# limuhit/pseudocylindrical_convolution

Measured on AMD Instinct MI355X. Metric: ERP MPix/s enc+dec, 4096x2048 model-idx 3, higher is better.
Workload: dtype f32; 1 GPU; ERP 4096x2048 encode+decode, model-idx 3 --ssim (valid_dim 56), 8 frame(s)/GPU/step; frames_per_gpu=8, parallelism=frames sharded, no data-path collective, weights=seeded random (transforms seed 1234, entropy randn*0.05 seed 7), content=smooth, cores_per_rank=16

## Files before the change

include/pconv_hip.h:

```cpp
#ifndef PCONV_HIP_H
#define PCONV_HIP_H

#include <stddef.h>
#include <stdint.h>

#ifdef __cplusplus
extern "C" {
#endif

#define PCONV_OK 0
#define PCONV_EINVAL (-1)
#define PCONV_ELAUNCH (-2)
#define PCONV_ENOMEM (-3)

const char *pconv_last_error(void);
int pconv_abi_version(void);
int pconv_device_count(void);


int pconv_host_tile_widths(const float *weight, int npart, int height, int width,
                           int32_t *widths);
int pconv_host_slice_widths(const float *weight, int npart, int height, int width,
                            int32_t *widths);

int pconv_host_slice_taps(const int32_t *widths, int npart, int width,
                          int32_t *tap_col, float *tap_coef );

int pconv_host_uslice_taps(const int32_t *widths, int npart, int width,
                           int32_t *tap_col, float *tap_coef);

int pconv_host_pad_table(const int32_t *widths, int npart, int height, int width, int pad,
                         int32_t *src_tile, int32_t *src_row, int32_t *col, float *wgt);

int pconv_host_wavefront(const int32_t *widths, int npart, int height, int width,
                         int32_t *order, int32_t *plane_start);

int pconv_host_causal_halo(const int32_t *widths, int npart, int channel, int height,
                           int width, int pad, int32_t *dst, int32_t *src0, int32_t *src1,
                           float *wgt, int32_t *entry_plane, int32_t *plane_start);

int pconv_host_causal_table(const int32_t *widths, int npart, int height, int width, int pad,
                            int32_t *col, float *wgt);

int pconv_host_project_table(const float *theta, const float *phi, int nview, float fov,
                             int h_out, int w_out, int height, int width, float *tf);


int pconv_sphere_slice(const float *in, float *out, const int32_t *widths,
                       const int32_t *tap_col, const float *tap_coef, int n, int c,
                       int height, int width, int npart, int pad, void *stream);

int pconv_sphere_uslice(const float *in, float *out, const int32_t *widths,
                        const int32_t *tap_col, const float *tap_coef, int n, int c, int h,
                        int width, int npart, int pad, void *stream);

int pconv_pseudo_pad(const float *in, float *out, const int32_t *widths,
                     const int32_t *src_tile, const int32_t *src_row, const int32_t *col,
                     const float *wgt, int tn, int c, int h, int w, int pad, int npart,
                     void *stream);

int pconv_pseudo_pad_ring(float *buf, const int32_t *widths, const int32_t *src_tile,
                          const int32_t *src_row, const int32_t *col, const float *wgt, int tn,
                          int c, int h, int w, int pad, int store, int npart, void *stream);

int pconv_pseudo_fill(float *data, const int32_t *widths, int tn, int c, int h, int w,
                      int npart, int pad, int trim, float fvalue, void *stream);

int pconv_dtow(const float *in, float *out, int n, int c, int h, int w, int stride, int d2w,
               void *stream);

int pconv_quant(const float *x, const float *weight, float *level_tab, float *out_val,
                float *out_idx, float *count, const int32_t *widths, int tn, int c, int h,
                int w, int levels, int npart, void *stream);

int pconv_leaky_clip(float *x, long long n, void *stream);

int pconv_frames_u8_to_f32(const uint8_t *in, float *out, int n, int height, int width, void *stream);
int pconv_frames_f32_to_u8(const float *in, uint8_t *out, int n, int height, int width, void *stream);

int pconv_erp_coded_size(int h, int w, int *H, int *W, int *top);
int pconv_frames_u8_to_f32_erp(const uint8_t *in, float *out, int n, int h, int w, void *stream);
int pconv_erp_pad_f32(const float *in, float *out, int n, int h, int w, void *stream);
int pconv_frames_f32_to_u8_crop(const float *in, uint8_t *out, int n, int h, int w, void *stream);

#define PCONV_YUV_420P 0
#define PCONV_YUV_NV12 1
#define PCONV_YUV_420P10LE 2
#define PCONV_YUV_BT709 0
#define PCONV_YUV_BT601 1
#define PCONV_YUV_LIMITED 0
#define PCONV_YUV_FULL 1
#define PCONV_YUV_MAX_WIDTH 11520
int pconv_frames_yuv420_to_f32(const void *in, float *out, int n, int h, int w, int fmt, int matrix, int range,
                               void *stream);
int pconv_frames_f32_to_yuv420(const float *in, void *out, int n, int h, int w, int fmt, int matrix, int range,
                               void *stream);

#define PCONV_WS_WEIGHT_SPHERE 0
#define PCONV_WS_WEIGHT_UNIFORM 1
long long pconv_ws_metrics_workspace_bytes(int n, int h, int w);
int pconv_ws_metrics_f32(const float *x, const float *y, int n, int c, int h, int w, int weighting, void *workspace,
                         double *out, void *stream);
int pconv_ws_metrics_u8(const uint8_t *x, const uint8_t *y, int n, int c, int h, int w, int weighting,
                        void *workspace, double *out, void *stream);

int pconv_ws_metrics_backward_f32(const float *x, const float *y, const double *gout, int n, int c, int h, int w,
                                  int weighting, float *grad_y, void *stream);

long long pconv_ws_msssim_workspace_bytes(int n, int c, int h, int w);
int pconv_ws_msssim_f32(const float *x, const float *y, int n, int c, int h, int w, int weighting, void *workspace,
                        double *out, void *stream);
int pconv_ws_msssim_u8(const uint8_t *x, const uint8_t *y, int n, int c, int h, int w, int weighting, void *workspace,
                       double *out, void *stream);
long long pconv_ws_msssim_backward_workspace_bytes(int n, int c, int h, int w);
int pconv_ws_msssim_backward_f32(const float *x, const float *y, const void *workspace, const double *values,
                                 const double *gout, int n, int c, int h, int w, int weighting, int swapped,
                                 void *backward_workspace, float *grad_y, void *stream);

int pconv_host_lanczos_taps(int n_in, int n_out, int32_t *first, float *weights, int *taps);
long long pconv_erp_resample_workspace_bytes(int n, int c, int h, int w, int h2, int w2);
int pconv_erp_resample_f32(const float *in, float *out, void *workspace, const int32_t *first_x, const float *wx, int tx,
                           const int32_t *first_y, const float *wy, int ty, int n, int c, int h, int w, int h2, int w2,
                           int clamp, void *stream);

long long pconv_host_lanczos_reverse_size(int n_in, int n_out);
int pconv_host_lanczos_reverse(int n_in, int n_out, int pole, int32_t *rev_start, int32_t *rev_entry, uint8_t *crossed);
long long pconv_erp_resample_backward_workspace_bytes(int n, int c, int h, int w, int h2, int w2);
int pconv_erp_resample_backward_f32(const float *gout, float *gin, void *workspace, const float *wx, int tx,
                                    const int32_t *rev_start_x, const int32_t *rev_entry_x, const float *wy, int ty,
                                    const int32_t *rev_start_y, const int32_t *rev_entry_y, const uint8_t *rev_crossed_y,
                                    int n, int c, int h, int w, int h2, int w2, void *stream);

#define PCONV_ERP_ROTATE_PHASES 256
#define PCONV_ERP_ROTATE_TAPS 6
int pconv_host_erp_rotation_matrix(int yaw, int pitch, int roll, int inverse, double *m);
int pconv_host_lanczos_phases(float *weights);
int pconv_erp_rotation_map(int32_t *map, int h, int w, int yaw, int pitch, int roll, int inverse, void *stream);
int pconv_erp_remap_f32(const float *in, float *out, const int32_t *map, const float *phases, int n, int c, int h, int w,
                        int clamp, void *stream);

#define PCONV_VIEWPORT_MAX_SS 4
int pconv_host_viewport_basis(int yaw, int pitch, int roll, int hfov, int vfov, double *out);
int pconv_viewport_map(int32_t *map, int h, int w, int gh, int gw, int yaw, int pitch, int roll, int hfov, int vfov,
                       void *stream);
int pconv_viewport_render_f32(const float *in, float *out, const int32_t *map, const float *phases, int n, int c, int h,
                              int w, int vh, int vw, int ss, long long out_frame_stride, int clamp, void *stream);

#define PCONV_CUBE_CMP 1
#define PCONV_CUBE_EAC 2
#define PCONV_CUBE_PAD 3
#define PCONV_CUBE_MAX_FACE 9453
int pconv_host_cube_face_of(double x, double y, double z);
int pconv_cube_from_erp_map(int32_t *map, int kind, int a, int ss, int h, int w, void *stream);
int pconv_cube_pad_f32(const float *in, float *out, const int32_t *table, int n, int c, int a, void *stream);
int pconv_cube_to_erp_map(int32_t *map, int kind, int a, int h, int w, int ss, void *stream);

#define PCONV_SPHERE_POINTS_LANCZOS 0
#define PCONV_SPHERE_POINTS_NEAREST 1
#define PCONV_SPHERE_POINTS_CHUNK 1024
int pconv_sphere_points_records(const double *points, int32_t *records, long long P, int h, int w, void *stream);
int pconv_sphere_points_sample_f32(const float *in, float *out, const int32_t *records, const float *phases, int n, int c,
                                   int h, int w, long long P, int mode, void *stream);
long long pconv_sphere_points_mse_workspace_bytes(int n, int c, long long P);
int pconv_sphere_points_mse_f32(const float *x, int h1, int w1, const int32_t *rec_x, const float *y, int h2, int w2,
                                const int32_t *rec_y, const float *phases, int n, int c, long long P, int mode,
                                void *workspace, double *out, void *stream);

long long pconv_host_remap_reverse_size(int gh, int gw);
int pconv_host_remap_reverse(const int32_t *map, int gh, int gw, int h, int w, int32_t *rev_start, int32_t *rev_entry);
int pconv_remap_backward_f32(const float *gout, float *gin, const int32_t *map, const float *phases, const int32_t *rev_start,
                             const int32_t *rev_entry, int n, int c, int h, int w, int vh, int vw, int ss,
                             long long gout_frame_stride, int accumulate, void *stream);

int pconv_dquant(const float *x, const float *weight, float *level_tab, float *out,
                 const int32_t *widths, int tn, int c, int h, int w, int wc, int levels,
                 int npart, void *stream);

int pconv_project(const float *in, const float *tf, float *out, int n, int c, int height,
                  int width, int nview, int h_out, int w_out, int nearest, void *stream);

int pconv_context_reshape(const float *in, float *out, int n, int c, int h, int w, int ngroup,
                          void *stream);


int pconv_context_reshape_backward(const float *top, float *bottom, int n, int c, int h, int w,
                                   int ngroup, void *stream);

int pconv_sphere_slice_backward(const float *gout, float *gin, const int32_t *widths,
                                const int32_t *tap_col, const float *tap_coef, int n, int c,
                                int height, int width, int npart, int pad, void *stream);

int pconv_sphere_uslice_backward(const float *gout, float *gin, const int32_t *widths,
                                 const int32_t *tap_col, const float *tap_coef, int n, int c, int h,
                                 int width, int npart, int pad, void *stream);

int pconv_host_pad_reverse(const int32_t *widths, int npart, int height, int width, int pad,
                           int32_t *rev_start, int32_t *rev_dst, float *rev_wgt);

int pconv_pseudo_pad_backward(const float *gout, float *gin, const int32_t *widths,
                              const int32_t *rev_start, const int32_t *rev_dst, const float *rev_wgt,
                              int tn, int c, int h, int w, int pad, int npart, void *stream);

int pconv_entropy_pad(const float *in, float *out, const int32_t *widths, const int32_t *col,
                      const float *wgt, int tn, int c, int h, int w, int pad, int npart, void *stream);
int pconv_host_entropy_pad_table(const int32_t *widths, int npart, int height, int width, int pad,
                                 int version, int32_t *col, float *wgt);
int pconv_host_causal_reverse(const int32_t *widths, int npart, int height, int width, int pad,
                              int version, int32_t *rev_start, int32_t *rev_dst, float *rev_wgt);
int pconv_entropy_pad_backward(const float *gout, float *gin, const int32_t *widths,
                               const int32_t *rev_start, const int32_t *rev_dst, const float *rev_wgt,
                               int tn, int c, int h, int w, int pad, int npart, void *stream);

int pconv_project_backward(const float *gout, const float *tf, float *gin, float *count, int n, int c,
                           int height, int width, int nview, int h_out, int w_out, int nearest,
                           void *stream);

int pconv_quant_backward(const float *x, const float *val, const float *idx, const float *g_val,
                         const float *g_idx, const float *level_tab, float *g_in, float *g_weight,
                         float *bins, const int32_t *widths, float top_alpha, int tn, int c, int h,
                         int w, int levels, int npart, void *stream);


long long pconv_host_tap_reverse_size(const int32_t *widths, int npart, int width, int uslice);

int pconv_host_tap_reverse(const int32_t *widths, int npart, int width, const int32_t *tap_col,
                           const float *tap_coef, int uslice, int32_t *rev_start, int32_t *rev_src,
                           float *rev_coef);

long long pconv_host_project_reverse_size(int nview, int inner, int nearest);

int pconv_host_project_reverse(const float *tf, int nview, int inner, int height, int width, int nearest,
                               int32_t *rev_start, int32_t *rev_sample, float *rev_wgt);

int pconv_sphere_slice_backward_ordered(const float *gout, float *gin, const int32_t *widths,
                                        const int32_t *rev_start, const int32_t *rev_src,
                                        const float *rev_coef, int n, int c, int height, int width,
                                        int npart, int pad, void *stream);
int pconv_sphere_uslice_backward_ordered(const float *gout, float *gin, const int32_t *widths,
                                         const int32_t *rev_start, const int32_t *rev_src,
                                         const float *rev_coef, int n, int c, int h, int width,
                                         int npart, int pad, void *stream);

int pconv_project_backward_ordered(const float *gout, const int32_t *rev_start, const int32_t *rev_sample,
                                   const float *rev_wgt, float *gin, float *count, int n, int c,
                                   int height, int width, int nview, int h_out, int w_out, void *stream);

long long pconv_quant_backward_ordered_workspace_bytes(int tn, int c, int levels);
int pconv_quant_backward_ordered(const float *x, const float *val, const float *idx, const float *g_val,
                                 const float *g_idx, const float *level_tab, float *g_in, float *g_weight,
                                 float *bins, void *workspace, const int32_t *widths, float top_alpha,
                                 int tn, int c, int h, int w, int levels, int npart, void *stream);

int pconv_mask_constrain(float *weight, int nout, int cin, int k, int ngroup, int constrain,
                         void *stream);

int pconv_gmm_loss(const float *weight, const float *delta, const float *mean,
                   const float *label, float *loss, float *d_weight, float *d_delta,
                   float *d_mean, float *d_label, int m, int ng, void *stream);

int pconv_conv_packed_size(int cout, int cin, int k, int *cout_pad, int *red_pad);
int pconv_conv_pack_weight(const float *w, float *packed, int cout, int cin, int k,
                           void *stream);
int pconv_conv2d(const float *in, const float *packed_w, const float *bias, float *out,
                 int tn, int cin, int h, int w, int cout, int k, int stride, int act,
                 const float *slope, const int32_t *col_limit, int npart,
                 const float *residual, const float *gate, int trim, int d2w,
                 const long long *views, void *stream);

int pconv_conv_pack_weight_transposed(const float *w, float *packed, int cout, int cin, int k,
                                      void *stream);
long long pconv_conv2d_dgrad_workspace_bytes(int tn, int cout, int h, int w, int k, int stride);
int pconv_conv_grad_prepare(const float *gout, float *prepared, int tn, int cout, int h, int w,
                            int k, int stride, void *stream);
int pconv_conv2d_dgrad(const float *gout, const float *packed_wt, float *gin, void *workspace,
                       int tn, int cin, int h, int w, int cout, int k, int stride, void *stream);
long long pconv_conv2d_wgrad_workspace_bytes(int tn, int cin, int cout, int k);
int pconv_conv2d_wgrad(const float *in, const float *gout, float *gw, float *gb, void *workspace,
                       int tn, int cin, int h, int w, int cout, int k, int stride, void *stream);

int pconv_conv5_packed_size(int cout, int cin, int *cout_pad, int *red_pad);
int pconv_conv5_pack_weight(const float *w, float *packed, int cout, int cin, void *stream);
int pconv_conv5_pack_weight_transposed(const float *w, float *packed, int cout, int cin, void *stream);
int pconv_conv5(const float *in, const float *packed_w, const float *bias, float *out, int tn, int cin,
                int h, int w, int cout, void *stream);
long long pconv_conv5_dgrad_workspace_bytes(int tn, int cout, int h, int w);
int pconv_conv5_dgrad(const float *gout, const float *packed_wt, float *gin, void *workspace, int tn,
                      int cin, int h, int w, int cout, void *stream);
long long pconv_conv5_wgrad_workspace_bytes(int tn, int cin, int cout);
int pconv_conv5_wgrad(const float *in, const float *gout, float *gw, float *gb, void *workspace, int tn,
                      int cin, int h, int w, int cout, void *stream);

long long pconv_wino_packed_size(int cout, int cin);
int pconv_wino_pack_weight(const float *w, float *packed, int cout, int cin, void *stream);
int pconv_wino_supported(int cin, int h, int w, int cout, int d2w);
int pconv_conv3x3_wino(const float *in, const float *packed_u, const float *bias, float *out,
                       int tn, int cin, int h, int w, int cout, int act, const float *slope,
                       const int32_t *col_limit, int npart, const float *residual, int trim,
                       int d2w, const long long *views, void *stream);
int pconv_conv3x3_wino_flat(const float *in, const float *packed_u, const float *bias, float *out,
                       int tn, int cin, int h, int w, int cout, int act, const float *slope,
                       const int32_t *col_limit, int npart, const float *residual, int trim,
                       int d2w, const long long *views, void *stream);

long long pconv_wino42_packed_size(int cout, int cin);
int pconv_wino42_pack_weight(const float *w, float *packed, int cout, int cin, void *stream);
int pconv_wino42_supported(int cin, int h, int w, int cout, int d2w);
int pconv_conv3x3_wino42(const float *in, const float *packed_u, const float *bias, float *out,
                       int tn, int cin, int h, int w, int cout, int act, const float *slope,
                       const int32_t *col_limit, int npart, const float *residual, int trim,
                       int d2w, const long long *views, void *stream);

int pconv_gdn(const float *in, const float *packed_gamma, const float *beta, float *out,
              int tn, int ch, int h, int w, int inverse, const int32_t *col_limit, int npart,
              const float *residual ,
              const long long *views ,
              void *stream);


int pconv_dinput2(const float *packed, float *ctx, const int32_t *order, int lo, int len,
                  int nimg, int ngroup, int npart, int h, int w, int pad, int psum,
                  float bias, int rep, void *stream);

int pconv_ctx_pad_run2(float *data, const int32_t *dst, const int32_t *src0,
                       const int32_t *src1, const float *wgt, const int32_t *entry_plane,
                       int lo, int len, int nimg, int cpn, int channel, int npart, int h, int w,
                       int pad, int psum, void *stream);

int pconv_entropy_conv(const float *x, const float *weight, const float *bias,
                       const float *slope, float *y, const int32_t *order,
                       const int32_t *plane_start, int first_plane, int nplane, int max_plane_len,
                       int nimg, int per_set, int cin, int cout, int ngroup, int k, int constrain,
                       int npart, int h, int w, int pad_in, int pad_out, int psum,
                       const float *residual, const int32_t *widths, const int32_t *vh_col,
                       const float *vh_wgt, void *stream);

int pconv_entropy_add(float *y, const float *x, const int32_t *order, int lo, int len,
                      int nimg, int channel, int ngroup, int npart, int h, int w, int pad,
                      int psum, void *stream);

int pconv_dextract2(const float *x, float *out, const int32_t *order, int lo, int len,
                    int nimg, int channel, int cpn, int npart, int h, int w, int psum,
                    void *stream);

int pconv_dextract2_batch(const float *x, float *out, const int32_t *order, int lo, int len,
                          int nimg, int channel, int cpn, int npart, int h, int w, int psum,
                          int nout, long long section_stride, void *stream);

int pconv_gmm_table(float *weight, float *delta, const float *mean, float *table, int tn,
                    int ng, int nstep, float bias, float total, float beta, int batch_arith,
                    void *stream);

int pconv_step_tables(const float *y, const float *symbols, int32_t *table, int32_t *labels,
                      const int32_t *order, int lo, int len, int nimg, int ngroup, int npart, int h,
                      int w, int psum, int nstep, float bias, float total, float beta, void *stream);

int pconv_symbols_to_ctx(const float *symbols, float *ctx, const int32_t *widths, int tn, int c,
                         int h, int w, int pad, int npart, float bias, int rep, void *stream);

int pconv_ctx_to_symbols(const float *ctx, float *out, const int32_t *widths, int tn, int c, int h,
                         int w, int pad, int npart, float bias, void *stream);

typedef struct pconv_entropy_engine pconv_entropy_engine;

pconv_entropy_engine *pconv_ee_create(int npart, int ngroup, int h, int w, int nimg,
                                      const float *tile_weight, float bias, int nlevels, float total,
                                      float beta);
void pconv_ee_destroy(pconv_entropy_engine *e);
int pconv_stream_create(void **stream);
int pconv_stream_destroy(void *stream);
int pconv_ee_set_layer(pconv_entropy_engine *e, int layer, const float *weight, const float *bias,
                       const float *slope, void *stream);
long long pconv_ee_symbols_per_image(const pconv_entropy_engine *e);
int pconv_ee_steps(const pconv_entropy_engine *e);
int pconv_ee_host_cpus(void);
int pconv_ee_spin_us(int call_threads);
int pconv_ee_host_plan(int nimg, int *groups, int *group_threads, int *queued_chain, int *blocking_sync);
int pconv_ee_wait_mode(const pconv_entropy_engine *e);
int pconv_ee_encoder_form(const pconv_entropy_engine *e, int layer);
#define PCONV_OPTION_AUTO (-2147483647 - 1)
int pconv_option(const pconv_entropy_engine *e, const char *name, int *value);
int pconv_device_blocking_sync(int enable);
int pconv_ee_encode(pconv_entropy_engine *e, const float *symbols, void *stream);
int pconv_ee_encode_begin(pconv_entropy_engine *e, const float *symbols, void *stream);
int pconv_ee_set_encode_ranges(pconv_entropy_engine *e, int nrange);
int pconv_ee_encode_end(pconv_entropy_engine *e, void *stream);
const uint8_t *pconv_ee_stream(const pconv_entropy_engine *e, int img, size_t *nbytes);
int pconv_ee_decode(pconv_entropy_engine *e, const uint8_t *const *streams, const size_t *nbytes,
                    float *symbols_out, void *stream);
int pconv_ee_rate(pconv_entropy_engine *e, const float *symbols, double *bits_dev, float *map_dev_or_null, void *stream);


typedef struct pconv_optim_tensor {
  float *p;
  const float *grad;
  float *acc;
  float *m;
  float *v;
  long long n;
  float step_size, bc2_sqrt, eps, one_minus_beta1, beta2, one_minus_beta2;
} pconv_optim_tensor;


long long pconv_host_optim_segments(const long long *counts, int ntensor, int32_t *segments);
long long pconv_optim_workspace_bytes(int ntensor, int nsegment);
int pconv_optim_sqnorm(const pconv_optim_tensor *records, const int32_t *segments, const long long *counts,
                       int ntensor, int nsegment, float clip, void *workspace, void *stream);
int pconv_optim_adam(const pconv_optim_tensor *records, const int32_t *segments, const long long *counts,
                     int ntensor, int nsegment, const void *workspace, void *stream);

#ifdef __cplusplus
}
#endif
#endif
```

pseudocylindrical_convolution_amd/PCONV.py:

```python
import collections
import ctypes
import functools
import os
import weakref

import numpy as np
import torch

from . import _native
from ._native import PconvError, call

__all__ = [
    "ProjectsOp", "DtowOp", "ContextReshapeOp", "EntropyGmmOp", "MaskConstrainOp",
    "SphereSliceOp", "SphereUsliceOp", "EntropyGmmTableOp", "EntropyContextOp",
    "EntropyCtxPadRun2Op", "DExtract2Op", "DInput2Op", "EntropyConv2Op", "PseudoContextOp",
    "PseudoPadOp", "PseudoFillOp", "PseudoEntropyContextOp", "PseudoEntropyPadOp",
    "PseudoQuantOp", "PseudoDQuantOp", "EntropyAddOp",
]

_contexts = weakref.WeakValueDictionary()


def _lookup(addr):
    try:
# ... 1516 lines not shown

def _sphere_points_records_of(what, rec, x):
    if rec.dtype != torch.int32 or rec.dim() != 2 or rec.shape[1] != 2 or not rec.is_contiguous() or rec.device != x.device \
            or not 1 <= rec.shape[0] <= SPHERE_POINTS_MAX:
        raise PconvError("%s: the records must be contiguous int32 (P, 2), 1 <= P < 2^28, on the input's device, got %s %s "
                         "on %s" % (what, rec.dtype, tuple(rec.shape), rec.device))
    return rec.shape[0]


def sphere_points_records(points, h, w, out=None):
    h, w = int(h), int(w)
    if not points.is_cuda or points.dtype != torch.float64 or points.dim() != 2 or points.shape[1] != 2 \
            or not points.is_contiguous() or not 1 <= points.shape[0] <= SPHERE_POINTS_MAX:
        raise PconvError("sphere_points_records: contiguous float64 (P, 2) points, 1 <= P < 2^28, on a GPU expected, got %s "
                         "%s on %s" % (points.dtype, tuple(points.shape), points.device))
    _require_sides("sphere_points_records", h, w)
    count = points.shape[0]
    out = _output("sphere_points_records", out, (count, 2), torch.int32, points.device, "the points' device")
    with _HbmTimed("sphere_points_records_kernel", "SpherePointsRecords %dx%d P%d" % (w, h, count), 24.0 * count, points.device):
        call("pconv_sphere_points_records", _ptr(points), _ptr(out), count, h, w, _stream(points.device))
    return out


def sphere_points_sample_f32(x, records, interp="lanczos", out=None):
    n, c, h, w = _require_frames(x, "sphere_points_sample_f32")
    mode = _sphere_points_mode("sphere_points_sample_f32", interp)
    count = _sphere_points_records_of("sphere_points_sample_f32", records, x)
    out = _output("sphere_points_sample_f32", out, (n, c, count), torch.float32, x.device, "the input's device")
    counted = 4.0 * n * c * count * ((36 if mode == 0 else 1) + 1) + 8.0 * n * count
    with _HbmTimed("sphere_points_sample_kernel", "SpherePointsSample %dx%d n%d P%d" % (w, h, n, count), counted, x.device):
        call("pconv_sphere_points_sample_f32", _ptr(x), _ptr(out), _ptr(records), _ptr(_phase_table(x.device)), n, c, h, w,
             count, mode, _stream(x.device))
    return out


def sphere_points_mse_device(x, rec_x, y, rec_y, interp="lanczos"):
    _require_gpu(x, "sphere_points_mse")
    _require_gpu(y, "sphere_points_mse")
    if x.dim() != 4 or y.dim() != 4 or x.shape[:2] != y.shape[:2] or x.device != y.device:
        raise PconvError("sphere_points_mse: two float32 (n, C, h, w) batches of equal n and C on one device expected, got "
                         "%s on %s and %s on %s" % (tuple(x.shape), x.device, tuple(y.shape), y.device))
    mode = _sphere_points_mode("sphere_points_mse", interp)
    count = _sphere_points_records_of("sphere_points_mse", rec_x, x)
    if _sphere_points_records_of("sphere_points_mse", rec_y, y) != count:
        raise PconvError("sphere_points_mse: the two record lists differ in length: %d and %d" % (count, rec_y.shape[0]))
    n, c = x.shape[:2]
    nbytes = call("pconv_sphere_points_mse_workspace_bytes", n, c, count)
    workspace = torch.empty((nbytes,), dtype=torch.uint8, device=x.device)
    out = torch.empty((n, c), dtype=torch.float64, device=x.device)
    counted = 4.0 * n * c * count * 2 * (36 if mode == 0 else 1) + 16.0 * n * c * count
    with _HbmTimed("sphere_points_mse_kernel", "SpherePointsMse n%d P%d" % (n, count), counted, x.device):
        call("pconv_sphere_points_mse_f32", _ptr(x), x.shape[2], x.shape[3], _ptr(rec_x), _ptr(y), y.shape[2], y.shape[3],
             _ptr(rec_y), _ptr(_phase_table(x.device)), n, c, count, mode, _ptr(workspace), _ptr(out), _stream(x.device))
    return out


def sphere_points_mse(x, rec_x, y, rec_y, interp="lanczos"):
    return sphere_points_mse_device(x, rec_x, y, rec_y, interp).cpu()


def viewport_map(h, w, gh, gw, view, device=None, out=None):
    h, w, gh, gw = int(h), int(w), int(gh), int(gw)
    try:
        yaw, pitch, roll, hfov, vfov = (int(v) for v in view)
    except (TypeError, ValueError):
        raise PconvError("viewport_map: a view is five integers in units of 2^-16 degree, got %r" % (view,))
    device = _gpu_device("viewport_map", device)
    if not (2 <= gh <= 1 << 22 and 2 <= gw <= 1 << 22) or 8 * gh * gw >= 1 << 31:
        raise PconvError("viewport_map: a grid of %dx%d: sides of 2 .. 2^22 and a map below 2^31 bytes expected" % (gw, gh))
    out = _output("viewport_map", out, (gh, gw, 2), torch.int32, device, device)
    with torch.cuda.device(device), _HbmTimed("viewport_map_kernel", "ViewportMap %dx%d" % (gw, gh), 8.0 * gh * gw, device):
        call("pconv_viewport_map", _ptr(out), h, w, gh, gw, yaw, pitch, roll, hfov, vfov, _stream(device))
    return out


def viewport_render_f32(x, map, vh, vw, ss, clamp=False, out=None, slot=0):
    n, c, h, w = _require_frames(x, "viewport_render_f32")
    vh, vw, ss, slot = int(vh), int(vw), int(ss), int(slot)
    _require_view("viewport_render_f32", vh, vw, ss)
    _require_map("viewport_render_f32", map, vh * ss, vw * ss, x.device, "the input's device")
    table = _phase_table(x.device)
    if out is None:
        out = torch.empty((n, 1, c, vh, vw), dtype=torch.float32, device=x.device)
    elif out.dim() != 5 or out.shape[0] != n or tuple(out.shape[2:]) != (c, vh, vw) or out.dtype != torch.float32 \
            or not out.is_contiguous() or out.device != x.device:
        raise PconvError("viewport_render_f32: out must be contiguous float32 (%d, V, %d, %d, %d) on the input's device"
                         % (n, c, vh, vw))
    views = out.shape[1]
    if not 0 <= slot < views:
        raise PconvError("viewport_render_f32: slot %d of %d views" % (slot, views))
    frame = c * vh * vw
    counted = 4.0 * 36 * n * c * vh * vw * ss * ss + 8.0 * n * c * vh * vw * ss * ss + 4.0 * n * frame
    with _HbmTimed("viewport_render_f32_kernel", "ViewportRender %dx%d->%dx%d ss%d n%d" % (w, h, vw, vh, ss, n), counted,
                   x.device):
        call("pconv_viewport_render_f32", _ptr(x), out.data_ptr() + 4 * slot * frame, _ptr(map), _ptr(table), n, c, h, w,
             vh, vw, ss, views * frame, 1 if clamp else 0, _stream(x.device))
    return out


def remap_backward_f32(gout, map, lists, h, w, vh, vw, ss, gin=None, slot=0, accumulate=False):
    _require_gpu(gout, "remap_backward_f32")
    h, w, vh, vw, ss, slot = int(h), int(w), int(vh), int(vw), int(ss), int(slot)
    if gout.dim() == 4:
        gout = gout.unsqueeze(1)
    if gout.dim() != 5 or tuple(gout.shape[3:]) != (vh, vw) or not gout.is_contiguous():
        raise PconvError("remap_backward_f32: a contiguous float32 (n, V, C, %d, %d) or (n, C, %d, %d) gradient expected, got %s"
                         % (vh, vw, vh, vw, tuple(gout.shape)))
    n, views, c = gout.shape[:3]
    if not 0 <= slot < views:
        raise PconvError("remap_backward_f32: slot %d of %d views" % (slot, views))
    _require_view("remap_backward_f32", vh, vw, ss)
    _require_map("remap_backward_f32", map, vh * ss, vw * ss, gout.device, "the gradient's device")
    entries = 36 * vh * ss * vw * ss
    try:
        start, entry = lists
        good = all(t.dtype == torch.int32 and t.dim() == 1 and t.is_contiguous() and t.device == gout.device
                   for t in (start, entry)) and start.numel() == h * w + 1 and entry.numel() == entries
    except (TypeError, ValueError, AttributeError):
        good = False
    if not good:
        raise PconvError("remap_backward_f32: lists must be (start, entry) of viewport.reverse_lists for this map and a %dx%d "
                         "source: contiguous int32 of %d and %d elements on the gradient's device" % (w, h, h * w + 1, entries))
    if gin is None and accumulate:
        raise PconvError("remap_backward_f32: accumulate needs the gin to add to")
    gin = _output("remap_backward_f32", gin, (n, c, h, w), torch.float32, gout.device, "the gradient's device", "gin")
    table = _phase_table(gout.device)
    frame = c * vh * vw
    counted = n * ((c + 3) // 4) * (4.0 * entries + 8.0 * entries + 4.0 * (h * w + 1)) + 4.0 * n * c * entries \
        + 4.0 * gin.numel() * (2 if accumulate else 1)
    with _HbmTimed("remap_backward_f32_kernel", "RemapBackward %dx%d<-%dx%d ss%d n%d" % (w, h, vw, vh, ss, n), counted,
                   gout.device):
        call("pconv_remap_backward_f32", gout.data_ptr() + 4 * slot * frame, _ptr(gin), _ptr(map), _ptr(table), _ptr(start),
             _ptr(entry), n, c, h, w, vh, vw, ss, views * frame, 1 if accumulate else 0, _stream(gout.device))
    return gin


CUBE_KINDS = {"cmp": 1, "eac": 2}
CUBE_PAD = 3
CUBE_MAX_FACE = 9453


def _cube_args(what, kind, a, ss):
    if kind not in CUBE_KINDS:
        raise PconvError("%s: kind must be one of %s, got %r" % (what, sorted(CUBE_KINDS), kind))
    a, ss = int(a), int(ss)
    if not (2 <= a <= CUBE_MAX_FACE and 1 <= ss <= 4):
        raise PconvError("%s: a face size of %d with ss = %d: a of 2 .. %d and ss of 1 .. 4 expected" % (what, a, ss, CUBE_MAX_FACE))
    return CUBE_KINDS[kind], a, ss


def cube_from_erp_map(kind, a, ss, h, w, device=None, out=None):
    code, a, ss = _cube_args("cube_from_erp_map", kind, a, ss)
    h, w = int(h), int(w)
    device = _gpu_device("cube_from_erp_map", device)
    _require_sides("cube_from_erp_map", h, w)
    gs = a * ss
    if 8 * 6 * gs * gs >= 1 << 31:
        raise PconvError("cube_from_erp_map: a map of %dx%d records is 2^31 bytes or more" % (gs, 6 * gs))
    out = _output("cube_from_erp_map", out, (6 * gs, gs, 2), torch.int32, device, device)
    with torch.cuda.device(device), _HbmTimed("cube_from_erp_map_kernel", "CubeFromErpMap a%d ss%d" % (a, ss), 48.0 * gs * gs,
                                              device):
        call("pconv_cube_from_erp_map", _ptr(out), code, a, ss, h, w, _stream(device))
    return out


def cube_to_erp_map(kind, a, h, w, ss, device=None, out=None):
    code, a, ss = _cube_args("cube_to_erp_map", kind, a, ss)
    h, w = int(h), int(w)
    device = _gpu_device("cube_to_erp_map", device)
    _require_sides("cube_to_erp_map", h, w)
    if 8 * h * ss * w * ss >= 1 << 31:
        raise PconvError("cube_to_erp_map: a map of %dx%d records is 2^31 bytes or more" % (w * ss, h * ss))
    out = _output("cube_to_erp_map", out, (h * ss, w * ss, 2), torch.int32, device, device)
    with torch.cuda.device(device), _HbmTimed("cube_to_erp_map_kernel", "CubeToErpMap %dx%d ss%d" % (w, h, ss),
                                              8.0 * h * w * ss * ss, device):
        call("pconv_cube_to_erp_map", _ptr(out), code, a, h, w, ss, _stream(device))
    return out


def cube_pad_f32(x, table, out=None):
    n, c, h6, a = _require_frames(x, "cube_pad_f32")
    if h6 != 6 * a or not 2 <= a <= CUBE_MAX_FACE:
        raise PconvError("cube_pad_f32: a face stack (n, C, 6 a, a), a of 2 .. %d, expected, got %s" % (CUBE_MAX_FACE, tuple(x.shape)))
    A = a + 2 * CUBE_PAD
    ring = 6 * (A * A - a * a)
    if table.dtype != torch.int32 or tuple(table.shape) != (ring, 3) or not table.is_contiguous() or table.device != x.device:
        raise PconvError("cube_pad_f32: the table must be contiguous int32 (%d, 3) on the input's device" % ring)
    out = _output("cube_pad_f32", out, (n, c, 6 * A, A), torch.float32, x.device, "the input's device")
    counted = 4.0 * (x.numel() + out.numel()) + n * c * ring * (12.0 + 16.0)
    with _HbmTimed("cube_pad_f32_kernel", "CubePad a%d n%d" % (a, n), counted, x.device):
        call("pconv_cube_pad_f32", _ptr(x), _ptr(out), _ptr(table), n, c, a, _stream(x.device))
    return out


WS_WEIGHTINGS = {"ws": 0, "uniform": 1}


def ws_metrics(x, y, weighting="ws"):
    return ws_metrics_device(x, y, weighting).cpu()


def _ws_frames(what, x, y, weighting, float_only, min_side, entry):
    if weighting not in WS_WEIGHTINGS:
        raise PconvError("%s: weighting must be one of %s, got %r" % (what, sorted(WS_WEIGHTINGS), weighting))
    if not (x.is_cuda and y.is_cuda):
        raise PconvError("%s: expected GPU tensors (this build has no CPU path), got %s and %s" % (what, x.device, y.device))
    if x.device != y.device or x.dtype != y.dtype or x.shape != y.shape:
        raise PconvError("%s: the two batches differ: %s %s %s vs %s %s %s"
                         % (what, x.device, x.dtype, tuple(x.shape), y.device, y.dtype, tuple(y.shape)))
    if not (x.is_contiguous() and y.is_contiguous()) or x.dim() != 4:
        raise PconvError("%s: contiguous 4-D tensors expected" % what)
    if x.dtype == torch.float32:
        n, c, h, w = x.shape
        fn = entry + "_f32"
    elif x.dtype == torch.uint8 and x.shape[3] == 3 and not float_only:
        n, h, w, c = x.shape
        fn = entry + "_u8"
    else:
        raise PconvError("%s: float32 (n, C, h, w)%s expected, got %s %s"
                         % (what, "" if float_only else " or uint8 (n, h, w, 3)", x.dtype, tuple(x.shape)))
    if h < min_side or w < min_side:
        raise PconvError("%s: h and w must be at least %d, got %dx%d" % (what, min_side, w, h))
    return (n, c, h, w), fn


def _ws_gout(what, gout, x):
    n = x.shape[0]
    if not gout.is_cuda or gout.device != x.device or gout.dtype != torch.float64 or tuple(gout.shape) != (n, 2) \
            or not gout.is_contiguous():
        raise PconvError("%s: gout must be contiguous float64 (%d, 2) on the inputs' device, got %s %s %s"
                         % (what, n, gout.device, gout.dtype, tuple(gout.shape)))


def ws_metrics_device(x, y, weighting="ws"):
    (n, c, h, w), fn = _ws_frames("ws_metrics", x, y, weighting, False, 1, "pconv_ws_metrics")
    nbytes = call("pconv_ws_metrics_workspace_bytes", n, h, w)
    workspace = torch.empty((nbytes,), dtype=torch.uint8, device=x.device)
    out = torch.empty((n, 2), dtype=torch.float64, device=x.device)
    with _HbmTimed("ms_forward_kernel", "WsMetrics n%d" % n, 2.0 * x.numel() * x.element_size(), x.device):
        call(fn, _ptr(x), _ptr(y), n, c, h, w, WS_WEIGHTINGS[weighting], _ptr(workspace), _ptr(out), _stream(x.device))
    return out


def ws_metrics_backward(x, y, gout, weighting="ws"):
    (n, c, h, w), _ = _ws_frames("ws_metrics_backward", x, y, weighting, True, 1, "pconv_ws_metrics")
    _ws_gout("ws_metrics_backward", gout, x)
    out = torch.empty_like(x)
    with _HbmTimed("ms_backward_kernel", "WsMetricsBackward n%d" % n, 12.0 * x.numel(), x.device):
        call("pconv_ws_metrics_backward_f32", _ptr(x), _ptr(y), _ptr(gout), n, c, h, w, WS_WEIGHTINGS[weighting],
             _ptr(out), _stream(x.device))
    return out


WS_MS_SCALES, WS_MS_MIN_SIDE = 5, 16


def ws_msssim_device(x, y, weighting="ws"):
    (n, c, h, w), fn = _ws_frames("ws_msssim", x, y, weighting, False, WS_MS_MIN_SIDE, "pconv_ws_msssim")
    nbytes = call("pconv_ws_msssim_workspace_bytes", n, c, h, w)
    workspace = torch.empty((nbytes,), dtype=torch.uint8, device=x.device)
    out = torch.empty((n, 7), dtype=torch.float64, device=x.device)
    counted = 2.0 * x.numel() * x.element_size() + 2.0 * (2.0 * n * c * h * w * 4 / 3)
    with _HbmTimed("ms_forward_kernel", "WsMsSsim n%d" % n, counted, x.device):
        call(fn, _ptr(x), _ptr(y), n, c, h, w, WS_WEIGHTINGS[weighting], _ptr(workspace), _ptr(out), _stream(x.device))
    return out, workspace


def ws_msssim(x, y, weighting="ws"):
    out, workspace = ws_msssim_device(x, y, weighting)
    return out.cpu(), workspace


def ws_msssim_levels(workspace, n, c, h, w):
    levels, at = [], 0
    for s in range(1, WS_MS_SCALES):
        hs, ws = h >> s, w >> s
        size = n * c * hs * ws
        pair = workspace[4 * at:4 * (at + 2 * size)].view(torch.float32)
        levels.append((pair[:size].view(n, c, hs, ws), pair[size:].view(n, c, hs, ws)))
        at += 2 * size
    return levels


def ws_msssim_backward(x, y, workspace, values, gout, weighting="ws", swapped=False):
    (n, c, h, w), _ = _ws_frames("ws_msssim_backward", x, y, weighting, True, WS_MS_MIN_SIDE, "pconv_ws_msssim")
    _ws_gout("ws_msssim_backward", gout, x)
    if values.device != x.device or values.dtype != torch.float64 or tuple(values.shape) != (n, 7) \
            or not values.is_contiguous():
        raise PconvError("ws_msssim_backward: values must be contiguous float64 (%d, 7) on the inputs' device, got %s %s %s"
                         % (n, values.device, values.dtype, tuple(values.shape)))
    nbytes = call("pconv_ws_msssim_workspace_bytes", n, c, h, w)
    if workspace.device != x.device or workspace.dtype != torch.uint8 or workspace.numel() != nbytes \
            or not workspace.is_contiguous():
        raise PconvError("ws_msssim_backward: the workspace must be the %d bytes ws_msssim_device returned, got %s %s %s"
                         % (nbytes, workspace.device, workspace.dtype, tuple(workspace.shape)))
    coarse = torch.empty((call("pconv_ws_msssim_backward_workspace_bytes", n, c, h, w),), dtype=torch.uint8, device=x.device)
    out = torch.empty_like(x)
    with _HbmTimed("ms_backward_kernel", "WsMsSsimBackward n%d" % n, 16.0 * x.numel(), x.device):
        call("pconv_ws_msssim_backward_f32", _ptr(x), _ptr(y), _ptr(workspace), _ptr(values), _ptr(gout), n, c, h, w,
             WS_WEIGHTINGS[weighting], 1 if swapped else 0, _ptr(coarse), _ptr(out), _stream(x.device))
    return out


def tile_gdn(owner, x, gamma, beta, inverse, col_limit=None, npart=0, residual=None, ring=0):
    x = _require_rows(x, "tile_gdn")
    tn, ch, h, w = x.shape
    stream = _stream(x.device)
    packed = packed_conv_weight(owner, gamma.view(ch, ch, 1, 1), stream)
    out = _ring_output((tn, ch, h, w), ring, x)
    residual = _like_output(residual, out, "tile_gdn: residual")
    views = _views(x, out, residual)

    def describe():
        return (conv_kernel_name(ch, 1, 1, True, cin=ch, pixels=tn * h * w), "GDN %d w%d" % (ch, w),
                2.0 * ch * ch * tn * h * w * _VALID_FRACTION,
                4.0 * ch * tn * h * w * _VALID_FRACTION * (3 if residual is not None else 2))

    with _ConvTimed(x.device, describe):
        call("pconv_gdn", _ptr(x), _ptr(packed), _ptr(beta.detach().contiguous()), _ptr(out), tn, ch, h, w,
             1 if inverse else 0, _ptr(col_limit), int(npart), _ptr(residual), ctypes.addressof(views), stream)
    return out


FUSED_EPILOGUE = True


def tile_conv2d(owner, x, weight, bias, stride, slope=None, col_limit=None, npart=0, sigmoid=False, gate=None,
                residual=None, trim=False, ring=0, d2w=False):
    x = _require_rows(x, "tile_conv2d")
    tn, cin, h, w = x.shape
    cout, cin_w, k, k2 = weight.shape
    if cin != cin_w or k != k2:
        raise PconvError("tile_conv2d: weight %s does not fit input %s" % (tuple(weight.shape), tuple(x.shape)))
    stream = _stream(x.device)
    ho, wo = (h - k) // stride + 1, (w - k) // stride + 1
    out = _ring_output((tn, cout // 4, 2 * ho, 2 * wo) if d2w else (tn, cout, ho, wo), ring, x)
    if sigmoid and slope is not None:
        raise PconvError("tile_conv2d: PReLU and sigmoid are exclusive")
    if d2w and (gate is not None or residual is not None or trim or sigmoid or cout % 4):
        raise PconvError("tile_conv2d: d2w takes no sigmoid / gate / residual / trim and needs cout % 4 == 0")
    gate = _like_output(gate, out, "tile_conv2d: gate")
    residual = _like_output(residual, out, "tile_conv2d: residual")
    aligned = k == 3 and _aligned8(out) and (residual is None or _aligned8(residual))
    launches, fallback = conv_plan(cin, h, w, cout, k, stride, d2w, sigmoid or gate is not None, aligned)
    if fallback:
        key = (cin, h, w, cout, bool(d2w))
        conv_fallbacks[key] = conv_fallbacks.get(key, 0) + 1
    act = 4 if sigmoid else (1 if slope is not None else 0)
    bias_p, slope_p = _ptr(bias.detach()) if bias is not None else None, _ptr(slope.detach()) if slope is not None else None

    def winograd(kind, r0, rows):
        kernel = CONV_KERNELS[kind]
        whole = r0 == 0 and rows == ho
        rs = 2 if d2w else 1
        xv = x if whole else x[:, :, r0:r0 + rows + 2]
        ov = out if whole else out[:, :, rs * r0:rs * (r0 + rows)]
        rv = residual if (whole or residual is None) else residual[:, :, r0:r0 + rows]

        def describe():
            return (kernel.probe_name, "3x3 s1 %d->%d w%d" % (cin, cout, wo) + ("" if whole else (" rows %d of %d" % (rows, ho))),
                    2.0 * cin * 9 * cout * tn * rows * wo * _VALID_FRACTION,
                    4.0 * tn * _VALID_FRACTION * (cin * (rows + 2) * w + cout * rows * wo * (1 + (residual is not None))))

        with _ConvTimed(x.device, describe):
            views = _views(xv, ov, rv)
            call(kernel.entry, _ptr(xv), _ptr(_packed_weight(owner, weight, kind, stream)), bias_p, _ptr(ov), tn, cin,
                 rows + 2, w, cout, act, slope_p, _ptr(col_limit), int(npart), _ptr(rv), 1 if trim else 0,
                 1 if d2w else 0, ctypes.addressof(views), stream)

    def direct():
        def describe():
            return (conv_kernel_name(cout, k, stride, cin=cin, pixels=tn * h * w),
                    "%dx%d s%d %d->%d w%d" % (k, k, stride, cin, cout, wo), 2.0 * cin * k * k * cout * tn * ho * wo * _VALID_FRACTION,
                    4.0 * tn * _VALID_FRACTION * (cin * h * w + cout * ho * wo * (1 + (residual is not None) + (gate is not None))))

        with _ConvTimed(x.device, describe):
            views = _views(x, out, residual, gate)
            call("pconv_conv2d", _ptr(x), _ptr(_packed_weight(owner, weight, "direct", stream)), bias_p, _ptr(out),
                 tn, cin, h, w, cout, k, int(stride), act, slope_p, _ptr(col_limit), int(npart),
                 _ptr(residual), _ptr(gate), 1 if trim else 0, 1 if d2w else 0, ctypes.addressof(views), stream)

    for kind, r0, rows in launches:
        if kind == "direct":
            direct()
        else:
            winograd(kind, r0, rows)
    return out


def _conv_tensors(where, tensors):
    first = tensors[0][1]
    for name, t, dims in tensors:
        if not isinstance(t, torch.Tensor) or t.dim() != dims:
            raise PconvError("%s: %s must be a %d-D tensor" % (where, name, dims))
        _require_gpu(t.detach(), "%s: %s" % (where, name))
        if t.device != first.device:
            raise PconvError("%s: %s is on %s, %s on %s" % (where, name, t.device, tensors[0][0], first.device))


ConvFamily = collections.namedtuple(
    "ConvFamily", "ksizes strides sized slot_t packed_size pack_weight_transposed dgrad_workspace dgrad wgrad_workspace wgrad")
_TILE_CONV = ConvFamily((1, 3), (1, 2), True, "_pconv_packed_t", "pconv_conv_packed_size", "pconv_conv_pack_weight_transposed",
                        "pconv_conv2d_dgrad_workspace_bytes", "pconv_conv2d_dgrad", "pconv_conv2d_wgrad_workspace_bytes",
                        "pconv_conv2d_wgrad")
_CONV5 = ConvFamily((5,), (1,), False, "_pconv_packed5_t", "pconv_conv5_packed_size", "pconv_conv5_pack_weight_transposed",
                    "pconv_conv5_dgrad_workspace_bytes", "pconv_conv5_dgrad", "pconv_conv5_wgrad_workspace_bytes",
                    "pconv_conv5_wgrad")


def _pack_transposed(weight, family, stream):
    cout, cin, k = weight.shape[:3]
    ks = (k,) if family.sized else ()
    return _pack(weight, family.packed_size, (cin, cout) + ks + (None, None), family.pack_weight_transposed, (cout, cin) + ks,
                 stream)


def _conv_backward(where, family, x, weight, gout, stride, need, owner):
    need_x, need_w, need_b = (bool(n) for n in need)
    _conv_tensors(where, [("gout", gout, 4), ("x", x, 4), ("weight", weight, 4)])
    tn, cout, ho, wo = gout.shape
    cout_w, cin, k, k2 = weight.shape
    stride = int(stride)
    tn_x, cin_x, h, w = x.shape
    if (tn_x, cin_x, cout_w, k2) != (tn, cin, cout, k) or k not in family.ksizes or stride not in family.strides or \
            ((h - k) // stride + 1, (w - k) // stride + 1) != (ho, wo) or ho < 1 or wo < 1:
        raise PconvError("%s: x %s, weight %s, gout %s, stride %d do not fit"
                         % (where, tuple(x.shape), tuple(weight.shape), tuple(gout.shape), stride))
    stream = _stream(gout.device)
    lib = _native.hip_lib()
    ks, kst = ((k,), (k, stride)) if family.sized else ((), ())

    def workspace(nbytes):
        if nbytes < 0:
            raise PconvError("%s: workspace query failed: %s" % (where, (lib.pconv_last_error() or b"").decode()))
        return torch.empty(int(nbytes), dtype=torch.uint8, device=gout.device) if nbytes else None

    gin = gw = gb = None
    if need_x:
        packed = _cached_pack(weight if owner is None else owner, family.slot_t, weight, _pack_transposed, family, stream)
        gin = torch.empty((tn, cin, h, w), dtype=torch.float32, device=gout.device)
        ws = workspace(getattr(lib, family.dgrad_workspace)(tn, cout, h, w, *kst))
        call(family.dgrad, _ptr(gout), _ptr(packed), _ptr(gin), _ptr(ws), tn, cin, h, w, cout, *kst + (stream,))
    if need_w or need_b:
        if need_w:
            gw = torch.empty((cout, cin, k, k), dtype=torch.float32, device=gout.device)
        if need_b:
            gb = torch.empty((cout,), dtype=torch.float32, device=gout.device)
        ws = workspace(getattr(lib, family.wgrad_workspace)(tn, cin, cout, *ks) if need_w else tn * cout * 8)
        call(family.wgrad, _ptr(x) if need_w else None, _ptr(gout), _ptr(gw), _ptr(gb), _ptr(ws), tn, cin, h, w, cout,
             *kst + (stream,))
    return gin, gw, gb


def tile_conv2d_backward(x, weight, gout, stride, need=(True, True, True), owner=None):
    return _conv_backward("tile_conv2d_backward", _TILE_CONV, x, weight, gout, stride, need, owner)



OptimSegments = collections.namedtuple("OptimSegments", "table counts ntensor nsegment")


def optim_segments(counts, device):
    counts = np.ascontiguousarray(counts, dtype=np.int64)
    if counts.ndim != 1 or counts.size < 1:
        raise PconvError("optim_segments: a non-empty list of element counts expected")
    nsegment = call("pconv_host_optim_segments", _np_ptr(counts), counts.size, None)
    table = np.empty((nsegment, 2), dtype=np.int32)
    call("pconv_host_optim_segments", _np_ptr(counts), counts.size, _np_ptr(table))
    return OptimSegments(torch.from_numpy(table).to(device), counts, int(counts.size), int(nsegment))


def optim_step(records, segments, clip, device):
    if records.dtype != torch.int64 or tuple(records.shape) != (segments.ntensor, 9) or not records.is_cuda or \
            not records.is_contiguous() or records.device != segments.table.device or records.device != torch.device(device):
        raise PconvError("optim_step: records must be a contiguous (%d, 9) int64 tensor on %s" % (segments.ntensor, device))
    stream = _stream(records.device)
    nbytes = call("pconv_optim_workspace_bytes", segments.ntensor, segments.nsegment)
    ws = torch.empty(nbytes // 8, dtype=torch.float64, device=records.device)
    args = (_ptr(records), _ptr(segments.table), _np_ptr(segments.counts), segments.ntensor, segments.nsegment)
    call("pconv_optim_sqnorm", *args + (float(clip), _ptr(ws), stream))
    call("pconv_optim_adam", *args + (_ptr(ws), stream))
    return ws



def _pack5(weight, stream):
    cout, cin = weight.shape[:2]
    return _pack(weight, "pconv_conv5_packed_size", (cout, cin, None, None), "pconv_conv5_pack_weight", (cout, cin), stream)


def conv5x5(owner, x, weight, bias):
    _conv_tensors("conv5x5", [("x", x, 4), ("weight", weight, 4)] + ([("bias", bias, 1)] if bias is not None else []))
    tn, cin, h, w = x.shape
    cout, cin_w, k, k2 = weight.shape
    if cin != cin_w or (k, k2) != (5, 5) or h < 5 or w < 5 or (bias is not None and bias.shape[0] != cout):
        raise PconvError("conv5x5: weight %s does not fit input %s" % (tuple(weight.shape), tuple(x.shape)))
    stream = _stream(x.device)
    out = torch.empty((tn, cout, h - 4, w - 4), dtype=torch.float32, device=x.device)
    call("pconv_conv5", _ptr(x), _ptr(_cached_pack(owner, "_pconv_packed5", weight, _pack5, stream)),
         _ptr(bias.detach()) if bias is not None else None, _ptr(out), tn, cin, h, w, cout, stream)
    return out


def conv5x5_backward(x, weight, gout, need=(True, True, True), owner=None):
    return _conv_backward("conv5x5_backward", _CONV5, x, weight, gout, 1, need, owner)
```

pseudocylindrical_convolution_amd/PCONV_operator/ops.py:

```python
import math

import torch
from torch import nn

from . import backend
from .BaseOpModule import BaseOpModule, native_call
from .GDN import LowerBound
from .base import set_weight


def _per_gpu(module, factory):
    return {gid: factory(gid) for gid in module.device_list}


class SphereSlice(BaseOpModule):

    def __init__(self, npart, interp_type=0, pad=0, opt=False, device=0, time_it=False):
        super(SphereSlice, self).__init__(device)
        weight = set_weight(npart, opt)
        self.op = _per_gpu(self, lambda g: backend.ops().SphereSliceOp(npart, interp_type, pad, weight, g, time_it))

    def forward(self, x):
        return native_call(self, 'forward', (x,))


class SphereUslice(BaseOpModule):

    def __init__(self, npart, interp_type=0, pad=0, opt=False, device=0, time_it=False):
        super(SphereUslice, self).__init__(device)
        weight = set_weight(npart, opt)
        self.op = _per_gpu(self, lambda g: backend.ops().SphereUsliceOp(npart, interp_type, pad, weight, g, time_it))

    def forward(self, x):
        return native_call(self, 'forward', (x,))


class Dtow(BaseOpModule):

    def __init__(self, stride=2, d2w=False, device=0, time_it=False):
        super(Dtow, self).__init__(device)
        self.op = _per_gpu(self, lambda g: backend.ops().DtowOp(stride, d2w, g, time_it))

    def forward(self, x):
        return native_call(self, 'forward', (x,))


class MultiProjectM(BaseOpModule):

    def __init__(self, h, w, thetas, phis, fov=0.6, near=False, device_id=0, time_flag=False):
        super(MultiProjectM, self).__init__(device_id)
        self.op = _per_gpu(self, lambda g: backend.ops().ProjectsOp(int(h), int(w), thetas, phis, fov, near, g, time_flag))

    def forward(self, x):
        return native_call(self, 'forward', (x,))


class MultiProject(MultiProjectM):
    THETAS = [-0.5, 0, 0.5, 1, -0.5, 0, 0.5, 1, -0.5, 0, 0.5, 1, 0, 0]
    PHIS = [0, 0, 0, 0, 0.25, 0.25, 0.25, 0.25, -0.25, -0.25, -0.25, -0.25, 0.5, -0.5]

    def __init__(self, h, w, fov=0.6, near=False, device_id=0, time_flag=False):
        self.thetas, self.phis = list(self.THETAS), list(self.PHIS)
        super(MultiProject, self).__init__(h, w, self.thetas, self.phis, fov, near, device_id, time_flag)


class _Context(BaseOpModule):

    def setup_context(self, w):
        for op in self.op.values():
            op.start_context(w)

    def get_addr(self, gid):
        return self.op[gid].addr()


class PseudoContextV2(_Context):

    def __init__(self, npart, opt=True, rt=20, device=0, time_it=False):
        super(PseudoContextV2, self).__init__(device)
        weight = set_weight(npart, opt)
        self.op = _per_gpu(self, lambda g: backend.ops().PseudoContextOp(npart, rt, weight, g, time_it))

    def produce_fill_param(self, gid, h, w):
        return self.op[gid].produce_fill_param(h, w)


class PseudoEntropyContext(_Context):

    def __init__(self, npart, context_version=1, opt=True, rt=20, device=0, time_it=False):
        super(PseudoEntropyContext, self).__init__(device)
        weight = set_weight(npart, opt)
        self.op = _per_gpu(self, lambda g: backend.ops().PseudoEntropyContextOp(npart, rt, context_version, weight, g, time_it))


class EntropyContextNew(_Context):

    def __init__(self, npart, rt=18, opt=False, device=0, time_it=False):
        super(EntropyContextNew, self).__init__(device)
        weight = set_weight(npart, opt)
        self.op = _per_gpu(self, lambda g: backend.ops().EntropyContextOp(npart, rt, weight, g, time_it))


class PseudoPadV2(BaseOpModule):

    def __init__(self, pad, npart, ctx, device=0, time_it=False):
        super(PseudoPadV2, self).__init__(device)
        self.op = _per_gpu(self, lambda g: backend.ops().PseudoPadOp(pad, npart, ctx.get_addr(g), g, time_it))

    def forward(self, x):
        op = self.native(x)
        if getattr(x, "_pconv_ring", None) is not None and hasattr(op, "forward_ring") \
                and not torch.is_grad_enabled():
            return op.forward_ring(x)
        return native_call(self, 'forward', (x,))


class PseudoEntropyPad(BaseOpModule):

    def __init__(self, pad, npart, ctx, device=0, time_it=False):
        super(PseudoEntropyPad, self).__init__(device)
        self.op = _per_gpu(self, lambda g: backend.ops().PseudoEntropyPadOp(pad, npart, ctx.get_addr(g), g, time_it))

    def forward(self, x):
        return native_call(self, 'forward', (x,))


class PseudoFillV2(BaseOpModule):

    def __init__(self, pad, npart, ctx, fvalue=0, trim=0, device=0, time_it=False):
        super(PseudoFillV2, self).__init__(device)
        version = 0 if isinstance(ctx, PseudoContextV2) else (1 if isinstance(ctx, PseudoEntropyContext) else 2)
        self.op = _per_gpu(self, lambda g: backend.ops().PseudoFillOp(pad, npart, fvalue, trim, ctx.get_addr(g), version, g, time_it))

    def forward(self, x):
        return native_call(self, 'forward', (x,))


class PseudoGDNV2(nn.Module):

    def __init__(self, ch, npart, ctx, device=0, inverse=False, beta_min=1e-6, gamma_init=.1,
                 reparam_offset=2 ** -18):
        super(PseudoGDNV2, self).__init__()
        self.inverse = inverse
        self.beta_min = beta_min
        self.gamma_init = gamma_init
        self.reparam_offset = torch.FloatTensor([reparam_offset])
        self.trim = PseudoFillV2(0, npart, ctx, device=device)
        self.mask = None
        self.__dict__["ctx"] = ctx
        gid = device if isinstance(device, int) else device[0]
        self.build(ch, torch.device(backend.device_of(gid)))

    def build(self, ch, device):
        self.pedestal = self.reparam_offset ** 2
        self.beta_bound = (self.beta_min + self.reparam_offset ** 2) ** .5
        self.gamma_bound = self.reparam_offset
        self.beta = nn.Parameter(torch.sqrt(torch.ones(ch) + self.pedestal).to(device))
        gamma = torch.sqrt(self.gamma_init * torch.eye(ch) + self.pedestal)
        self.gamma = nn.Parameter(gamma.to(device))
        self.pedestal = self.pedestal.to(device)

    def setup_mask(self, x):
        if self.mask is not None and self.mask.shape == x.shape and self.mask.device == x.device:
            return
        self.mask = self.trim(torch.ones_like(x).detach())

    def effective(self):
        key = (self.gamma._version, self.beta._version, self.gamma.device, backend.param_epoch())
        if getattr(self, "_effective", (None,))[0] != key:
            with torch.no_grad():
                pedestal = self.pedestal.to(self.gamma.device)
                beta = LowerBound.apply(self.beta, self.beta_bound) ** 2 - pedestal
                gamma = LowerBound.apply(self.gamma, self.gamma_bound) ** 2 - pedestal
            self._effective = (key, gamma.contiguous(), beta.contiguous())
        return self._effective[1], self._effective[2]

    def forward(self, inputs, residual=None, trim=None, ring=0):
        ops = backend.ops()
        if hasattr(ops, "tile_gdn") and inputs.is_cuda and not torch.is_grad_enabled():
            gamma, beta = self.effective()
            ctx_op = self.ctx.native(inputs)
            limit, npart = ops.conv_col_limit(ctx_op, inputs.shape[2], inputs.shape[3], 0, inputs)
            return ops.tile_gdn(self, inputs, gamma, beta, self.inverse, limit, npart, residual, ring)
        out = self._formula(inputs)
        if residual is not None:
            out = residual + out
        return trim(out) if trim is not None else out

    def _formula(self, inputs):
        self.pedestal = self.pedestal.to(inputs.device)
        ch = inputs.size(1)
        self.setup_mask(inputs)
        inputs = inputs * self.mask
        beta = LowerBound.apply(self.beta, self.beta_bound) ** 2 - self.pedestal
        gamma = LowerBound.apply(self.gamma, self.gamma_bound) ** 2 - self.pedestal
        ops = backend.ops()
        trains = torch.is_grad_enabled() and (inputs.requires_grad or gamma.requires_grad or beta.requires_grad)
        if trains and inputs.is_cuda and hasattr(ops, "tile_conv2d_backward") and ops.conv_grad_is_native():
            norm_ = TileConvCall.apply(None, (inputs ** 2).contiguous(), gamma.view(ch, ch, 1, 1).contiguous(),
                                       beta.contiguous(), 1)
        else:
            norm_ = nn.functional.conv2d(inputs ** 2, gamma.view(ch, ch, 1, 1), beta)
        norm_ = torch.sqrt(norm_)
        norm_ = norm_ * self.mask + 1 - self.mask
        return inputs * norm_ if self.inverse else inputs / norm_


class _QuantCall(torch.autograd.Function):

    @staticmethod
    def forward(ctx, module, x, weight, count, training):
        op = module.native(x)
        outs = op.forward(x, weight, count, training)
        ctx.op = op
        ctx.save_for_backward(x, outs[0])
        return outs[0] if len(outs) == 1 else (outs[0], outs[1])

    @staticmethod
    def backward(ctx, *grads):
        x, out = ctx.saved_tensors
        g = [t.contiguous() if t is not None else torch.zeros_like(x) for t in grads]
        gx, gw, gc = ctx.op.backward(g, x, out)
        return None, gx, gw, gc.clone().detach(), None


class _Uncached(object):
    """owner of the packed weights of one TileConvCall whose weight is not a parameter"""


class TileConvCall(torch.autograd.Function):

    @staticmethod
    def forward(ctx, owner, x, weight, bias, stride):
        ops = backend.ops()
        owner = owner if owner is not None else _Uncached()
        ctx.owner, ctx.stride, ctx.has_bias = owner, int(stride), bias is not None
        ctx.save_for_backward(x, weight)
        return ops.tile_conv2d(owner, x, weight, bias, int(stride))

    @staticmethod
    @torch.autograd.function.once_differentiable
    def backward(ctx, gout):
        x, weight = ctx.saved_tensors
        need = (ctx.needs_input_grad[1], ctx.needs_input_grad[2], ctx.has_bias and ctx.needs_input_grad[3])
        gin, gw, gb = backend.ops().tile_conv2d_backward(x.contiguous(), weight, gout.contiguous(), ctx.stride, need,
                                                         owner=ctx.owner)
        return None, gin, gw, gb, None


class MaskConvCall(torch.autograd.Function):

    @staticmethod
    def forward(ctx, owner, x, weight, bias):
        ctx.owner, ctx.has_bias = owner, bias is not None
        ctx.save_for_backward(x, weight)
        return backend.ops().conv5x5(owner, x, weight, bias)

    @staticmethod
    @torch.autograd.function.once_differentiable
    def backward(ctx, gout):
        x, weight = ctx.saved_tensors
        need = (ctx.needs_input_grad[1], ctx.needs_input_grad[2], ctx.has_bias and ctx.needs_input_grad[3])
        gin, gw, gb = backend.ops().conv5x5_backward(x, weight, gout.contiguous(), need, owner=ctx.owner)
        return None, gin, gw, gb


class PseudoQUANTV2(BaseOpModule):

    def __init__(self, channel, bin_num, npart, ctx, check_iters=100, weight_decay=0.9, ntop=1,
                 top_alpha=0.1, device_id=0, time_flag=False):
        super(PseudoQUANTV2, self).__init__(device_id)
        dev = backend.device_of(self.device_list[0])
        first = 1. / (bin_num + 1)
        weight = torch.zeros((channel, bin_num), dtype=torch.float32)
        weight[:, 0] = first
        weight[:, 1:] = math.log(first)
        self.weight = nn.Parameter(weight.to(dev))
        self.count = nn.Parameter(torch.zeros((channel, bin_num), dtype=torch.float32).to(dev))
        self.ntop = ntop
        self.op = _per_gpu(self, lambda g: backend.ops().PseudoQuantOp(
            channel, bin_num, npart, weight_decay, check_iters, ntop, top_alpha, ctx.get_addr(g), g, time_flag))

    def forward(self, x):
        if not x.is_contiguous():
            x = x.contiguous()
        if torch.is_grad_enabled() and (x.requires_grad or self.weight.requires_grad):
            return _QuantCall.apply(self, x, self.weight, self.count, self.training)
        outs = self.native(x).forward(x, self.weight, self.count, self.training)
        return outs[0] if len(outs) == 1 else (outs[0], outs[1])

    def call_counters(self):
        return {int(g): int(op.iter_) for g, op in self.op.items()}

    def set_call_counters(self, counters):
        for g, n in counters.items():
            self.op[int(g)].iter_ = int(n)


class PseudoDQUANT(BaseOpModule):

    def __init__(self, channel, bin_num, npart, ctx, device_id=0, time_flag=False):
        super(PseudoDQUANT, self).__init__(device_id)
        dev = backend.device_of(self.device_list[0])
        self.weight = nn.Parameter(torch.zeros((channel, bin_num), dtype=torch.float32).to(dev))
        self.op = _per_gpu(self, lambda g: backend.ops().PseudoDQuantOp(npart, channel, bin_num, ctx.get_addr(g), g, time_flag))

    def forward(self, x):
        if not x.is_contiguous():
            x = x.contiguous()
        return self.native(x).forward(x, self.weight)[0]


class _Restartable(BaseOpModule):

    def restart(self):
        for op in self.op.values():
            op.restart()


class EntropyAdd(_Restartable):

    def __init__(self, npart, channel, ngroup, pad, ctx, device=0, time_it=False):
        super(EntropyAdd, self).__init__(device)
        self.op = _per_gpu(self, lambda g: backend.ops().EntropyAddOp(npart, channel, ngroup, pad, ctx.get_addr(g), g, time_it))

    def forward(self, x, y):
        return self.native(x).forward(x, y)[0]


class EntropyCtxPadRun2(_Restartable):

    def __init__(self, pad, npart, ngroup, ctx, input=False, device=0, time_it=False):
        super(EntropyCtxPadRun2, self).__init__(device)
        self.op = _per_gpu(self, lambda g: backend.ops().EntropyCtxPadRun2Op(pad, npart, ngroup, input, ctx.get_addr(g), g, time_it))

    def forward(self, x):
        return self.native(x).forward(x)[0]


class DExtract2(_Restartable):

    def __init__(self, npart, nchannel, label, ctx, device=0, time_it=False):
        super(DExtract2, self).__init__(device)
        self.op = _per_gpu(self, lambda g: backend.ops().DExtract2Op(npart, nchannel, label, ctx.get_addr(g), g, time_it))

    def forward(self, x):
        if not x.is_contiguous():
            x = x.contiguous()
        out = self.native(x).forward(x)
        return out[0], out[1]


class DExtract2Batch(_Restartable):

    def __init__(self, npart, nchannel, ctx, device=0, time_it=False):
        super(DExtract2Batch, self).__init__(device)
        self.op = _per_gpu(self, lambda g: backend.ops().DExtract2Op(npart, nchannel, True, ctx.get_addr(g), g, time_it))

    def forward(self, x):
        out = self.native(x).forward_batch(x)
        return out[0], out[1]


class DInput2(_Restartable):

    def __init__(self, nchannel, npart, ctx, pad=0, bias=0, repeat=1, device=0, time_it=False):
        super(DInput2, self).__init__(device)
        self.op = _per_gpu(self, lambda g: backend.ops().DInput2Op(nchannel, npart, pad, bias, repeat, ctx.get_addr(g), g, time_it))

    def forward(self, x):
        if not x.is_contiguous():
            x = x.contiguous()
        return self.native(x).forward(x)[0]


class EntropyConv2(_Restartable):

    def __init__(self, npart, ngroup, c_in, c_out, kernel_size, ctx, pad_in=2, pad_out=2, hidden=False,
                 act=True, device=0, time_it=False):
        super(EntropyConv2, self).__init__(device)
        constrain = 6 if hidden else 5
        channel, nout = ngroup * c_in, ngroup * c_out
        self.op = _per_gpu(self, lambda g: backend.ops().EntropyConv2Op(
            npart, channel, ngroup, nout, kernel_size, constrain, pad_in, pad_out, ctx.get_addr(g), g, time_it))
        self.weight = nn.Parameter(torch.rand((nout, channel, kernel_size, kernel_size), dtype=torch.float32))
        self.bias = nn.Parameter(torch.zeros((nout), dtype=torch.float32))
        self.act = act
        self.relu = nn.Parameter(torch.zeros((nout), dtype=torch.float32)) if act else None

    def forward(self, x):
        op = self.native(x)
        if self.act:
            return op.forward_act(x, self.weight, self.bias, self.relu)[0]
        return op.forward(x, self.weight, self.bias)[0]


class EntropyConv2Batch(_Restartable):

    def __init__(self, npart, ngroup, c_in, c_out, kernel_size, ctx, pad_in=2, pad_out=2, batch=3,
                 hidden=False, act=True, device=0, time_it=False):
        super(EntropyConv2Batch, self).__init__(device)
        constrain = 6 if hidden else 5
        channel, nout = ngroup * c_in, ngroup * c_out
        self.op = _per_gpu(self, lambda g: backend.ops().EntropyConv2Op(
            npart, channel, ngroup, nout, kernel_size, constrain, pad_in, pad_out, ctx.get_addr(g), g, time_it))
        self.weight = nn.Parameter(torch.rand((batch, nout, channel, kernel_size, kernel_size), dtype=torch.float32))
        self.bias = nn.Parameter(torch.rand((batch, nout), dtype=torch.float32))
        self.act = act
        self.relu = nn.Parameter(torch.rand((batch, nout), dtype=torch.float32)) if act else None

    def forward(self, x):
        op = self.native(x)
        if self.act:
            return op.forward_act_batch(x, self.weight, self.bias, self.relu)[0]
        return op.forward_batch(x, self.weight, self.bias)[0]


class EntropyConvD(nn.Module):

    def __init__(self, ngroups, cin, cout, hidden, npart, out_layer, ctx, device_id, act=True):
        super(EntropyConvD, self).__init__()
        self.pad = EntropyCtxPadRun2(2, npart, ngroups, ctx, not hidden, device=device_id)
        self.conv = EntropyConv2(npart, ngroups, cin, cout, 5, ctx, 2, 0 if out_layer else 2, hidden=hidden,
                                 act=act, device=device_id)

    def forward(self, x):
        return self.conv(self.pad(x))


class EntropyResidualBlockD(nn.Module):

    def __init__(self, ngroups, cpn, npart, ctx, device_id=0):
        super(EntropyResidualBlockD, self).__init__()
        self.conv1 = EntropyConvD(ngroups, cpn, cpn, True, npart, False, ctx, device_id, True)
        self.conv2 = EntropyConvD(ngroups, cpn, cpn, True, npart, False, ctx, device_id, True)
        self.add = EntropyAdd(npart, cpn * ngroups, ngroups, 2, ctx, device=device_id)

    def forward(self, x):
        return self.add(self.conv2(self.conv1(x)), x)


class EntropyGmmTable(BaseOpModule):

    def __init__(self, nstep, bias, num_gaussian, total_region, beta=1e-6, device=0, time_it=False):
        super(EntropyGmmTable, self).__init__(device)
        self.op = _per_gpu(self, lambda g: backend.ops().EntropyGmmTableOp(nstep, bias, num_gaussian, total_region, beta, g, time_it))

    def forward(self, weight, delta, mean, ntop):
        args = [t if t.is_contiguous() else t.contiguous() for t in (weight, delta, mean)]
        return self.native(weight).forward(args[0], args[1], args[2], ntop)[0]


class EntropyBatchGmmTable(BaseOpModule):

    def __init__(self, nstep, bias, num_gaussian, total_region, beta=1e-6, device=0, time_it=False):
        super(EntropyBatchGmmTable, self).__init__(device)
        self.op = _per_gpu(self, lambda g: backend.ops().EntropyGmmTableOp(nstep, bias, num_gaussian, total_region, beta, g, time_it))

    def forward(self, x, ntop):
        if not x.is_contiguous():
            x = x.contiguous()
        return self.native(x).forward_batch(x, ntop)[0]


class EntropyGmm(BaseOpModule):

    def __init__(self, num_gaussian=3, ignore_label=0, device=0, time_it=False):
        super(EntropyGmm, self).__init__(device)
        self.op = _per_gpu(self, lambda g: backend.ops().EntropyGmmOp(num_gaussian, ignore_label, g, time_it))

    def forward(self, weight, delta, mean, label):
        return native_call(self, 'forward', (weight, delta, mean, label))


class ContextReshape(BaseOpModule):

    def __init__(self, ngroup, device=0, time_it=False):
        super(ContextReshape, self).__init__(device)
        self.op = _per_gpu(self, lambda g: backend.ops().ContextReshapeOp(ngroup, g, time_it))

    def forward(self, x):
        return native_call(self, 'forward', (x,))


class _MaskConv(BaseOpModule):

# ... 92 lines not shown
```

pseudocylindrical_convolution_amd/_native.py:

```python
import ctypes
import os
from ctypes import POINTER, c_char_p, c_float, c_int, c_int32, c_longlong, c_size_t, c_uint8, c_uint32, c_void_p

HERE = os.path.dirname(os.path.abspath(__file__))


class PconvError(RuntimeError):
    pass


P = c_void_p
I = c_int
F = c_float
LL = c_longlong
D = ctypes.c_double

_HIP_SIGNATURES = {
    "pconv_host_tile_widths": [P, I, I, I, P],
    "pconv_host_slice_widths": [P, I, I, I, P],
    "pconv_host_slice_taps": [P, I, I, P, P],
    "pconv_host_uslice_taps": [P, I, I, P, P],
    "pconv_host_pad_table": [P, I, I, I, I, P, P, P, P],
    "pconv_host_wavefront": [P, I, I, I, P, P],
    "pconv_host_causal_halo": [P, I, I, I, I, I, P, P, P, P, P, P],
    "pconv_host_project_table": [P, P, I, F, I, I, I, I, P],
    "pconv_sphere_slice": [P, P, P, P, P, I, I, I, I, I, I, P],
    "pconv_sphere_uslice": [P, P, P, P, P, I, I, I, I, I, I, P],
    "pconv_pseudo_pad": [P, P, P, P, P, P, P, I, I, I, I, I, I, P],
    "pconv_pseudo_pad_ring": [P, P, P, P, P, P, I, I, I, I, I, I, I, P],
    "pconv_pseudo_fill": [P, P, I, I, I, I, I, I, I, F, P],
    "pconv_dtow": [P, P, I, I, I, I, I, I, P],
    "pconv_quant": [P, P, P, P, P, P, P, I, I, I, I, I, I, P],
    "pconv_dquant": [P, P, P, P, P, I, I, I, I, I, I, I, P],
    "pconv_leaky_clip": [P, LL, P],
    "pconv_frames_u8_to_f32": [P, P, I, I, I, P],
    "pconv_frames_f32_to_u8": [P, P, I, I, I, P],
    "pconv_erp_coded_size": [I, I, P, P, P],
    "pconv_frames_u8_to_f32_erp": [P, P, I, I, I, P],
    "pconv_erp_pad_f32": [P, P, I, I, I, P],
    "pconv_frames_f32_to_u8_crop": [P, P, I, I, I, P],
    "pconv_frames_yuv420_to_f32": [P, P, I, I, I, I, I, I, P],
    "pconv_frames_f32_to_yuv420": [P, P, I, I, I, I, I, I, P],
    "pconv_ws_metrics_workspace_bytes": [I, I, I],
    "pconv_ws_metrics_f32": [P, P, I, I, I, I, I, P, P, P],
    "pconv_ws_metrics_u8": [P, P, I, I, I, I, I, P, P, P],
    "pconv_ws_metrics_backward_f32": [P, P, P, I, I, I, I, I, P, P],
    "pconv_ws_msssim_workspace_bytes": [I, I, I, I],
    "pconv_ws_msssim_f32": [P, P, I, I, I, I, I, P, P, P],
    "pconv_ws_msssim_u8": [P, P, I, I, I, I, I, P, P, P],
    "pconv_ws_msssim_backward_workspace_bytes": [I, I, I, I],
    "pconv_ws_msssim_backward_f32": [P, P, P, P, P, I, I, I, I, I, I, P, P, P],
    "pconv_host_lanczos_taps": [I, I, P, P, P],
    "pconv_erp_resample_workspace_bytes": [I, I, I, I, I, I],
    "pconv_erp_resample_f32": [P, P, P, P, P, I, P, P, I, I, I, I, I, I, I, I, P],
    "pconv_host_lanczos_reverse_size": [I, I],
    "pconv_host_lanczos_reverse": [I, I, I, P, P, P],
    "pconv_erp_resample_backward_workspace_bytes": [I, I, I, I, I, I],
    "pconv_erp_resample_backward_f32": [P, P, P, P, I, P, P, P, I, P, P, P, I, I, I, I, I, I, P],
    "pconv_host_erp_rotation_matrix": [I, I, I, I, P],
    "pconv_host_lanczos_phases": [P],
    "pconv_erp_rotation_map": [P, I, I, I, I, I, I, P],
    "pconv_erp_remap_f32": [P, P, P, P, I, I, I, I, I, P],
    "pconv_host_viewport_basis": [I, I, I, I, I, P],
    "pconv_viewport_map": [P, I, I, I, I, I, I, I, I, I, P],
    "pconv_viewport_render_f32": [P, P, P, P, I, I, I, I, I, I, I, LL, I, P],
    "pconv_host_cube_face_of": [D, D, D],
    "pconv_cube_from_erp_map": [P, I, I, I, I, I, P],
    "pconv_cube_pad_f32": [P, P, P, I, I, I, P],
    "pconv_cube_to_erp_map": [P, I, I, I, I, I, P],
    "pconv_host_remap_reverse_size": [I, I],
    "pconv_host_remap_reverse": [P, I, I, I, I, P, P],
    "pconv_remap_backward_f32": [P, P, P, P, P, P, I, I, I, I, I, I, I, LL, I, P],
    "pconv_sphere_points_records": [P, P, LL, I, I, P],
    "pconv_sphere_points_sample_f32": [P, P, P, P, I, I, I, I, LL, I, P],
    "pconv_sphere_points_mse_workspace_bytes": [I, I, LL],
    "pconv_sphere_points_mse_f32": [P, I, I, P, P, I, I, P, P, I, I, LL, I, P, P, P],
    "pconv_project": [P, P, P, I, I, I, I, I, I, I, I, P],
    "pconv_context_reshape": [P, P, I, I, I, I, I, P],
    "pconv_mask_constrain": [P, I, I, I, I, I, P],
    "pconv_context_reshape_backward": [P, P, I, I, I, I, I, P],
    "pconv_sphere_slice_backward": [P, P, P, P, P, I, I, I, I, I, I, P],
    "pconv_sphere_uslice_backward": [P, P, P, P, P, I, I, I, I, I, I, P],
    "pconv_host_pad_reverse": [P, I, I, I, I, P, P, P],
    "pconv_pseudo_pad_backward": [P, P, P, P, P, P, I, I, I, I, I, I, P],
    "pconv_quant_backward": [P, P, P, P, P, P, P, P, P, P, F, I, I, I, I, I, I, P],
    "pconv_project_backward": [P, P, P, P, I, I, I, I, I, I, I, I, P],
    "pconv_host_tap_reverse_size": [P, I, I, I],
    "pconv_host_tap_reverse": [P, I, I, P, P, I, P, P, P],
    "pconv_host_project_reverse_size": [I, I, I],
    "pconv_host_project_reverse": [P, I, I, I, I, I, P, P, P],
    "pconv_sphere_slice_backward_ordered": [P, P, P, P, P, P, I, I, I, I, I, I, P],
    "pconv_sphere_uslice_backward_ordered": [P, P, P, P, P, P, I, I, I, I, I, I, P],
    "pconv_project_backward_ordered": [P, P, P, P, P, P, I, I, I, I, I, I, I, P],
    "pconv_quant_backward_ordered_workspace_bytes": [I, I, I],
    "pconv_quant_backward_ordered": [P, P, P, P, P, P, P, P, P, P, P, F, I, I, I, I, I, I, P],
    "pconv_entropy_pad": [P, P, P, P, P, I, I, I, I, I, I, P],
    "pconv_host_entropy_pad_table": [P, I, I, I, I, I, P, P],
    "pconv_host_causal_reverse": [P, I, I, I, I, I, P, P, P],
    "pconv_entropy_pad_backward": [P, P, P, P, P, P, I, I, I, I, I, I, P],
    "pconv_gmm_loss": [P, P, P, P, P, P, P, P, P, I, I, P],
    "pconv_conv_packed_size": [I, I, I, P, P],
    "pconv_conv_pack_weight": [P, P, I, I, I, P],
    "pconv_conv2d": [P, P, P, P, I, I, I, I, I, I, I, I, P, P, I, P, P, I, I, P, P],
    "pconv_conv_pack_weight_transposed": [P, P, I, I, I, P],
    "pconv_conv2d_dgrad_workspace_bytes": [I, I, I, I, I, I],
    "pconv_conv_grad_prepare": [P, P, I, I, I, I, I, I, P],
    "pconv_conv2d_dgrad": [P, P, P, P, I, I, I, I, I, I, I, P],
    "pconv_conv2d_wgrad_workspace_bytes": [I, I, I, I],
    "pconv_conv2d_wgrad": [P, P, P, P, P, I, I, I, I, I, I, I, P],
    "pconv_conv5_packed_size": [I, I, P, P],
    "pconv_conv5_pack_weight": [P, P, I, I, P],
    "pconv_conv5_pack_weight_transposed": [P, P, I, I, P],
    "pconv_conv5": [P, P, P, P, I, I, I, I, I, P],
    "pconv_conv5_dgrad_workspace_bytes": [I, I, I, I],
    "pconv_conv5_dgrad": [P, P, P, P, I, I, I, I, I, P],
    "pconv_conv5_wgrad_workspace_bytes": [I, I, I],
    "pconv_conv5_wgrad": [P, P, P, P, P, I, I, I, I, I, P],
    "pconv_gdn": [P, P, P, P, I, I, I, I, I, P, I, P, P, P],
    "pconv_wino_packed_size": [I, I],
    "pconv_wino_pack_weight": [P, P, I, I, P],
    "pconv_wino_supported": [I, I, I, I, I],
    "pconv_conv3x3_wino": [P, P, P, P, I, I, I, I, I, I, P, P, I, P, I, I, P, P],
    "pconv_conv3x3_wino_flat": [P, P, P, P, I, I, I, I, I, I, P, P, I, P, I, I, P, P],
    "pconv_wino42_packed_size": [I, I],
    "pconv_wino42_pack_weight": [P, P, I, I, P],
    "pconv_wino42_supported": [I, I, I, I, I],
    "pconv_conv3x3_wino42": [P, P, P, P, I, I, I, I, I, I, P, P, I, P, I, I, P, P],
    "pconv_dinput2": [P, P, P, I, I, I, I, I, I, I, I, I, F, I, P],
    "pconv_ctx_pad_run2": [P, P, P, P, P, P, I, I, I, I, I, I, I, I, I, I, P],
    "pconv_entropy_conv": [P, P, P, P, P, P, P, I, I, I, I, I, I, I, I, I, I, I, I, I, I, I, I, P, P, P, P, P],
    "pconv_host_causal_table": [P, I, I, I, I, P, P],
    "pconv_entropy_add": [P, P, P, I, I, I, I, I, I, I, I, I, I, P],
    "pconv_dextract2": [P, P, P, I, I, I, I, I, I, I, I, I, P],
    "pconv_dextract2_batch": [P, P, P, I, I, I, I, I, I, I, I, I, I, LL, P],
    "pconv_gmm_table": [P, P, P, P, I, I, I, F, F, F, I, P],
    "pconv_ctx_to_symbols": [P, P, P, I, I, I, I, I, I, F, P],
    "pconv_symbols_to_ctx": [P, P, P, I, I, I, I, I, I, F, I, P],
    "pconv_step_tables": [P, P, P, P, P, I, I, I, I, I, I, I, I, I, F, F, F, P],
    "pconv_ee_set_layer": [P, I, P, P, P, P],
    "pconv_ee_steps": [P],
    "pconv_ee_host_cpus": [],
    "pconv_ee_spin_us": [I],
    "pconv_ee_host_plan": [I, P, P, P, P],
    "pconv_ee_wait_mode": [P],
    "pconv_ee_encoder_form": [P, I],
    "pconv_option": [P, c_char_p, P],
    "pconv_device_blocking_sync": [I],
    "pconv_stream_create": [P],
    "pconv_stream_destroy": [P],
    "pconv_ee_encode": [P, P, P],
    "pconv_ee_encode_begin": [P, P, P],
    "pconv_ee_set_encode_ranges": [P, I],
    "pconv_ee_encode_end": [P, P],
    "pconv_ee_decode": [P, P, P, P, P],
    "pconv_ee_rate": [P, P, P, P, P],
    "pconv_host_optim_segments": [P, I, P],
    "pconv_optim_workspace_bytes": [I, I],
    "pconv_optim_sqnorm": [P, P, P, I, I, F, P, P],
    "pconv_optim_adam": [P, P, P, I, I, P, P],
}

_CODER_SIGNATURES = {
    "pconv_coder_new": ([c_char_p], c_void_p),
    "pconv_coder_free": ([c_void_p], None),
    "pconv_coder_error": ([c_void_p], c_char_p),
    "pconv_coder_start_encoder": ([c_void_p], c_int),
    "pconv_coder_encode": ([c_void_p, P, c_uint32, c_uint32, c_uint32], c_int),
    "pconv_coder_encodes": ([c_void_p, P, c_int, P, c_int], c_int),
    "pconv_coder_end_encoder": ([c_void_p], c_int),
    "pconv_coder_bytes": ([c_void_p, POINTER(c_size_t)], POINTER(c_uint8)),
    "pconv_coder_start_decoder": ([c_void_p], c_int),
    "pconv_coder_start_decoder_mem": ([c_void_p, P, c_size_t], c_int),
    "pconv_coder_decode": ([c_void_p, P, c_uint32, c_uint32], c_int),
    "pconv_coder_decodes": ([c_void_p, P, c_int, P, c_int], c_int),
    "pconv_coder_decodes_i32": ([c_void_p, P, c_int, P, c_int], c_int),
    "pconv_coder_encodes_rows16": ([c_void_p, P, c_int], c_int),
    "pconv_coder_decodes_rows16_i32": ([c_void_p, P, P, c_int], c_int),
}

_hip = None
_coder = None


def _load(name):
    path = os.path.join(HERE, name)
    if name == "libpconv_hip.so" and os.environ.get("PCONV_HIP_LIB"):
        path = os.environ["PCONV_HIP_LIB"]
    if not os.path.exists(path):
        raise PconvError(
            "%s is not built: run `python -m pseudocylindrical_convolution_amd.build` "
            "(needs hipcc, targets gfx950); there is no CPU fallback" % path)
    return ctypes.CDLL(path)


def hip_lib():
    global _hip
    if _hip is None:
        lib = _load("libpconv_hip.so")
        for fn, args in _HIP_SIGNATURES.items():
            f = getattr(lib, fn)
            f.argtypes = args
            f.restype = c_int
        lib.pconv_last_error.restype = c_char_p
        lib.pconv_last_error.argtypes = []
        lib.pconv_abi_version.restype = c_int
        lib.pconv_device_count.restype = c_int
        lib.pconv_ee_create.argtypes = [I, I, I, I, I, P, F, I, F, F]
        lib.pconv_ee_create.restype = c_void_p
        lib.pconv_ee_destroy.argtypes = [P]
        lib.pconv_ee_destroy.restype = None
        lib.pconv_ee_symbols_per_image.argtypes = [P]
        lib.pconv_ee_symbols_per_image.restype = c_longlong
        lib.pconv_ee_stream.argtypes = [P, I, POINTER(c_size_t)]
        lib.pconv_ee_stream.restype = POINTER(c_uint8)
        lib.pconv_wino_packed_size.restype = c_longlong
        lib.pconv_wino42_packed_size.restype = c_longlong
        lib.pconv_ws_metrics_workspace_bytes.restype = c_longlong
        lib.pconv_ws_msssim_workspace_bytes.restype = c_longlong
        lib.pconv_ws_msssim_backward_workspace_bytes.restype = c_longlong
        lib.pconv_erp_resample_workspace_bytes.restype = c_longlong
        lib.pconv_erp_resample_backward_workspace_bytes.restype = c_longlong
        lib.pconv_host_lanczos_reverse_size.restype = c_longlong
        lib.pconv_sphere_points_mse_workspace_bytes.restype = c_longlong
        lib.pconv_host_tap_reverse_size.restype = c_longlong
        lib.pconv_host_project_reverse_size.restype = c_longlong
        lib.pconv_host_remap_reverse_size.restype = c_longlong
        lib.pconv_quant_backward_ordered_workspace_bytes.restype = c_longlong
        lib.pconv_conv2d_dgrad_workspace_bytes.restype = c_longlong
        lib.pconv_conv2d_wgrad_workspace_bytes.restype = c_longlong
        lib.pconv_conv5_dgrad_workspace_bytes.restype = c_longlong
        lib.pconv_conv5_wgrad_workspace_bytes.restype = c_longlong
        lib.pconv_host_optim_segments.restype = c_longlong
        lib.pconv_optim_workspace_bytes.restype = c_longlong
        _hip = lib
    return _hip


def coder_lib():
    global _coder
    if _coder is None:
        lib = _load("libpconv_coder.so")
        for fn, (args, res) in _CODER_SIGNATURES.items():
            f = getattr(lib, fn)
            f.argtypes = args
            f.restype = res
        _coder = lib
    return _coder


def declared_hip_symbols():
    return sorted(list(_HIP_SIGNATURES) + ["pconv_last_error", "pconv_abi_version", "pconv_device_count",
                                           "pconv_ee_create", "pconv_ee_destroy", "pconv_ee_symbols_per_image",
                                           "pconv_ee_stream"])


def declared_coder_symbols():
    return sorted(_CODER_SIGNATURES)


def check(rc, what=""):
    if rc < 0:
        msg = hip_lib().pconv_last_error()
        raise PconvError("%s failed (%d): %s" % (what or "pconv call", rc, (msg or b"").decode()))
    return rc


def call(fn, *args):
    lib = hip_lib()
    return check(getattr(lib, fn)(*args), fn)


def option(name, engine=None):
    value = c_int(0)
    call("pconv_option", engine, name.encode(), ctypes.addressof(value))
    return value.value
```

pseudocylindrical_convolution_amd/csrc/conv.hip:

```cpp
#include <atomic>
#include <utility>
#include "options.h"
#include "conv_host.h"

namespace {

typedef float f32x16 __attribute__((ext_vector_type(16)));

constexpr int kTileCols = 64;
#ifndef PCONV_PIPE_ROWS
#define PCONV_PIPE_ROWS(both) ((both) ? 8 : 8)
#endif
#ifndef PCONV_KC1
#define PCONV_KC1 16
#endif
constexpr int kKC5 = 2;
#ifndef PCONV_QUAD_AHEAD
#define PCONV_QUAD_AHEAD 2
#endif
#ifndef PCONV_QUAD_AHEAD_GDN
#define PCONV_QUAD_AHEAD_GDN 2
#endif

template <int ROWS, int KS, int S>
struct Patch {
  static constexpr int PS = (KS == 1) ? S : 1;
  static constexpr int Q = S / PS;
  static constexpr int PR = (ROWS - 1) * Q + KS;
  static constexpr int PC = (kTileCols - 1) * Q + KS;
};

template <int MT, int NT, int WM, int WN, int KS, int S, int KC>
struct ConvCfg {
  static constexpr int THREADS = 64 * WM * WN;
  static constexpr int ROWS = WN * NT / 2;
  static constexpr int BM = 32 * MT * WM;
  static constexpr int KK = KC * KS * KS;
  using P = Patch<ROWS, KS, S>;
  static constexpr int XSZ = KC * P::PR * P::PC;
  static constexpr int WSZ = KK * BM;
  static constexpr int STAGE = XSZ + WSZ;
  static constexpr int XLD = (XSZ + THREADS - 1) / THREADS;
  static constexpr int WLD = (WSZ / 4 + THREADS - 1) / THREADS;
  static constexpr int MTv = MT, NTv = NT, KSv = KS;
  static constexpr int patch_off(int k) {
    return (k / (KS * KS)) * P::PR * P::PC + ((k / KS) % KS) * P::PC + (k % KS);
  }
  static constexpr int ND = (KS == 1) ? 1 : 3;
  static constexpr int delta(int i) {
    return KS == 1 ? P::PR * P::PC : (i == 0 ? 1 : (i == 1 ? P::PC - (KS - 1) : P::PR * P::PC - (KS - 1) * P::PC - (KS - 1)));
  }
  static constexpr int delta_index(int kp) {
    const int d = patch_off(2 * kp + 1) - patch_off(2 * kp);
    return d == delta(0) ? 0 : (d == delta(1) ? 1 : 2);
  }
  static_assert((WN * NT) % 2 == 0, "pixel tile is whole rows of two 32-column segments");
  static_assert(KK % 2 == 0, "chunk reduction length must be even");
  static_assert(BM % 4 == 0, "weight slab rows are float4 multiples");
};

struct ConvEpilogue {
  const float *bias, *slope, *residual, *gate;
  const int32_t *col_limit;
  int npart, act, trim;
  ConvView vres, vgate;
  int d2w;
};


template <int BM, int ROWS, int THREADS>
__device__ __forceinline__ void conv_zero_tile(float *outp, const ConvView &vout, int d2w, int cout0, int cout,
                                               int r0, int c0, int ho, int wo, int tid) {
  for (int e = tid; e < BM * ROWS * kTileCols; e += THREADS) {
    const int col = e % kTileCols, row = (e / kTileCols) % ROWS, co = e / (kTileCols * ROWS);
    if (cout0 + co < cout && r0 + row < ho && c0 + col < wo) {
      const int cg = cout0 + co;
      if (d2w)
        outp[(size_t)(cg >> 2) * vout.cs + (size_t)(2 * (r0 + row) + ((cg >> 1) & 1)) * vout.rs +
             2 * (c0 + col) + (cg & 1)] = 0.f;
      else
        outp[(size_t)cg * vout.cs + (size_t)(r0 + row) * vout.rs + c0 + col] = 0.f;
    }
  }
}

template <int MT, int NT, int WN, int EB = 16>
__device__ __forceinline__ void conv_epilogue(f32x16 (&acc)[MT][NT], const ConvEpilogue &ep, const float *inp,
                                              float *outp, const ConvView &vin, const ConvView &vout, int t, int r0,
                                              int c0, int cout0, int cout, int ho, int wo, int wm, int wn, int l31,
                                              int half, const float *bias_s, const float *slope_s) {
  const int32_t *__restrict__ col_limit = ep.col_limit;
  const int npart = ep.npart, act = ep.act;
  const int trim_at = ((ep.trim || act == 2 || act == 3) && col_limit) ? col_limit[t % npart] : wo;
  const float *resp = ep.residual ? ep.residual + (size_t)t * ep.vres.ts : nullptr;
  const float *gatep = ep.gate ? ep.gate + (size_t)t * ep.vgate.ts : nullptr;
  if (ep.d2w) {
#pragma unroll
    for (int m = 0; m < MT; m++) {
#pragma unroll
      for (int rp = 0; rp < 8; rp++) {
        const int r = 2 * rp;
        const int co = cout0 + (wm * MT + m) * 32 + (r & 3) + 8 * (r >> 2) + 4 * half;
        if (co >= cout) continue;
        const float b0 = bias_s[co - cout0], b1 = bias_s[co - cout0 + 1];
        const float s0 = slope_s[co - cout0], s1 = slope_s[co - cout0 + 1];
        const int cq = co >> 2, sy = (co >> 1) & 1;
#pragma unroll
        for (int n = 0; n < NT; n++) {
          const int seg = wn * NT + n;
          const int orow = r0 + (seg >> 1), ocol = c0 + (seg & 1) * 32 + l31;
          if (orow < ho && ocol < wo) {
            float2 v = make_float2(acc[m][n][r] + b0, acc[m][n][r + 1] + b1);
            if (act == 1) {
              if (v.x < 0) v.x = v.x * s0;
              if (v.y < 0) v.y = v.y * s1;
            }
            *reinterpret_cast<float2 *>(outp + (size_t)cq * vout.cs + (size_t)(2 * orow + sy) * vout.rs + 2 * ocol) = v;
          }
        }
      }
    }
    return;
  }
  static_assert(16 % EB == 0, "epilogue batches are whole fractions of a 32-cout tile");
#pragma unroll
  for (int m = 0; m < MT; m++) {
#pragma unroll
    for (int rb = 0; rb < 16; rb += EB) {
      float rv[EB][NT], q1[EB][NT];
      const bool gdn = act == 2 || act == 3;
      auto batch = [&](float (&dst)[EB][NT], const float *src, const ConvView &v) {
#pragma unroll
        for (int rr = 0; rr < EB; rr++) {
          const int r = rb + rr;
          const int co = cout0 + (wm * MT + m) * 32 + (r & 3) + 8 * (r >> 2) + 4 * half;
#pragma unroll
          for (int n = 0; n < NT; n++) {
            const int seg = wn * NT + n;
            const int orow = r0 + (seg >> 1), ocol = c0 + (seg & 1) * 32 + l31;
            dst[rr][n] = (co < cout && orow < ho && ocol < wo) ? src[(size_t)co * v.cs + (size_t)orow * v.rs + ocol] : 1.f;
          }
        }
      };
      if (resp) batch(rv, resp, ep.vres);
      if (gdn) batch(q1, inp, vin);
      if (gatep) batch(q1, gatep, ep.vgate);
#pragma unroll
      for (int rr = 0; rr < EB; rr++) {
        const int r = rb + rr;
        const int co = cout0 + (wm * MT + m) * 32 + (r & 3) + 8 * (r >> 2) + 4 * half;
        if (co >= cout) continue;
        const float bco = bias_s[co - cout0], sl = slope_s[co - cout0];
#pragma unroll
        for (int n = 0; n < NT; n++) {
          const int seg = wn * NT + n;
          const int orow = r0 + (seg >> 1), ocol = c0 + (seg & 1) * 32 + l31;
          if (orow < ho && ocol < wo) {
            const size_t oi = (size_t)co * vout.cs + (size_t)orow * vout.rs + ocol;
            float v = acc[m][n][r] + bco;
            if (act == 1) {
              if (v < 0) v = v * sl;
            } else if (gdn) {
              const float xv = q1[rr][n];
              const float nrm = sqrtf(v);
              v = act == 2 ? xv / nrm : xv * nrm;
            } else if (act == 4) {
              v = 1.f / (1.f + expf(-v));
            }
            if (gatep) v = q1[rr][n] * v;
            if (resp) v = rv[rr][n] + v;
            if (ocol >= trim_at) v = 0.f;
            outp[oi] = v;
          }
        }
      }
    }
  }
}

template <int MT, int NT, int WN, bool SQ, bool RES>
__device__ __forceinline__ void conv_epilogue_pipe(f32x16 (&acc)[MT][NT], const ConvEpilogue &ep, const float *inp,
                                                   float *outp, const ConvView &vin, const ConvView &vout, int t, int r0,
                                                   int c0, int cout0, int cout, int ho, int wo, int wm, int wn, int l31,
                                                   int half, const float *bias_s, const float *slope_s) {
  const int act = ep.act;
  const int trim_at = ((ep.trim || act == 2 || act == 3) && ep.col_limit) ? ep.col_limit[t % ep.npart] : wo;
  const float *resp = RES ? ep.residual + (size_t)t * ep.vres.ts : nullptr;
  constexpr int NROW = MT * 16, EB = PCONV_PIPE_ROWS(SQ && RES), NB = NROW / EB;
  struct RowIn {
    float r[NT], x[NT];
  };
  auto row_cout = [&](int q) { return cout0 + (wm * MT + (q >> 4)) * 32 + (q & 3) + 8 * ((q & 15) >> 2) + 4 * half; };
  auto request = [&](int q) {
    RowIn v;
    int co = row_cout(q);
    co = co < cout ? co : cout - 1;
#pragma unroll
    for (int n = 0; n < NT; n++) {
      const int seg = wn * NT + n;
      int orow = r0 + (seg >> 1), ocol = c0 + (seg & 1) * 32 + l31;
      orow = orow < ho ? orow : ho - 1;
      ocol = ocol < wo ? ocol : wo - 1;
      v.r[n] = RES ? resp[(size_t)co * ep.vres.cs + (size_t)orow * ep.vres.rs + ocol] : 0.f;
      v.x[n] = SQ ? inp[(size_t)co * vin.cs + (size_t)orow * vin.rs + ocol] : 0.f;
    }
    return v;
  };
  RowIn cur[EB], nxt[EB];
  if (RES || SQ) {
#pragma unroll
    for (int e = 0; e < EB; e++) cur[e] = request(e);
  }
#pragma unroll
  for (int bi = 0; bi < NB; bi++) {
    if ((RES || SQ) && bi + 1 < NB) {
#pragma unroll
      for (int e = 0; e < EB; e++) nxt[e] = request((bi + 1) * EB + e);
    }
#pragma unroll
    for (int e = 0; e < EB; e++) {
      const int q = bi * EB + e, m = q >> 4, r = q & 15;
      const int co = row_cout(q);
      if (co < cout) {
        const float bco = bias_s[co - cout0], sl = slope_s[co - cout0];
#pragma unroll
        for (int n = 0; n < NT; n++) {
          const int seg = wn * NT + n;
          const int orow = r0 + (seg >> 1), ocol = c0 + (seg & 1) * 32 + l31;
          if (orow < ho && ocol < wo) {
            float v = acc[m][n][r] + bco;
            if (SQ) {
              const float xv = cur[e].x[n];
              const float nrm = sqrtf(v);
              v = act == 2 ? xv / nrm : xv * nrm;
            } else if (act == 1) {
              if (v < 0) v = v * sl;
            }
            if (RES) v = cur[e].r[n] + v;
            if (ocol >= trim_at) v = 0.f;
            outp[(size_t)co * vout.cs + (size_t)orow * vout.rs + ocol] = v;
          }
        }
      }
    }
    if ((RES || SQ) && bi + 1 < NB) {
#pragma unroll
      for (int e = 0; e < EB; e++) cur[e] = nxt[e];
    }
  }
}

typedef __attribute__((address_space(3))) void lds_ptr_t;
typedef const __attribute__((address_space(1))) void glb_ptr_t;
typedef const __attribute__((address_space(1))) char glb_bytes_t;

template <int I, int N, class F>
__device__ __forceinline__ void static_for_(F &&f) {
  if constexpr (I < N) {
    f(std::integral_constant<int, I>{});
    static_for_<I + 1, N>(f);
  }
}

__device__ __forceinline__ float4 ld4_base_off(const float *base, unsigned off) {
  asm volatile("" : "+v"(off));
  typedef float v4f __attribute__((ext_vector_type(4)));
  const v4f v = *reinterpret_cast<const __attribute__((address_space(1))) v4f *>((glb_bytes_t *)base + off);
  return make_float4(v.x, v.y, v.z, v.w);
}
__device__ __forceinline__ void st4_base_off(float *base, unsigned off, const float4 &v) {
  asm volatile("" : "+v"(off));
  typedef float v4f __attribute__((ext_vector_type(4)));
  typedef __attribute__((address_space(1))) char glb_char_t;
  const v4f q = {v.x, v.y, v.z, v.w};
  *reinterpret_cast<__attribute__((address_space(1))) v4f *>((glb_char_t *)base + off) = q;
}

template <int MT, int WM, int WN, bool SQ, bool RES>
__device__ __forceinline__ void conv_epilogue_quads(f32x16 (&acc)[MT][1], const ConvEpilogue &ep, const float *in_t,
                                                    float *out_t, const ConvView &vin, const ConvView &vout, int t,
                                                    int r0, int c0, int cout0, int ho, int wo, int wm, int wn, int l31,
                                                    int half, float *park, const float *bias_s, const float *slope_s,
                                                    int tid) {
  constexpr int PX = 32 * WN, QROW = PX / 4, RROWS = 32 * WM, NQR = RROWS * QROW / 512, RSTEP = 512 / QROW;
  static_assert(WM * WN == 8 && RROWS * QROW % 512 == 0 && 32 % RSTEP == 0, "eight waves, whole quads per lane and round");
  const int act = ep.act;
  const int trim_at = ((ep.trim || act == 2 || act == 3) && ep.col_limit) ? ep.col_limit[t % ep.npart] : wo;
  const bool trims = trim_at < c0 + kTileCols;
  const int row0 = tid / QROW, px = (tid % QROW) * 4;
  const int orow_raw = r0 + px / kTileCols, ocol = c0 + px % kTileCols;
  const bool row_ok = orow_raw < ho;
  const int orow = row_ok ? orow_raw : ho - 1;
  auto krow = [](int m, int j) { return ((j * RSTEP) / 32 * MT + m) * 32 + (j * RSTEP) % 32; };
  const unsigned lb_out = (unsigned)(((long long)row0 * vout.cs + (long long)orow * vout.rs + ocol) * 4);
  const unsigned lb_res = RES ? (unsigned)(((long long)row0 * ep.vres.cs + (long long)orow * ep.vres.rs + ocol) * 4) : 0u;
  const unsigned lb_in = (unsigned)(((long long)row0 * vin.cs + (long long)orow * vin.rs + ocol) * 4);
  const float *res_t = RES ? ep.residual + (size_t)t * ep.vres.ts + (size_t)cout0 * ep.vres.cs : nullptr;
  const float *x_t = in_t + (size_t)cout0 * vin.cs;
  float *o_t = out_t + (size_t)cout0 * vout.cs;
  struct QuadIn {
    float4 r, x;
  };
  constexpr int NF = MT * NQR;
  constexpr int D = (SQ && RES) ? PCONV_QUAD_AHEAD_GDN : PCONV_QUAD_AHEAD;
  QuadIn ring[D + 1];
  auto request = [&](auto fc) {
    constexpr int f = decltype(fc)::value, m = f / NQR, j = f % NQR;
    if (RES) ring[f % (D + 1)].r = ld4_base_off(res_t + (size_t)krow(m, j) * ep.vres.cs, lb_res);
    if (SQ) ring[f % (D + 1)].x = ld4_base_off(x_t + (size_t)krow(m, j) * vin.cs, lb_in);
  };
  auto finish = [&](float v, float xv, float rv, float sl, bool trimmed, auto preluc, auto trimc) {
    if (SQ) {
      const float nrm = sqrtf(v);
      v = act == 2 ? xv / nrm : xv * nrm;
    } else if (decltype(preluc)::value) {
      if (v < 0) v = v * sl;
    }
    if (RES) v = rv + v;
    if (decltype(trimc)::value && trimmed) v = 0.f;
    return v;
  };
  auto take_out = [&](auto fc, auto preluc, auto trimc) {
    constexpr int f = decltype(fc)::value, m = f / NQR, j = f % NQR;
    const QuadIn &src = ring[f % (D + 1)];
    const int cb = krow(m, j) + row0;
    const float4 o4 = *reinterpret_cast<const float4 *>(park + (j * RSTEP + row0) * PX + px);
    const float bco = bias_s[cb];
    const float sl = decltype(preluc)::value ? slope_s[cb] : 1.f;
    const float o[4] = {o4.x, o4.y, o4.z, o4.w};
    const float xs[4] = {src.x.x, src.x.y, src.x.z, src.x.w};
    const float rs[4] = {src.r.x, src.r.y, src.r.z, src.r.w};
    float v[4];
#pragma unroll
    for (int k = 0; k < 4; k++) v[k] = finish(o[k] + bco, xs[k], rs[k], sl, ocol + k >= trim_at, preluc, trimc);
    if (row_ok) st4_base_off(o_t + (size_t)krow(m, j) * vout.cs, lb_out, make_float4(v[0], v[1], v[2], v[3]));
  };
  auto whole_tile = [&](auto preluc, auto trimc) {
    if constexpr (RES || SQ) static_for_<0, (D < NF ? D : NF)>([&](auto fc) { request(fc); });
    static_for_<0, MT>([&](auto mc) {
      constexpr int m = decltype(mc)::value;
#pragma unroll
      for (int r = 0; r < 16; r++) park[(wm * 32 + (r & 3) + 8 * (r >> 2) + 4 * half) * PX + wn * 32 + l31] = acc[m][0][r];
      asm volatile("s_waitcnt lgkmcnt(0)\n\ts_barrier" ::: "memory");
      static_for_<0, NQR>([&](auto jc) {
        constexpr int f = m * NQR + decltype(jc)::value;
        if constexpr ((RES || SQ) && f + D < NF) request(std::integral_constant<int, f + D>{});
        take_out(std::integral_constant<int, f>{}, preluc, trimc);
      });
      if constexpr (m + 1 < MT) asm volatile("s_waitcnt lgkmcnt(0)\n\ts_barrier" ::: "memory");
    });
  };
  if (!SQ && act == 1) {
    if (trims)
      whole_tile(std::true_type{}, std::true_type{});
    else
      whole_tile(std::true_type{}, std::false_type{});
  } else {
    if (trims)
      whole_tile(std::false_type{}, std::true_type{});
    else
      whole_tile(std::false_type{}, std::false_type{});
  }
}

template <int MT, int WM, int WN>
__device__ __forceinline__ void conv_epilogue_quads_d2w(f32x16 (&acc)[MT][1], const ConvEpilogue &ep, float *out_t,
                                                        const ConvView &vout, int r0, int c0, int cout0, int wm, int wn,
                                                        int l31, int half, float *park, const float *bias_s,
                                                        const float *slope_s, int tid) {
  constexpr int PX = 32 * WN, PROW = PX / 2, RROWS = 32 * WM, NQR = (RROWS / 2) * PROW / 512, PSTEP = 512 / PROW;
  static_assert(WM * WN == 8 && (RROWS / 2) * PROW % 512 == 0 && 16 % PSTEP == 0, "eight waves, whole quads per lane and round");
  const bool prelu = ep.act == 1;
  const int pair0 = tid / PROW, px = (tid % PROW) * 2;
  const int orow = r0 + px / kTileCols, ocol = c0 + px % kTileCols;
  auto krow = [](int m, int j) { return ((2 * j * PSTEP) / 32 * MT + m) * 32 + (2 * j * PSTEP) % 32; };
#pragma unroll
  for (int m = 0; m < MT; m++) {
#pragma unroll
    for (int r = 0; r < 16; r++) park[(wm * 32 + (r & 3) + 8 * (r >> 2) + 4 * half) * PX + wn * 32 + l31] = acc[m][0][r];
    asm volatile("s_waitcnt lgkmcnt(0)\n\ts_barrier" ::: "memory");
#pragma unroll
    for (int j = 0; j < NQR; j++) {
      const int cb = krow(m, j) + 2 * pair0;
      const float2 a = *reinterpret_cast<const float2 *>(park + (2 * (j * PSTEP + pair0)) * PX + px);
      const float2 b = *reinterpret_cast<const float2 *>(park + (2 * (j * PSTEP + pair0) + 1) * PX + px);
      const float ba = bias_s[cb], bb = bias_s[cb + 1];
      float v[4] = {a.x + ba, b.x + bb, a.y + ba, b.y + bb};
      if (prelu) {
        const float sa = slope_s[cb], sb = slope_s[cb + 1];
        if (v[0] < 0) v[0] = v[0] * sa;
        if (v[1] < 0) v[1] = v[1] * sb;
        if (v[2] < 0) v[2] = v[2] * sa;
        if (v[3] < 0) v[3] = v[3] * sb;
      }
      const int co = cout0 + cb;
      float *dst = out_t + (size_t)(co >> 2) * vout.cs + (size_t)(2 * orow + ((co >> 1) & 1)) * vout.rs + 2 * ocol;
      *reinterpret_cast<float4 *>(dst) = make_float4(v[0], v[1], v[2], v[3]);
    }
    if (m + 1 < MT) asm volatile("s_waitcnt lgkmcnt(0)\n\ts_barrier" ::: "memory");
  }
}

template <class C>
struct ConvStager {
  using P = typename C::P;
  static constexpr int PIECES = C::XLD + C::WLD;
  const float *xb, *wb;
  float *xs, *ws;
  const unsigned (&xoffs)[C::XLD];
  const unsigned (&woffs)[C::WLD];
  int tid, wave, tail;
  long long cs;
  bool active, ragged;

  template <int J>
  __device__ __forceinline__ void issue() const {
    if (!active) return;
    if constexpr (J < C::XLD) {
      const int e = tid + J * C::THREADS;
      if (e < C::XSZ) {
        unsigned off = xoffs[J];
        if (ragged) {
          const int ci = e / (P::PC * P::PR);
          if (ci >= tail) off -= (unsigned)((ci - tail + 1) * cs * 4);
        }
        asm volatile("" : "+v"(off));
        __builtin_amdgcn_global_load_lds((glb_ptr_t *)((glb_bytes_t *)xb + off),
                                         (lds_ptr_t *)(xs + J * C::THREADS + wave * 64), 4, 0, 0);
      }
    } else {
      constexpr int JW = J - C::XLD;
      const int e4 = tid + JW * C::THREADS;
      if (e4 < C::WSZ / 4) {
        unsigned off = woffs[JW];
        asm volatile("" : "+v"(off));
        __builtin_amdgcn_global_load_lds((glb_ptr_t *)((glb_bytes_t *)wb + off),
                                         (lds_ptr_t *)(ws + (JW * C::THREADS + wave * 64) * 4), 16, 0, 0);
      }
    }
  }

  template <int J = 0>
  __device__ __forceinline__ void issue_all() const {
    if constexpr (J < PIECES) {
      issue<J>();
      issue_all<J + 1>();
    }
  }
};

template <int OFF>
__device__ __forceinline__ float lds_read_imm(unsigned addr) {
  static_assert(OFF >= 0 && OFF < 65536, "ds_read offset field is 16 bits");
  float v;
  asm volatile("ds_read_b32 %0, %1 offset:%2" : "=v"(v) : "v"(addr), "n"(OFF));
  return v;
}

template <class C, int KP>
__device__ __forceinline__ void conv_read_pair(float (&A)[C::MTv], float (&B)[C::NTv], unsigned abase,
                                               const unsigned (&bbase)[C::NTv][C::ND]) {
  static_assert(C::MTv <= 3 && C::NTv <= 2, "operand reads are written out for MT <= 3, NT <= 2");
  constexpr int aoff = 2 * KP * C::BM * 4;
  A[0] = lds_read_imm<aoff>(abase);
  if constexpr (C::MTv > 1) A[1] = lds_read_imm<aoff + 128>(abase);
  if constexpr (C::MTv > 2) A[2] = lds_read_imm<aoff + 256>(abase);
  constexpr int boff = C::patch_off(2 * KP) * 4, di = C::delta_index(KP);
  B[0] = lds_read_imm<boff>(bbase[0][di]);
  if constexpr (C::NTv > 1) B[1] = lds_read_imm<boff>(bbase[1][di]);
}

template <int PENDING, int MT, int NT>
__device__ __forceinline__ void conv_wait_pair(float (&A)[MT], float (&B)[NT]) {
  if constexpr (MT == 3 && NT == 1)
    asm volatile("s_waitcnt lgkmcnt(%4)" : "+v"(A[0]), "+v"(A[1]), "+v"(A[2]), "+v"(B[0]) : "n"(PENDING));
  else if constexpr (MT == 1 && NT == 1)
    asm volatile("s_waitcnt lgkmcnt(%2)" : "+v"(A[0]), "+v"(B[0]) : "n"(PENDING));
  else if constexpr (MT == 3 && NT == 2)
    asm volatile("s_waitcnt lgkmcnt(%5)" : "+v"(A[0]), "+v"(A[1]), "+v"(A[2]), "+v"(B[0]), "+v"(B[1]) : "n"(PENDING));
  else
    static_assert(MT == 3 || MT == 1, "conv_wait_pair: unsupported tile");
}

#ifndef PCONV_PREFETCH
#define PCONV_PREFETCH 1
#endif
constexpr int kAhead = PCONV_PREFETCH;

template <class C, bool SQ, int KP>
__device__ __forceinline__ void conv_chunk_step(f32x16 (&acc)[C::MTv][C::NTv], float (&a)[kAhead + 1][C::MTv],
                                                float (&b)[kAhead + 1][C::NTv], unsigned abase,
                                                const unsigned (&bbase)[C::NTv][C::ND]) {
  constexpr int NP = C::KK / 2, SETS = kAhead + 1;
  if constexpr (KP + kAhead < NP)
    conv_read_pair<C, KP + kAhead>(a[(KP + kAhead) % SETS], b[(KP + kAhead) % SETS], abase, bbase);
  constexpr int ahead = (NP - 1 - KP) < kAhead ? (NP - 1 - KP) : kAhead;
  float(&A)[C::MTv] = a[KP % SETS];
  float(&B)[C::NTv] = b[KP % SETS];
  conv_wait_pair<ahead * (C::MTv + C::NTv)>(A, B);
  if (SQ) {
#pragma unroll
    for (int n = 0; n < C::NTv; n++) B[n] = B[n] * B[n];
  }
  __builtin_amdgcn_sched_barrier(0);
#pragma unroll
  for (int m = 0; m < C::MTv; m++)
#pragma unroll
    for (int n = 0; n < C::NTv; n++) acc[m][n] = __builtin_amdgcn_mfma_f32_32x32x2f32(A[m], B[n], acc[m][n], 0, 0, 0);
  __builtin_amdgcn_sched_barrier(0);
  if constexpr (KP + 1 < NP) conv_chunk_step<C, SQ, KP + 1>(acc, a, b, abase, bbase);
}

template <class C, int KP>
__device__ __forceinline__ void conv_chunk_prologue(float (&a)[kAhead + 1][C::MTv], float (&b)[kAhead + 1][C::NTv],
                                                    unsigned abase, const unsigned (&bbase)[C::NTv][C::ND]) {
  if constexpr (KP < kAhead && KP < C::KK / 2) {
    conv_read_pair<C, KP>(a[KP], b[KP], abase, bbase);
    conv_chunk_prologue<C, KP + 1>(a, b, abase, bbase);
  }
}

#ifndef PCONV_1X1_WAVES_EU
#define PCONV_1X1_WAVES_EU 2
#endif
#ifndef PCONV_1X1_EPI_ROWS
#define PCONV_1X1_EPI_ROWS 16
#endif

#ifndef PCONV_QUAD_FALLBACK_ROWS
#define PCONV_QUAD_FALLBACK_ROWS 4
#endif
#ifdef PCONV_CONV_STAMP
__device__ unsigned long long conv_stamps[64][8][6];
#define CONV_STAMP(v) const unsigned long long v = __builtin_readcyclecounter()
#else
#define CONV_STAMP(v)
#endif

template <int MT, int NT, int WM, int WN, int KS, int S, int KC, bool SQ, int WAY = 0>
__global__ __launch_bounds__(64 * WM * WN, (KS == 1 && S == 1 && MT == 3) ? PCONV_1X1_WAVES_EU : 2) void conv_mfma_kernel(
    const float *__restrict__ in, const float *__restrict__ wp, float *__restrict__ out, int cin, int h,
    int w, int cout, int cout_pad, int ho, int wo, int tiles_r, int tiles_c, int cblocks, int xcd_group, ConvView vin,
    ConvView vout, ConvEpilogue ep) {
  const int32_t *__restrict__ col_limit = ep.col_limit;
  const int npart = ep.npart;
  using C = ConvCfg<MT, NT, WM, WN, KS, S, KC>;
  using P = typename C::P;
  constexpr int kThreads = C::THREADS;
  constexpr int kTileRows = C::ROWS;
  extern __shared__ float lds[];
  CONV_STAMP(st0);

  int b = blockIdx.x;
  if (xcd_group > 0) {
    const int full = (int)(gridDim.x / (8u * xcd_group)) * 8 * xcd_group;
    if (b < full) {
      const int x = b & 7, j = b >> 3;
      b = (j / xcd_group) * 8 * xcd_group + x * xcd_group + j % xcd_group;
    }
  }
  const int cb = b % cblocks;
  b /= cblocks;
  const int trx = b % tiles_r;
  b /= tiles_r;
  const int tcx = b % tiles_c;
  const int t = b / tiles_c;
  const int r0 = trx * kTileRows, c0 = tcx * kTileCols;
  const int cout0 = cb * C::BM;

  const int tid = threadIdx.x;
  const int lane = tid & 63;
  const int wave = __builtin_amdgcn_readfirstlane(tid >> 6);
  const int wm = wave / WN, wn = wave % WN;
  const int l31 = lane & 31, half = lane >> 5;

  float *outp = out + (size_t)t * vout.ts;

  if (col_limit && c0 >= col_limit[t % npart]) {
    conv_zero_tile<C::BM, kTileRows, kThreads>(outp, vout, ep.d2w, cout0, cout, r0, c0, ho, wo, tid);
    return;
  }

  const float *inp = in + (size_t)t * vin.ts;
  const int nchunk = (cin + KC - 1) / KC;

  f32x16 acc[MT][NT];
#pragma unroll
  for (int m = 0; m < MT; m++)
#pragma unroll
    for (int n = 0; n < NT; n++)
#pragma unroll
      for (int r = 0; r < 16; r++) acc[m][n][r] = 0.f;

  unsigned xoffs[C::XLD], woffs[C::WLD];
#pragma unroll
  for (int j = 0; j < C::XLD; j++) {
    int e = tid + j * kThreads;
    e = e < C::XSZ ? e : 0;
    const int pc = e % P::PC;
    const int pr = (e / P::PC) % P::PR;
    const int ci = e / (P::PC * P::PR);
    int ir = r0 * S + pr * P::PS;
    int ic = c0 * S + pc * P::PS;
    ir = ir < h ? ir : h - 1;
    ic = ic < w ? ic : w - 1;
    xoffs[j] = (unsigned)((ci * vin.cs + (long long)ir * vin.rs + ic) * 4);
  }
#pragma unroll
  for (int j = 0; j < C::WLD; j++) {
    int e4 = tid + j * kThreads;
    e4 = e4 < C::WSZ / 4 ? e4 : 0;
    const int kk = e4 / (C::BM / 4);
    const int co = (e4 % (C::BM / 4)) * 4;
    woffs[j] = (unsigned)(kk * cout_pad + co) * 4u;
  }
  const int tail = cin % KC;
  const size_t xstep = (size_t)KC * vin.cs, wstep = (size_t)C::KK * cout_pad;

  auto stager = [&](int chunk, int buf) {
    float *xs = lds + buf * C::STAGE;
    return ConvStager<C>{inp + chunk * xstep, wp + chunk * wstep + cout0, xs, xs + C::XSZ, xoffs, woffs, tid, wave, tail,
                         vin.cs, chunk < nchunk, tail != 0 && chunk == nchunk - 1};
  };

  const unsigned lds0 = (unsigned)reinterpret_cast<uintptr_t>(lds);
  unsigned abase = lds0 + (unsigned)(C::XSZ + half * C::BM + wm * MT * 32 + l31) * 4u;
  unsigned bbase[NT][C::ND];
#pragma unroll
  for (int n = 0; n < NT; n++) {
    const int seg = wn * NT + n;
    const int prow = seg >> 1, pcol = (seg & 1) * 32 + l31;
#pragma unroll
    for (int d = 0; d < C::ND; d++)
      bbase[n][d] = lds0 + (unsigned)(prow * P::Q * P::PC + pcol * P::Q + half * C::delta(d)) * 4u;
  }
  static_assert(C::STAGE * 4 <= 65536, "operand offsets of one buffer fit the 16-bit immediate");
  static_assert(kAhead * (MT + NT) <= 15, "lgkmcnt counts to 15");

  float my_bias = 0.f, my_slope = 0.f;
  if (tid < C::BM) {
    const int co = cout0 + tid < cout ? cout0 + tid : cout - 1;
    if (ep.bias) my_bias = ep.bias[co];
    if (ep.act == 1) my_slope = ep.slope[co];
  }

  stager(0, 0).issue_all();
  __syncthreads();
  CONV_STAMP(st1);

  for (int chunk = 0; chunk < nchunk; chunk++) {
    stager(chunk + 1, (chunk & 1) ^ 1).issue_all();
    float a[kAhead + 1][MT], b[kAhead + 1][NT];
    conv_chunk_prologue<C, 0>(a, b, abase, bbase);
    conv_chunk_step<C, SQ, 0>(acc, a, b, abase, bbase);
    const unsigned flip = (chunk & 1) ? (unsigned)(-C::STAGE * 4) : (unsigned)(C::STAGE * 4);
    abase += flip;
#pragma unroll
    for (int n = 0; n < NT; n++)
#pragma unroll
      for (int d = 0; d < C::ND; d++) bbase[n][d] += flip;
    __syncthreads();
  }

  CONV_STAMP(st2);
  static_assert(2 * C::BM <= C::STAGE && C::BM <= kThreads, "bias / slope table fits the stage memory");
  if (tid < C::BM) {
    lds[tid] = my_bias;
    lds[C::BM + tid] = my_slope;
  }
  __syncthreads();
  {
    if constexpr (WAY == 0) {
      conv_epilogue<MT, NT, WN, (KS == 1 && S == 1 && MT == 3) ? PCONV_1X1_EPI_ROWS : 16>(acc, ep, inp, outp, vin, vout, t, r0, c0, cout0,
                                                                                          cout, ho, wo, wm, wn, l31, half, lds, lds + C::BM);
    } else if constexpr (WAY == 5) {
      static_assert(WAY != 5 || (MT == 3 && NT == 1 && kThreads == 512 && !SQ), "d2w quad way out: 96 couts x 32 pixels per wave");
      static_assert(WAY != 5 || (2 * C::BM + 32 * WM * 32 * WN) <= 2 * C::STAGE, "a round fits the stage memory behind the tables");
      if (c0 + kTileCols <= wo && r0 + kTileRows <= ho && cout0 + C::BM <= cout)
        conv_epilogue_quads_d2w<MT, WM, WN>(acc, ep, outp, vout, r0, c0, cout0, wm, wn, l31, half, lds + 2 * C::BM, lds, lds + C::BM, tid);
      else
        conv_epilogue<MT, NT, WN, PCONV_QUAD_FALLBACK_ROWS>(acc, ep, inp, outp, vin, vout, t, r0, c0, cout0, cout, ho, wo, wm, wn, l31, half,
                                                           lds, lds + C::BM);
    } else if constexpr (WAY >= 3) {
      static_assert(WAY < 3 || WAY == 5 || (MT == 3 && NT == 1 && kThreads == 512 && (!SQ || (KS == 1 && S == 1))), "quad way out: 96 couts x 32 pixels per wave, eight waves");
      static_assert(WAY < 3 || WAY == 5 || (2 * C::BM + 32 * WM * 32 * WN) <= 2 * C::STAGE, "a round fits the stage memory behind the tables");
      if (c0 + kTileCols <= wo && cout0 + C::BM <= cout)
        conv_epilogue_quads<MT, WM, WN, SQ, WAY == 4>(acc, ep, inp, outp, vin, vout, t, r0, c0, cout0, ho, wo, wm, wn, l31,
                                                      half, lds + 2 * C::BM, lds, lds + C::BM, tid);
      else
        conv_epilogue<MT, NT, WN, PCONV_QUAD_FALLBACK_ROWS>(acc, ep, inp, outp, vin, vout, t, r0, c0, cout0, cout, ho, wo, wm, wn, l31, half,
                                                           lds, lds + C::BM);
    } else
      conv_epilogue_pipe<MT, NT, WN, SQ, WAY == 2>(acc, ep, inp, outp, vin, vout, t, r0, c0, cout0, cout, ho, wo, wm, wn,
                                                  l31, half, lds, lds + C::BM);
  }
#ifdef PCONV_CONV_STAMP
  {
    asm volatile("s_waitcnt vmcnt(0)" ::: "memory");
    CONV_STAMP(st3);
    const int slot = (int)blockIdx.x - (int)(gridDim.x / 2);
    if (slot >= 0 && slot < 64 && lane == 0) {
      unsigned hw;
      asm volatile("s_getreg_b32 %0, hwreg(HW_REG_HW_ID)" : "=s"(hw));
      unsigned long long *o = conv_stamps[slot][wave & 7];
      o[0] = st0, o[1] = st1, o[2] = st2, o[3] = st3, o[4] = hw, o[5] = blockIdx.x;
    }
  }
#endif
}

typedef const __attribute__((address_space(1))) char global_bytes;
__device__ __forceinline__ float4 load4_base_off(global_bytes *base, unsigned off) {
  asm volatile("" : "+v"(off));
  typedef float v4f __attribute__((ext_vector_type(4)));
  const v4f v = *reinterpret_cast<const __attribute__((address_space(1))) v4f *>(base + off);
  return make_float4(v.x, v.y, v.z, v.w);
}

template <int WM, bool SQ, bool RES>
__global__ __launch_bounds__(512, 2) void conv1x1_rb_kernel(
    const float *__restrict__ in, const float *__restrict__ wp, float *__restrict__ out, int kpad, int h, int w,
    int cout, int cout_pad, int tiles_r, int tiles_c, int cblocks, int passes, int stagger, ConvView vin,
    ConvView vout, ConvEpilogue ep) {
  constexpr int kThreads = 512, MT = 3, NT = 4, BM = 96 * WM, WP = 8 / WM, ROWS = WP / 2, D = 5;
  constexpr int kCols = 256;
  extern __shared__ float lds[];
  int b = blockIdx.x;
  const int cb = b % cblocks;
  b /= cblocks;
  const int trx = b % tiles_r;
  b /= tiles_r;
  const int tcx = b % tiles_c;
  const int t = b / tiles_c;
  const int cout0 = cb * BM;
  const int tid = threadIdx.x, lane = tid & 63, wave = tid >> 6;
  const int wm = wave % WM, wq = wave / WM;
  const int l31 = lane & 31, half = lane >> 5;
  float *outp = out + (size_t)t * vout.ts;
  const float *inp = in + (size_t)t * vin.ts;
  const int gc0 = tcx * kCols + (wq & 1) * 128;
  const int limit = ep.col_limit ? ep.col_limit[t % ep.npart] : w;
  const int dead_at = ep.col_limit ? (limit + 63) / 64 * 64 : w;
  const bool tile_dead = tcx * kCols >= dead_at;
  if (!tile_dead) {
    typedef __attribute__((address_space(3))) void lds_ptr_t;
    typedef const __attribute__((address_space(1))) void glb_ptr_t;
    const int n4 = kpad * BM / 4;
    for (int e4 = tid; e4 < n4; e4 += kThreads) {
      const int kk = e4 / (BM / 4), co = (e4 % (BM / 4)) * 4;
      __builtin_amdgcn_global_load_lds((glb_ptr_t *)(wp + (size_t)kk * cout_pad + cout0 + co),
                                       (lds_ptr_t *)(lds + (size_t)(e4 - lane) * 4), 16, 0, 0);
    }
    if (tid < BM) {
      const int co = cout0 + tid < cout ? cout0 + tid : cout - 1;
      lds[kpad * BM + tid] = ep.bias ? ep.bias[co] : 0.f;
      lds[kpad * BM + BM + tid] = ep.act == 1 ? ep.slope[co] : 1.f;
    }
    __syncthreads();
  }
  const float *bias_s = lds + kpad * BM, *slope_s = bias_s + BM;
  if (gc0 >= w) return;
  const int KP = kpad / 2;
  const size_t kstep = (size_t)2 * vin.cs * sizeof(float);
  const float *wsl = lds + half * BM + wm * 96 + l31;
  const int col = gc0 + 4 * l31 < w - 4 ? gc0 + 4 * l31 : w - 4;
  const bool group_dead = gc0 >= dead_at;
  if (wave >= 4)
    for (int i = 0; i < stagger; i++) __builtin_amdgcn_s_sleep(127);
#pragma unroll 1
  for (int pass = 0; pass < passes; pass++) {
    const int orow = (trx * passes + pass) * ROWS + (wq >> 1);
    if (orow >= h) break;
    int cbase = __builtin_amdgcn_readfirstlane(cout0 + wm * 96);
    asm volatile("" : "+s"(cbase));
    if (group_dead) {
      const int c2 = gc0 + 2 * lane;
#pragma unroll 1
      for (int e = 0; e < 96; e++) {
        const int co = cbase + e;
        if (co >= cout) break;
        for (int j = 0; j < 2; j++) {
          if (c2 + j >= w) continue;
          outp[(size_t)co * vout.cs + (size_t)orow * vout.rs + c2 + j] = 0.f;
        }
      }
      continue;
    }
    const unsigned loff = (unsigned)(((long long)half * vin.cs + (long long)orow * vin.rs + col) * sizeof(float));
    const unsigned long long in_u = reinterpret_cast<unsigned long long>(inp);
    global_bytes *bbase = reinterpret_cast<global_bytes *>(
        ((unsigned long long)(unsigned)__builtin_amdgcn_readfirstlane((unsigned)(in_u >> 32)) << 32) |
        (unsigned long long)(unsigned)__builtin_amdgcn_readfirstlane((unsigned)in_u));
    f32x16 acc[MT][NT];
#pragma unroll
    for (int m = 0; m < MT; m++)
#pragma unroll
      for (int n = 0; n < NT; n++)
#pragma unroll
        for (int r = 0; r < 16; r++) acc[m][n][r] = 0.f;
    float4 bq[D];
    float a[2][MT];
#pragma unroll
    for (int j = 0; j < D; j++) bq[j] = load4_base_off(bbase + (size_t)(j < KP ? j : KP - 1) * kstep, loff);
#pragma unroll
    for (int m = 0; m < MT; m++) a[0][m] = wsl[m * 32];
    constexpr int U = (D % 2) ? 2 * D : D;
#pragma unroll 1
    for (int kp0 = 0; kp0 < KP; kp0 += U) {
#pragma unroll
      for (int j = 0; j < U; j++) {
        const int kp = kp0 + j;
        if (kp < KP) {
          float4 bv = bq[j % D];
          const int kpre = kp + D < KP ? kp + D : KP - 1;
          bq[j % D] = load4_base_off(bbase + (size_t)kpre * kstep, loff);
          const int knext = kp + 1 < KP ? kp + 1 : KP - 1;
#pragma unroll
          for (int m = 0; m < MT; m++) a[(j + 1) & 1][m] = wsl[(size_t)knext * 2 * BM + m * 32];
          if (SQ) {
            bv.x *= bv.x;
            bv.y *= bv.y;
            bv.z *= bv.z;
            bv.w *= bv.w;
          }
          __builtin_amdgcn_sched_barrier(0);
#pragma unroll
          for (int m = 0; m < MT; m++) {
            acc[m][0] = __builtin_amdgcn_mfma_f32_32x32x2f32(a[j & 1][m], bv.x, acc[m][0], 0, 0, 0);
            acc[m][1] = __builtin_amdgcn_mfma_f32_32x32x2f32(a[j & 1][m], bv.y, acc[m][1], 0, 0, 0);
            acc[m][2] = __builtin_amdgcn_mfma_f32_32x32x2f32(a[j & 1][m], bv.z, acc[m][2], 0, 0, 0);
            acc[m][3] = __builtin_amdgcn_mfma_f32_32x32x2f32(a[j & 1][m], bv.w, acc[m][3], 0, 0, 0);
          }
          __builtin_amdgcn_sched_barrier(0);
        }
      }
    }
    const int act = ep.act;
    const int trim_at = ((ep.trim || act == 2 || act == 3) && ep.col_limit) ? limit : dead_at;
    const float *resp = RES ? ep.residual + (size_t)t * ep.vres.ts : nullptr;
    constexpr int NROW = MT * 16, EB = (SQ && RES) ? 1 : 4, NB = NROW / EB;
    struct RowIn {
      float4 r, x;
    };
    auto row_cout = [&](int q) { return cbase + (q >> 4) * 32 + (q & 3) + 8 * ((q & 15) >> 2) + 4 * half; };
    auto request = [&](int q) {
      RowIn v = {make_float4(0.f, 0.f, 0.f, 0.f), make_float4(0.f, 0.f, 0.f, 0.f)};
      int co = row_cout(q);
      co = co < cout ? co : cout - 1;
      if (RES) v.r = *reinterpret_cast<const float4 *>(resp + (size_t)co * ep.vres.cs + (size_t)orow * ep.vres.rs + col);
      if (SQ) v.x = *reinterpret_cast<const float4 *>(inp + (size_t)co * vin.cs + (size_t)orow * vin.rs + col);
      return v;
    };
    RowIn cur[EB], nxt[EB];
    if (RES || SQ) {
#pragma unroll
      for (int e = 0; e < EB; e++) cur[e] = request(e);
    }
#pragma unroll
    for (int bi = 0; bi < NB; bi++) {
      if ((RES || SQ) && bi + 1 < NB) {
#pragma unroll
        for (int e = 0; e < EB; e++) nxt[e] = request((bi + 1) * EB + e);
      }
#pragma unroll
      for (int e = 0; e < EB; e++) {
        const int q = bi * EB + e, m = q >> 4, r = q & 15;
        const int co = row_cout(q);
        if (co < cout) {
          const float bco = bias_s[co - cout0], sl = slope_s[co - cout0];
          float v[4] = {acc[m][0][r] + bco, acc[m][1][r] + bco, acc[m][2][r] + bco, acc[m][3][r] + bco};
          if (SQ) {
            const float xs[4] = {cur[e].x.x, cur[e].x.y, cur[e].x.z, cur[e].x.w};
#pragma unroll
            for (int j = 0; j < 4; j++) {
              const float nrm = sqrtf(v[j]);
              v[j] = act == 2 ? xs[j] / nrm : xs[j] * nrm;
            }
          } else {
#pragma unroll
            for (int j = 0; j < 4; j++)
              if (v[j] < 0) v[j] = v[j] * sl;
          }
          if (RES) {
            v[0] = cur[e].r.x + v[0];
            v[1] = cur[e].r.y + v[1];
            v[2] = cur[e].r.z + v[2];
            v[3] = cur[e].r.w + v[3];
          }
#pragma unroll
          for (int j = 0; j < 4; j++)
            if (col + j >= trim_at) v[j] = 0.f;
          *reinterpret_cast<float4 *>(outp + (size_t)co * vout.cs + (size_t)orow * vout.rs + col) =
              make_float4(v[0], v[1], v[2], v[3]);
        }
      }
      if ((RES || SQ) && bi + 1 < NB) {
#pragma unroll
        for (int e = 0; e < EB; e++) cur[e] = nxt[e];
      }
    }
  }
}

template <int WM, bool SQ, bool RES>
int launch_conv1x1(const float *in, const float *wp, float *out, int tn, int cin, int h, int w, int cout,
                   int cout_pad, const ConvView &vin, const ConvView &vout, const ConvEpilogue &ep,
                   const ConvOptions &opt, hipStream_t stream) {
  constexpr int BM = 96 * WM, ROWS = (8 / WM) / 2;
  const int kpad = (cin + 15) / 16 * 16;
  const int tiles_c = (w + 255) / 256;
  const int cblocks = (cout + BM - 1) / BM;
  const long long single = (long long)tn * ((h + ROWS - 1) / ROWS) * tiles_c * cblocks;
  const int passes = single >= 4096 ? 4 : (single >= 2048 ? 2 : 1);
  const int tiles_r = (h + ROWS * passes - 1) / (ROWS * passes);
  const long long grid = (long long)tn * tiles_r * tiles_c * cblocks;
  if (grid <= 0 || grid > 0x7fffffffLL) {
    pconv_set_error("conv2d: grid %lld out of range", grid);
    return PCONV_EINVAL;
  }
  const size_t smem = ((size_t)kpad * BM + 2 * BM) * sizeof(float);
  auto kern = conv1x1_rb_kernel<WM, SQ, RES>;
  if (smem > 64 * 1024) {
    static std::atomic<unsigned long long> raised{0};
    if (int rc = pconv_raise_lds(kern, smem, raised, "conv2d")) return rc;
  }
  const int stagger = opt.stagger >= 0 ? opt.stagger : 0;
  hipLaunchKernelGGL(kern, dim3((unsigned)grid), dim3(512), smem, stream, in, wp, out, kpad, h, w, cout, cout_pad,
                     tiles_r, tiles_c, cblocks, passes, stagger, vin, vout, ep);
  return PCONV_OK;
}

inline bool use_resident_1x1(const ConvOptions &opt, int cin, int cout, int tn, int h, int w) {
  if (opt.conv1x1 == 1) return false;
  const int kpad = (cin + 15) / 16 * 16;
  const int bm = cout > 96 ? 192 : 96;
  if (!(cin >= 32 && cin % 16 == 0 && cout > 32 && ((size_t)kpad * bm + 2 * bm) * sizeof(float) <= 160 * 1024)) return false;
  if (w < 4) return false;
  if (opt.conv1x1 == 2) return true;
  (void)tn, (void)h;
  return false;
}

template <int KS, int KC>
__global__ __launch_bounds__(512, 2) void conv_small_kernel(const float *__restrict__ in, const float *__restrict__ wp,
                                                            float *__restrict__ out, int cin, int h, int w, int cout,
                                                            int cout_pad, int ho, int wo, int tiles_r, int tiles_c,
                                                            ConvView vin, ConvView vout, ConvEpilogue ep) {
  static_assert(KS == 3, "small-cout kernel: 3x3 stride 1");
  constexpr int ROWS = 8, PR = ROWS + KS - 1, PC = kTileCols + KS - 1, KK = KC * KS * KS, NS = KK / 4;
  constexpr int XSZ = KC * PR * PC, WSZ = KK * 16, STAGE = XSZ + WSZ, kThreads = 512;
  constexpr int XLD = (XSZ + kThreads - 1) / kThreads;
  static_assert(KK % 4 == 0 && KK * 4 <= kThreads && (2 * STAGE) * 4 + 256 < 65536, "immediate offsets reach both buffers");
  __shared__ __attribute__((aligned(16))) float lds[2 * STAGE];
  int b = blockIdx.x;
  const int trx = b % tiles_r;
  b /= tiles_r;
  const int tcx = b % tiles_c;
  const int t = b / tiles_c;
  const int r0 = trx * ROWS, c0 = tcx * kTileCols;
  const int tid = threadIdx.x, lane = tid & 63;
  const int wave = __builtin_amdgcn_readfirstlane(tid >> 6);
  const int r = lane & 15, q = lane >> 4;
  float *outp = out + (size_t)t * vout.ts;
  if (ep.col_limit && c0 >= ep.col_limit[t % ep.npart]) {
    conv_zero_tile<16, ROWS, kThreads>(outp, vout, ep.d2w, 0, cout, r0, c0, ho, wo, tid);
    return;
  }
  const float *inp = in + (size_t)t * vin.ts;
  const int nchunk = (cin + KC - 1) / KC, tail = cin % KC;
  unsigned xoffs[XLD];
#pragma unroll
  for (int j = 0; j < XLD; j++) {
    int e = tid + j * kThreads;
    e = e < XSZ ? e : 0;
    const int pc = e % PC, pr = (e / PC) % PR, ci = e / (PC * PR);
    int ir = r0 + pr, ic = c0 + pc;
    ir = ir < h ? ir : h - 1;
    ic = ic < w ? ic : w - 1;
    xoffs[j] = (unsigned)((ci * vin.cs + (long long)ir * vin.rs + ic) * 4);
  }
  const int we4 = tid < KK * 4 ? tid : 0;
  const unsigned woff = (unsigned)(((we4 >> 2) * cout_pad + (we4 & 3) * 4) * 4);
  const size_t xstep = (size_t)KC * vin.cs, wstep = (size_t)KK * cout_pad;
  auto stage = [&](int chunk, int buf) {
    if (chunk >= nchunk) return;
    float *xs = lds + buf * STAGE;
    const float *xb = inp + chunk * xstep;
    const bool ragged = tail != 0 && chunk == nchunk - 1;
#pragma unroll
    for (int j = 0; j < XLD; j++) {
      const int e = tid + j * kThreads;
      if (e < XSZ) {
        unsigned off = xoffs[j];
        if (ragged) {
          const int ci = e / (PC * PR);
          if (ci >= tail) off -= (unsigned)((ci - tail + 1) * vin.cs * 4);
        }
        asm volatile("" : "+v"(off));
        __builtin_amdgcn_global_load_lds((glb_ptr_t *)((glb_bytes_t *)xb + off), (lds_ptr_t *)(xs + j * kThreads + wave * 64), 4, 0,
                                         0);
      }
    }
    if (tid < KK * 4) {
      unsigned off = woff;
      asm volatile("" : "+v"(off));
      __builtin_amdgcn_global_load_lds((glb_ptr_t *)((glb_bytes_t *)(wp + chunk * wstep) + off),
                                       (lds_ptr_t *)(xs + XSZ + wave * 64 * 4), 16, 0, 0);
    }
  };
  int boff[NS];
#pragma unroll
  for (int s4 = 0; s4 < NS; s4++) {
    const int k = 4 * s4 + q;
    boff[s4] = (k / (KS * KS)) * PR * PC + ((k / KS) % KS) * PC + k % KS + wave * PC + r;
  }
  const int aoff = XSZ + q * 16 + r;
  typedef float f32x4 __attribute__((ext_vector_type(4)));
  f32x4 acc[4];
#pragma unroll
  for (int n = 0; n < 4; n++) acc[n] = f32x4{0.f, 0.f, 0.f, 0.f};
  const unsigned lds0 = (unsigned)reinterpret_cast<uintptr_t>(lds);
  const unsigned abase = lds0 + (unsigned)aoff * 4u;
  unsigned bbase[NS];
#pragma unroll
  for (int s4 = 0; s4 < NS; s4++) bbase[s4] = lds0 + (unsigned)boff[s4] * 4u;
  auto chunk_body = [&](auto bufc) {
    constexpr int BO = decltype(bufc)::value * STAGE * 4;
    float a[2], bq[2][4];
    a[0] = lds_read_imm<BO>(abase);
    static_for_<0, 4>([&](auto nc) { bq[0][decltype(nc)::value] = lds_read_imm<BO + 64 * decltype(nc)::value>(bbase[0]); });
    static_for_<0, NS>([&](auto sc) {
      constexpr int S4 = decltype(sc)::value;
      if constexpr (S4 + 1 < NS) {
        a[(S4 + 1) & 1] = lds_read_imm<BO + (S4 + 1) * 256>(abase);
        static_for_<0, 4>([&](auto nc) {
          bq[(S4 + 1) & 1][decltype(nc)::value] = lds_read_imm<BO + 64 * decltype(nc)::value>(bbase[S4 + 1]);
        });
      }
      float &A = a[S4 & 1];
      float(&B)[4] = bq[S4 & 1];
      asm volatile("s_waitcnt lgkmcnt(%5)" : "+v"(A), "+v"(B[0]), "+v"(B[1]), "+v"(B[2]), "+v"(B[3]) : "n"(S4 + 1 < NS ? 5 : 0));
      __builtin_amdgcn_sched_barrier(0);
#pragma unroll
      for (int n = 0; n < 4; n++) acc[n] = __builtin_amdgcn_mfma_f32_16x16x4f32(A, B[n], acc[n], 0, 0, 0);
      __builtin_amdgcn_sched_barrier(0);
    });
  };
  stage(0, 0);
  __syncthreads();
  for (int chunk = 0; chunk < nchunk; chunk += 2) {
    stage(chunk + 1, 1);
    chunk_body(std::integral_constant<int, 0>{});
    __syncthreads();
    if (chunk + 1 >= nchunk) break;
    stage(chunk + 2, 0);
    chunk_body(std::integral_constant<int, 1>{});
    __syncthreads();
  }
  const int orow = r0 + wave;
  if (orow >= ho) return;
  const int act = ep.act;
  const int trim_at = (ep.trim && ep.col_limit) ? ep.col_limit[t % ep.npart] : wo;
  float bco[4], sl[4];
#pragma unroll
  for (int i = 0; i < 4; i++) {
    const int co = 4 * q + i < cout ? 4 * q + i : cout - 1;
    bco[i] = ep.bias ? ep.bias[co] : 0.f;
    sl[i] = act == 1 ? ep.slope[co] : 1.f;
  }
#pragma unroll
  for (int n = 0; n < 4; n++) {
    const int ocol = c0 + 16 * n + r;
    if (ocol >= wo) continue;
    float v[4];
#pragma unroll
    for (int i = 0; i < 4; i++) {
      v[i] = acc[n][i] + bco[i];
      if (act == 1 && v[i] < 0) v[i] = v[i] * sl[i];
    }
    if (ep.d2w) {
      if (4 * q + 3 < cout) {
#pragma unroll
        for (int sy = 0; sy < 2; sy++)
          *reinterpret_cast<float2 *>(outp + (size_t)q * vout.cs + (size_t)(2 * orow + sy) * vout.rs + 2 * ocol) =
              make_float2(v[2 * sy], v[2 * sy + 1]);
      }
    } else {
#pragma unroll
      for (int i = 0; i < 4; i++)
        if (4 * q + i < cout) outp[(size_t)(4 * q + i) * vout.cs + (size_t)orow * vout.rs + ocol] = ocol >= trim_at ? 0.f : v[i];
    }
  }
}

inline bool use_small_cout(const ConvOptions &opt) { return opt.small_cout != 0; }

int launch_conv_small(const float *in, const float *wp, float *out, int tn, int cin, int h, int w, int cout, int cout_pad,
                      int ho, int wo, const ConvView &vin, const ConvView &vout, const ConvEpilogue &ep, hipStream_t stream) {
  const int tiles_r = (ho + 7) / 8, tiles_c = (wo + kTileCols - 1) / kTileCols;
  const long long grid = (long long)tn * tiles_r * tiles_c;
  if (grid <= 0 || grid > 0x7fffffffLL) {
    pconv_set_error("conv2d: grid %lld out of range", grid);
    return PCONV_EINVAL;
  }
  hipLaunchKernelGGL((conv_small_kernel<3, 4>), dim3((unsigned)grid), dim3(512), 0, stream, in, wp, out, cin, h, w, cout,
                     cout_pad, ho, wo, tiles_r, tiles_c, vin, vout, ep);
  return PCONV_OK;
}

#ifdef PCONV_CONV_STAMP
extern "C" int pconv_conv_read_stamps(unsigned long long *out) {
  return hipMemcpyFromSymbol(out, HIP_SYMBOL(conv_stamps), sizeof(conv_stamps)) == hipSuccess ? 0 : 1;
}
#endif

inline bool pipe_way_out(const ConvOptions &opt) { return opt.wayout != 2; }
inline bool quad_way_out(const ConvOptions &opt) { return opt.wayout == 0; }

__global__ void pack_weight_kernel(const float *__restrict__ w, float *__restrict__ packed, int cout,
                                   int red, int cout_pad, int red_pad) {
  const int i = blockIdx.x * blockDim.x + threadIdx.x;
  if (i >= cout_pad * red_pad) return;
  const int co = i % cout_pad, kk = i / cout_pad;
  packed[i] = (co < cout && kk < red) ? w[(size_t)co * red + kk] : 0.f;
}

template <int MT, int NT, int WM, int WN, int KS, int S, int KC, bool SQ = false, int WAY = 0>
int launch_conv(const float *in, const float *wp, float *out, int tn, int cin, int h, int w, int cout,
                int cout_pad, int ho, int wo, const ConvView &vin, const ConvView &vout, const ConvEpilogue &ep,
                const ConvOptions &opt, hipStream_t stream) {
  using C = ConvCfg<MT, NT, WM, WN, KS, S, KC>;
  constexpr int kThreads = C::THREADS;
  constexpr int kTileRows = C::ROWS;
  const int tiles_r = (ho + kTileRows - 1) / kTileRows;
  const int tiles_c = (wo + kTileCols - 1) / kTileCols;
  const int cblocks = (cout + C::BM - 1) / C::BM;
  const long long grid = (long long)tn * tiles_r * tiles_c * cblocks;
  if (grid <= 0 || grid > 0x7fffffffLL) {
    pconv_set_error("conv2d: grid %lld out of range", grid);
    return PCONV_EINVAL;
  }
  const size_t smem = (size_t)2 * C::STAGE * sizeof(float);
  auto kern = conv_mfma_kernel<MT, NT, WM, WN, KS, S, KC, SQ, WAY>;
  if (smem > 64 * 1024) {
    static std::atomic<unsigned long long> raised{0};
    if (int rc = pconv_raise_lds(kern, smem, raised, "conv2d")) return rc;
  }
  const int xcd_group = (opt.xcd == 1 && KS == 3) ? cblocks * tiles_r : 0;
  hipLaunchKernelGGL(kern, dim3((unsigned)grid), dim3(kThreads), smem, stream, in, wp, out, cin, h, w, cout,
                     cout_pad, ho, wo, tiles_r, tiles_c, cblocks, xcd_group, vin, vout, ep);
  return PCONV_OK;
}

template <int KS, int S, int KC, class... Args>
int launch_by_tile(int cout, const Args &...args) {
  if (cout > 96) return launch_conv<3, 1, 2, 4, KS, S, KC>(args...);
  if (cout > 32) return launch_conv<3, 1, 1, 8, KS, S, KC>(args...);
  return launch_conv<1, 1, 1, 4, KS, S, KC>(args...);
}

int run_pack(const char *what, const float *w, float *packed, int cout, int cin, int k, void *stream) {
  PCONV_REQUIRE(w && packed, "%s: null pointer", what);
  int cp, rp;
  const long long total = pconv_conv_packed_floats(cout, cin, k, &cp, &rp);
  PCONV_REQUIRE(total <= 0x7fffffffLL, "%s: weight exceeds int32", what);
  hipLaunchKernelGGL(pack_weight_kernel, dim3(((int)total + 255) / 256), dim3(256), 0, as_stream(stream), w, packed, cout,
                     cin * k * k, cp, rp);
  PCONV_LAUNCH_CHECK(what);
  return PCONV_OK;
}

}

long long pconv_conv_packed_floats(int cout, int cin, int k, int *cout_pad, int *red_pad) {
  const int tile = cout > 96 ? 192 : (cout > 32 ? 96 : 32);
  const int kc = k == 1 ? PCONV_KC1 : (k == 5 ? kKC5 : 4);
  const long long cp = ((long long)cout + tile - 1) / tile * tile, rp = ((long long)cin + kc - 1) / kc * kc * k * k;
  if (cout_pad) *cout_pad = (int)cp;
  if (red_pad) *red_pad = (int)rp;
  return cp * rp;
}

extern "C" int pconv_conv_packed_size(int cout, int cin, int k, int *cout_pad, int *red_pad) {
  return (int)pconv_conv_packed_floats(cout, cin, k, cout_pad, red_pad);
}

extern "C" int pconv_conv_pack_weight(const float *w, float *packed, int cout, int cin, int k,
                                      void *stream) {
  PCONV_REQUIRE(cout > 0 && cin > 0 && (k == 1 || k == 3), "conv_pack_weight: bad argument");
  return run_pack("conv_pack_weight", w, packed, cout, cin, k, stream);
}

extern "C" int pconv_conv2d(const float *in, const float *packed_w, const float *bias, float *out,
                            int tn, int cin, int h, int w, int cout, int k, int stride, int act,
                            const float *slope, const int32_t *col_limit, int npart,
                            const float *residual, const float *gate, int trim, int d2w,
                            const long long *views, void *stream) {
  PCONV_REQUIRE(in && packed_w && out, "conv2d: null pointer");
  PCONV_REQUIRE(!d2w || (cout % 4 == 0 && act <= 1 && !residual && !gate && !trim),
                "conv2d: depth-to-width needs cout %% 4 == 0 and takes no sigmoid / gate / residual / trim");
  PCONV_REQUIRE((k == 1 || k == 3) && (stride == 1 || stride == 2), "conv2d: k=%d stride=%d unsupported",
                k, stride);
  PCONV_REQUIRE(h >= k && w >= k && tn > 0 && cin > 0 && cout > 0, "conv2d: bad shape");
  PCONV_REQUIRE(act == 0 || (act == 1 && slope) || act == 4, "conv2d: bad activation %d", act);
  PCONV_REQUIRE(!col_limit || npart > 0, "conv2d: col_limit needs npart");
  PCONV_REQUIRE(!trim || col_limit, "conv2d: trim needs col_limit");
  PCONV_REQUIRE(residual != out && gate != out, "conv2d: residual / gate must not alias the output");
  const int ho = (h - k) / stride + 1, wo = (w - k) / stride + 1;
  int cp, rp;
  pconv_conv_packed_size(cout, cin, k, &cp, &rp);
  hipStream_t s = as_stream(stream);
  const ConvOptions opt = ConvOptions::from_env();
  const int oc = d2w ? cout / 4 : cout, oh = d2w ? 2 * ho : ho, ow = d2w ? 2 * wo : wo;
  const ConvView vin = view_at(views, 0, cin, h, w), vout = view_at(views, 1, oc, oh, ow);
  const ConvEpilogue ep = {bias,  slope, residual, gate, col_limit, npart, act, trim,
                           view_at(views, 2, cout, ho, wo), view_at(views, 3, cout, ho, wo), d2w};
  PCONV_REQUIRE(!d2w || view_aligned8(vout, out), "conv2d: depth-to-width output must be 8-byte aligned row by row");
  PCONV_REQUIRE(view_ok(vin, cin, h, w) && view_ok(vout, oc, oh, ow) &&
                    (!residual || view_ok(ep.vres, cout, ho, wo)) && (!gate || view_ok(ep.vgate, cout, ho, wo)),
                "conv2d: strides overlap");
  PCONV_REQUIRE(((long long)(16 - 1) * vin.cs + (long long)(h - 1) * vin.rs + w) * 4 < (1LL << 32),
                "conv2d: input channel stride too large for 32-bit byte offsets inside a chunk");
  PCONV_REQUIRE(((long long)(32 - 1) * vout.cs + (long long)(oh - 1) * vout.rs + ow) * 4 < (1LL << 32) &&
                    (!residual || ((long long)(32 - 1) * ep.vres.cs + (long long)(ho - 1) * ep.vres.rs + wo) * 4 < (1LL << 32)),
                "conv2d: output / residual channel stride too large for 32-bit byte offsets inside a round");
  int rc;
#define ARGS in, packed_w, out, tn, cin, h, w, cout, cp, ho, wo, vin, vout, ep, opt, s
  if (k == 3 && stride == 1 && cout <= 16 && !residual && !gate && act != 4 && (!d2w || cout % 4 == 0) && use_small_cout(opt)) {
    rc = launch_conv_small(in, packed_w, out, tn, cin, h, w, cout, cp, ho, wo, vin, vout, ep, s);
  } else if (k == 3 && stride == 1) {
    rc = launch_by_tile<3, 1, 4>(cout, ARGS);
  } else if (k == 3 && stride == 2 && cout > 32 && !gate && !d2w && act != 4 && quad_way_out(opt)) {
    if (cout > 96)
      rc = residual ? launch_conv<3, 1, 2, 4, 3, 2, 4, false, 4>(ARGS) : launch_conv<3, 1, 2, 4, 3, 2, 4, false, 3>(ARGS);
    else
      rc = residual ? launch_conv<3, 1, 1, 8, 3, 2, 4, false, 4>(ARGS) : launch_conv<3, 1, 1, 8, 3, 2, 4, false, 3>(ARGS);
  } else if (k == 3 && stride == 2) {
    rc = launch_by_tile<3, 2, 4>(cout, ARGS);
  } else if (k == 1 && stride == 1 && !gate && !d2w && act != 4 && use_resident_1x1(opt, cin, cout, tn, h, w)) {
    if (cout > 96 && residual)
      rc = launch_conv1x1<2, false, true>(in, packed_w, out, tn, cin, h, w, cout, cp, vin, vout, ep, opt, s);
    else if (cout > 96)
      rc = launch_conv1x1<2, false, false>(in, packed_w, out, tn, cin, h, w, cout, cp, vin, vout, ep, opt, s);
    else if (residual)
      rc = launch_conv1x1<1, false, true>(in, packed_w, out, tn, cin, h, w, cout, cp, vin, vout, ep, opt, s);
    else
      rc = launch_conv1x1<1, false, false>(in, packed_w, out, tn, cin, h, w, cout, cp, vin, vout, ep, opt, s);
  } else if (k == 1 && stride == 1 && d2w && cout > 32 && quad_way_out(opt)) {
    if (cout > 96)
      rc = launch_conv<3, 1, 2, 4, 1, 1, PCONV_KC1, false, 5>(ARGS);
    else
      rc = launch_conv<3, 1, 1, 8, 1, 1, PCONV_KC1, false, 5>(ARGS);
  } else if (k == 1 && stride == 1 && !gate && !d2w && act != 4 && cout > 32 && quad_way_out(opt)) {
    if (cout > 96)
      rc = residual ? launch_conv<3, 1, 2, 4, 1, 1, PCONV_KC1, false, 4>(ARGS) : launch_conv<3, 1, 2, 4, 1, 1, PCONV_KC1, false, 3>(ARGS);
    else
      rc = residual ? launch_conv<3, 1, 1, 8, 1, 1, PCONV_KC1, false, 4>(ARGS) : launch_conv<3, 1, 1, 8, 1, 1, PCONV_KC1, false, 3>(ARGS);
  } else if (k == 1 && stride == 1 && !gate && !d2w && act != 4 && residual && pipe_way_out(opt)) {
    if (cout > 96)
      rc = launch_conv<3, 1, 2, 4, 1, 1, PCONV_KC1, false, 2>(ARGS);
    else if (cout > 32)
      rc = launch_conv<3, 1, 1, 8, 1, 1, PCONV_KC1, false, 2>(ARGS);
    else
      rc = launch_conv<1, 1, 1, 4, 1, 1, PCONV_KC1, false, 2>(ARGS);
  } else if (k == 1 && stride == 1) {
    rc = launch_by_tile<1, 1, PCONV_KC1>(cout, ARGS);
  } else if (cout > 32 && !gate && !d2w && act != 4 && quad_way_out(opt)) {
    if (cout > 96)
      rc = residual ? launch_conv<3, 1, 2, 4, 1, 2, PCONV_KC1, false, 4>(ARGS) : launch_conv<3, 1, 2, 4, 1, 2, PCONV_KC1, false, 3>(ARGS);
    else
      rc = residual ? launch_conv<3, 1, 1, 8, 1, 2, PCONV_KC1, false, 4>(ARGS) : launch_conv<3, 1, 1, 8, 1, 2, PCONV_KC1, false, 3>(ARGS);
  } else {
    rc = launch_by_tile<1, 2, PCONV_KC1>(cout, ARGS);
  }
#undef ARGS
  if (rc != PCONV_OK) return rc;
  PCONV_LAUNCH_CHECK("conv2d");
  return PCONV_OK;
}

constexpr int kK5 = 5;

extern "C" int pconv_conv5_packed_size(int cout, int cin, int *cout_pad, int *red_pad) {
  PCONV_REQUIRE(cout > 0 && cin > 0, "conv5_packed_size: bad shape");
  const long long total = pconv_conv_packed_floats(cout, cin, kK5, cout_pad, red_pad);
  PCONV_REQUIRE(total <= 0x7fffffffLL, "conv5_packed_size: weight exceeds int32");
  return (int)total;
}

extern "C" int pconv_conv5_pack_weight(const float *w, float *packed, int cout, int cin, void *stream) {
  PCONV_REQUIRE(cout > 0 && cin > 0, "conv5_pack_weight: bad shape");
  return run_pack("conv5_pack_weight", w, packed, cout, cin, kK5, stream);
}

extern "C" int pconv_conv5(const float *in, const float *packed_w, const float *bias, float *out, int tn, int cin, int h,
                           int w, int cout, void *stream) {
  PCONV_REQUIRE(in && packed_w && out, "conv5: null pointer");
  PCONV_REQUIRE(tn > 0 && cin > 0 && cout > 0 && h >= 5 && w >= 5, "conv5: bad shape (%d, %d, %d, %d) -> %d: h and w >= 5", tn,
                cin, h, w, cout);
  int cp, rp;
  PCONV_REQUIRE(pconv_conv5_packed_size(cout, cin, &cp, &rp) > 0 && (long long)h * w <= 0x7fffffffLL &&
                    (long long)tn * cin <= 0x7fffffffLL && (long long)tn * cout <= 0x7fffffffLL,
                "conv5: shape exceeds int32");
  PCONV_REQUIRE((reinterpret_cast<uintptr_t>(packed_w) & 15) == 0, "conv5: the packed weight must be 16-byte aligned");
  const int ho = h - 4, wo = w - 4;
  const ConvView vin = dense_view(cin, h, w), vout = dense_view(cout, ho, wo);
  PCONV_REQUIRE(((long long)(kKC5 - 1) * vin.cs + (long long)(h - 1) * vin.rs + w) * 4 < (1LL << 32),
                "conv5: plane too large for 32-bit byte offsets inside a chunk");
  const ConvEpilogue ep = {bias, nullptr, nullptr, nullptr, nullptr, 0, 0, 0, vout, vout, 0};
  const ConvOptions opt = ConvOptions::from_env();
  hipStream_t s = as_stream(stream);
  if (int rc = launch_by_tile<kK5, 1, kKC5>(cout, in, packed_w, out, tn, cin, h, w, cout, cp, ho, wo, vin, vout, ep, opt, s))
    return rc;
  PCONV_LAUNCH_CHECK("conv5");
  return PCONV_OK;
}

extern "C" int pconv_gdn(const float *in, const float *packed_gamma, const float *beta, float *out, int tn,
                         int ch, int h, int w, int inverse, const int32_t *col_limit, int npart,
                         const float *residual, const long long *views, void *stream) {
  PCONV_REQUIRE(in && packed_gamma && beta && out && in != out && residual != out, "gdn: bad pointer");
  PCONV_REQUIRE(tn > 0 && ch > 0 && h > 0 && w > 0, "gdn: bad shape");
  PCONV_REQUIRE(!col_limit || npart > 0, "gdn: col_limit needs npart");
  int cp, rp;
  pconv_conv_packed_size(ch, ch, 1, &cp, &rp);
  hipStream_t s = as_stream(stream);
  const ConvOptions opt = ConvOptions::from_env();
  const ConvView vin = view_at(views, 0, ch, h, w), vout = view_at(views, 1, ch, h, w);
  const ConvEpilogue ep = {beta, nullptr, residual, nullptr, col_limit, npart, inverse ? 3 : 2, 1,
                           view_at(views, 2, ch, h, w), dense_view(ch, h, w), 0};
  PCONV_REQUIRE(view_ok(vin, ch, h, w) && view_ok(vout, ch, h, w) && (!residual || view_ok(ep.vres, ch, h, w)),
                "gdn: strides overlap");
  int rc;
  if (use_resident_1x1(opt, ch, ch, tn, h, w) && ch > 96 && residual)
    rc = launch_conv1x1<2, true, true>(in, packed_gamma, out, tn, ch, h, w, ch, cp, vin, vout, ep, opt, s);
  else if (use_resident_1x1(opt, ch, ch, tn, h, w) && ch > 96)
    rc = launch_conv1x1<2, true, false>(in, packed_gamma, out, tn, ch, h, w, ch, cp, vin, vout, ep, opt, s);
  else if (use_resident_1x1(opt, ch, ch, tn, h, w) && residual)
    rc = launch_conv1x1<1, true, true>(in, packed_gamma, out, tn, ch, h, w, ch, cp, vin, vout, ep, opt, s);
  else if (use_resident_1x1(opt, ch, ch, tn, h, w))
    rc = launch_conv1x1<1, true, false>(in, packed_gamma, out, tn, ch, h, w, ch, cp, vin, vout, ep, opt, s);
  else if (quad_way_out(opt) && ch > 96)
    rc = residual ? launch_conv<3, 1, 2, 4, 1, 1, PCONV_KC1, true, 4>(in, packed_gamma, out, tn, ch, h, w, ch, cp, h, w, vin, vout, ep, opt, s)
                  : launch_conv<3, 1, 2, 4, 1, 1, PCONV_KC1, true, 3>(in, packed_gamma, out, tn, ch, h, w, ch, cp, h, w, vin, vout, ep, opt, s);
  else if (pipe_way_out(opt) && ch > 96 && residual)
    rc = launch_conv<3, 1, 2, 4, 1, 1, PCONV_KC1, true, 2>(in, packed_gamma, out, tn, ch, h, w, ch, cp, h, w, vin, vout, ep, opt, s);
  else if (pipe_way_out(opt) && ch > 96)
    rc = launch_conv<3, 1, 2, 4, 1, 1, PCONV_KC1, true, 1>(in, packed_gamma, out, tn, ch, h, w, ch, cp, h, w, vin, vout, ep, opt, s);
  else if (ch > 96)
    rc = launch_conv<3, 1, 2, 4, 1, 1, PCONV_KC1, true>(in, packed_gamma, out, tn, ch, h, w, ch, cp, h, w, vin, vout, ep, opt, s);
  else if (ch > 32)
    rc = launch_conv<3, 1, 1, 8, 1, 1, PCONV_KC1, true>(in, packed_gamma, out, tn, ch, h, w, ch, cp, h, w, vin, vout, ep, opt, s);
  else
    rc = launch_conv<1, 1, 1, 4, 1, 1, PCONV_KC1, true>(in, packed_gamma, out, tn, ch, h, w, ch, cp, h, w, vin, vout, ep, opt, s);
  if (rc != PCONV_OK) return rc;
  PCONV_LAUNCH_CHECK("gdn");
  return PCONV_OK;
}
```

pseudocylindrical_convolution_amd/model_zoo_v2.py:

```python
import os

import torch
from torch import nn

from .PCONV_operator import (ContextReshape, DropGrad, Dtow, EntropyGmm, Extract, MaskConv2, PseudoContextV2,
                             PseudoEntropyContext, PseudoEntropyPad, PseudoFillV2, PseudoGDNV2, PseudoPadV2,
                             PseudoQUANTV2, SphereSlice, SphereUslice, StubMask, TileConvCall, backend)

__all__ = ["ClipData", "TileConv2d", "ResidualBlock", "AttentionBlock", "ResidualBlockV2", "ResidualBlockDown",
           "SphereConv2", "EncoderV2", "ResidualBlockUp", "SphereConvOld", "DecoderV2", "EntropyConv",
           "EntropyResidualBlock", "EntropySubNet", "EntropyNet", "CMPNetV2MF", "CMPNetV2M", "CMPNetV2MFExtractor",
           "CMPNetV2Decoder", "CMPNetV2MFEntropy", "AccGrad"]


class _LeakyClip(torch.autograd.Function):

    @staticmethod
    def forward(ctx, x):
        ops = backend.ops()
        if x.is_cuda and not ctx.needs_input_grad[0] and hasattr(ops, "leaky_clip_"):
            return ops.leaky_clip_(x.detach().clone().contiguous())
        below, above = x < 0, x > 1
        y = x.clone().detach()
        y[below] = x[below] * 0.01
        y[above] = 1 + (x[above] - 1) * 0.01
        ctx.save_for_backward(below, above)
        return y

    @staticmethod
    def backward(ctx, grad_output):
        below, above = ctx.saved_tensors
        g = grad_output.clone().detach()
        g[below] = grad_output[below] * 0.01
        g[above] = grad_output[above] * 0.01
        return g


class ClipData(nn.Module):

    def forward(self, x):
        return _LeakyClip.apply(x)


class TileConv2d(nn.Conv2d):

    def _native(self, x, prelu=None, live=None, sigmoid=False, gate=None, residual=None, trim=None, ring=0,
                d2w=None):
        ops = backend.ops()
        slope = prelu.weight if prelu is not None else None
        vendor = not hasattr(ops, "tile_conv2d")
        native_grad = False
        if torch.is_grad_enabled() and (x.requires_grad or self.weight.requires_grad):
            vendor, live = True, None
            native_grad = hasattr(ops, "tile_conv2d_backward") and ops.conv_grad_is_native()
        fused = (not vendor) and getattr(ops, "FUSED_EPILOGUE", False)
        limit, npart = None, 0
        if live is not None and hasattr(ops, "conv_col_limit") and os.environ.get("PCONV_SKIP_DEAD", "1") == "1":
            ctx, base = live
            k, s = self.kernel_size[0], self.stride[0]
            wo = (x.shape[3] - k) // s + 1
            limit, npart = ops.conv_col_limit(ctx.native(x), x.shape[2], base, wo - base, x)
            if trim is not None and wo != base:
                raise ValueError("trim on an output that still carries halo columns")
        if fused and (trim is None or limit is not None):
            return ops.tile_conv2d(self, x, self.weight, self.bias, self.stride[0], slope, limit, npart,
                                   sigmoid=sigmoid, gate=gate, residual=residual, trim=trim is not None,
                                   ring=ring, d2w=d2w is not None)
        if vendor:
            if native_grad:
                y = TileConvCall.apply(self, x, self.weight, self.bias, self.stride[0])
            else:
                y = nn.functional.conv2d(x, self.weight, self.bias, self.stride)
            y = nn.functional.prelu(y, slope) if slope is not None else y
        else:
            y = ops.tile_conv2d(self, x, self.weight, self.bias, self.stride[0], slope, limit, npart)
        if sigmoid:
            y = torch.sigmoid(y)
        if gate is not None:
            y = gate * y
        if residual is not None:
            y = residual + y
        if d2w is not None:
            y = d2w(y)
        return trim(y) if trim is not None else y

    def forward(self, x, live=None, **epilogue):
        return self._native(x, None, live, **epilogue)

    def fuse(self, x, prelu, live=None, **epilogue):
        return self._native(x, prelu, live, **epilogue)


RING = 2 if os.environ.get("PCONV_PAD_RING", "1") == "1" else 0


def _conv(cin, cout, k, stride=1):
    return TileConv2d(cin, cout, k, stride)


class ResidualBlock(nn.Module):

    def __init__(self, channels, npart, ctx, device_id=0):
        super(ResidualBlock, self).__init__()
        mid = channels // 2
        self.pad = PseudoPadV2(1, npart, ctx, device=device_id)
        self.conv1 = _conv(channels, mid, 1)
        self.relu1 = nn.PReLU(mid)
        self.conv2 = _conv(mid, mid, 3)
        self.relu2 = nn.PReLU(mid)
        self.conv3 = _conv(mid, channels, 1)
        self.trim = PseudoFillV2(0, npart, ctx, device=device_id)
        self.__dict__["ctx"] = ctx

    def forward(self, x):
        live = (self.ctx, x.shape[3])
        y = self.conv1.fuse(self.pad(x), self.relu1, live)
        y = self.conv2.fuse(y, self.relu2, live)
        return self.conv3(y, live, residual=x, trim=self.trim, ring=RING)


class AttentionBlock(nn.Module):

    def __init__(self, channels, npart, ctx, device_id=0):
        super(AttentionBlock, self).__init__()
        block = lambda: ResidualBlock(channels, npart, ctx, device_id)
        self.trunk = nn.Sequential(block(), block(), block())
        self.attention = nn.Sequential(block(), block(), block(), _conv(channels, channels, 1), nn.Sigmoid())
        self.trim = PseudoFillV2(0, npart, ctx, device=device_id)
        self.__dict__["ctx"] = ctx

    def forward(self, x):
        a = x
        for m in self.attention[:3]:
            a = m(a)
        return self.attention[3](a, (self.ctx, x.shape[3]), sigmoid=True, gate=self.trunk(x), residual=x,
                                 trim=self.trim, ring=RING)


class ResidualBlockV2(nn.Module):

    def __init__(self, channels, npart, ctx, device_id):
        super(ResidualBlockV2, self).__init__()
        self.pad = PseudoPadV2(2, npart, ctx, device=device_id)
        self.conv1 = _conv(channels, channels, 3)
        self.relu1 = nn.PReLU(channels)
        self.conv2 = _conv(channels, channels, 3)
        self.relu2 = nn.PReLU(channels)
        self.trim = PseudoFillV2(0, npart, ctx, device=device_id)
        self.__dict__["ctx"] = ctx

    def forward(self, x):
        live = (self.ctx, x.shape[3])
        y = self.conv1.fuse(self.pad(x), self.relu1, live)
        return self.conv2.fuse(y, self.relu2, live, residual=x, trim=self.trim, ring=RING)


class ResidualBlockDown(nn.Module):

    def __init__(self, channels, channel_in, npart, ctx, device_id):
        super(ResidualBlockDown, self).__init__()
        self.pad1 = PseudoPadV2(1, npart, ctx, device=device_id)
        self.conv1 = _conv(channel_in, channels, 3, 2)
        self.relu1 = nn.PReLU(channels)
        self.pad2 = PseudoPadV2(1, npart, ctx, device=device_id)
        self.conv2 = _conv(channels, channels, 3)
        self.relu2 = PseudoGDNV2(channels, npart, ctx, device_id)
        self.short_cut = _conv(channel_in, channels, 1, 2)
        self.trim = PseudoFillV2(0, npart, ctx, device=device_id)
        self.__dict__["ctx"] = ctx

    def forward(self, x):
        live = (self.ctx, x.shape[3] // 2)
        t = self.short_cut(x, live)
        y = self.conv1.fuse(self.pad1(x), self.relu1, live, ring=RING)
        return self.relu2(self.conv2(self.pad2(y), live), residual=t, trim=self.trim, ring=RING)


class SphereConv2(nn.Module):

    def __init__(self, channel_in, channel_out, npart, ctx, device_id=0):
        super(SphereConv2, self).__init__()
        self.conv = _conv(channel_in, channel_out, 3, 2)
        self.pad = PseudoPadV2(1, npart, ctx, device=device_id)
        self.trim = PseudoFillV2(0, npart, ctx, device=device_id)
        self.__dict__["ctx"] = ctx

    def forward(self, x):
        return self.conv(self.pad(x), (self.ctx, x.shape[3] // 2), trim=self.trim, ring=RING)


class EncoderV2(nn.Module):

    def __init__(self, channels, code_channels, npart, ctx, device_id):
        super(EncoderV2, self).__init__()
        down = lambda cin: ResidualBlockDown(channels, cin, npart, ctx, device_id)
        res = lambda: ResidualBlockV2(channels, npart, ctx, device_id)
        att = lambda: AttentionBlock(channels, npart, ctx, device_id)
        self.net = nn.Sequential(
            down(3), res(), down(channels), att(), res(), down(channels), res(),
            SphereConv2(channels, channels, npart, ctx, device_id), att(),
            _conv(channels, code_channels, 1),
        )
        self.act = nn.Sigmoid()
        self.trim = PseudoFillV2(0, npart, ctx, device=device_id)
        self.__dict__["ctx"] = ctx
        backend.watch_state_dict(self)

    def forward(self, x):
        return self.forward_range(x, 0, len(self.net))

    def forward_range(self, x, lo, hi):
        last = len(self.net) - 1
        for m in self.net[lo:min(hi, last)]:
            x = m(x)
        if lo <= last < hi:
            x = self.net[-1](x, (self.ctx, x.shape[3]), sigmoid=True, trim=self.trim)
        return x


class ResidualBlockUp(nn.Module):

    def __init__(self, channels, npart, ctx, device_id):
        super(ResidualBlockUp, self).__init__()
        self.pad1 = PseudoPadV2(1, npart, ctx, device=device_id)
        self.conv1 = _conv(channels, channels * 4, 3)
        self.relu1 = nn.PReLU(channels * 4)
        self.dtow1 = Dtow(2, True, device_id)
        self.pad2 = PseudoPadV2(1, npart, ctx, device=device_id)
        self.conv2 = _conv(channels, channels, 3)
        self.relu2 = PseudoGDNV2(channels, npart, ctx, device_id, inverse=True)
        self.short_cut = _conv(channels, channels * 4, 1)
        self.dtow2 = Dtow(2, True, device_id)
        self.trim = PseudoFillV2(0, npart, ctx, device=device_id)
        self.__dict__["ctx"] = ctx

    def forward(self, x):
        w = x.shape[3]
        br1 = self.conv1.fuse(self.pad1(x), self.relu1, (self.ctx, w), d2w=self.dtow1, ring=RING)
        br2 = self.short_cut(x, (self.ctx, w), d2w=self.dtow2)
        return self.relu2(self.conv2(self.pad2(br1), (self.ctx, 2 * w)), residual=br2, trim=self.trim, ring=RING)


class SphereConvOld(nn.Module):

    def __init__(self, npart, channel_in, channel_out, ctx, device_id=0):
        super(SphereConvOld, self).__init__()
        self.conv = _conv(channel_in, channel_out, 1)
        self.trim = PseudoFillV2(0, npart, ctx, device=device_id)
        self.__dict__["ctx"] = ctx

    def forward(self, x):
        return self.conv(x, (self.ctx, x.shape[3]), trim=self.trim, ring=RING)


class DecoderV2(nn.Module):

    def __init__(self, channels, code_channels, npart, ctx, device_id):
        super(DecoderV2, self).__init__()
        up = lambda: ResidualBlockUp(channels, npart, ctx, device_id)
        res = lambda: ResidualBlockV2(channels, npart, ctx, device_id)
        att = lambda: AttentionBlock(channels, npart, ctx, device_id)
        self.net = nn.Sequential(
            SphereConvOld(npart, code_channels, channels, ctx, device_id),
            att(), res(), up(), res(), up(), att(), res(), up(), res(),
            PseudoPadV2(1, npart, ctx, device=device_id),
            _conv(channels, 12, 3),
            Dtow(2, True, device_id),
        )
        self.__dict__["ctx"] = ctx
        backend.watch_state_dict(self)

    def forward(self, x):
        return self.forward_range(x, 0, len(self.net))

    def forward_range(self, x, lo, hi):
        mods = list(self.net)
        body = len(mods) - 2
        for m in mods[lo:min(hi, body)]:
            x = m(x)
        if lo <= body < hi:
            x = mods[-2](x, (self.ctx, x.shape[3] - 2), d2w=mods[-1])
        return x


class EntropyConv(nn.Module):

    def __init__(self, ngroups, cin, cout, hidden, npart, ctx, device_id, act=True):
        super(EntropyConv, self).__init__()
        self.pad = PseudoEntropyPad(2, npart, ctx, device=device_id)
        self.conv = MaskConv2(ngroups, cin, cout, 5, hidden, device_id)
        self.trim = PseudoFillV2(0, npart, ctx, device=device_id)
        self.act = nn.PReLU(ngroups * cout) if act else None

    def forward(self, x):
        y = self.conv(self.pad(x))
        if self.act is not None:
            y = self.act(y)
        return self.trim(y)


class EntropyResidualBlock(nn.Module):

    def __init__(self, ngroups, cpn, npart, ctx, device_id=0):
        super(EntropyResidualBlock, self).__init__()
        self.conv1 = EntropyConv(ngroups, cpn, cpn, True, npart, ctx, device_id, True)
        self.conv2 = EntropyConv(ngroups, cpn, cpn, True, npart, ctx, device_id, True)

    def forward(self, x):
        return self.conv2(self.conv1(x)) + x


class EntropySubNet(nn.Module):

    def __init__(self, ngroups, cpn, npart, num_gaussian, net_type, ctx, device_id):
        super(EntropySubNet, self).__init__()
        block = lambda: EntropyResidualBlock(ngroups, cpn, npart, ctx, device_id)
        self.net = nn.Sequential(
            EntropyConv(ngroups, 1, cpn, False, npart, ctx, device_id),
            block(), block(), block(), block(), block(),
            EntropyConv(ngroups, cpn, num_gaussian, True, npart, ctx, device_id, False),
        )
        self.reshape = ContextReshape(ngroups, device_id)
        self.act = None
        if net_type == 0:
            self.act = nn.Softmax(dim=1)
        elif net_type == 2:
            self.act = nn.ReLU()
            self.net[6].conv.bias.data.fill_(2)

    def forward(self, x):
        y = self.reshape(self.net(x))
        return self.act(y) if self.act is not None else y


class EntropyNet(nn.Module):

    def __init__(self, ngroups, npart, ctx, cpn=3, num_gaussian=3, device_id=0, drop_flag=False):
        super(EntropyNet, self).__init__()
        self.drop = DropGrad(drop_flag)
        self.weight_net = EntropySubNet(ngroups, cpn, npart, num_gaussian, 0, ctx, device_id)
        self.mean_net = EntropySubNet(ngroups, cpn, npart, num_gaussian, 1, ctx, device_id)
        self.delta_net = EntropySubNet(ngroups, cpn, npart, num_gaussian, 2, ctx, device_id)
        self.mask = None
        self.fill = PseudoFillV2(0, npart, ctx, device=device_id)
        self.fill2 = PseudoFillV2(0, npart, ctx, device=device_id)
        self.ent_loss = EntropyGmm(num_gaussian, device=device_id)

    def setup_mask(self, x):
        with torch.no_grad():
            self.mask = self.fill(torch.ones_like(x).detach()).view(-1)

    def forward(self, x):
        self.setup_mask(x)
        x = self.drop(self.fill2(x))
        weight = self.weight_net(x)
        mean = self.mean_net(x)
        delta = self.delta_net(x) + 1e-6
        loss_vec = self.ent_loss(weight, delta, mean, x.view(-1, 1))
        return loss_vec * self.mask, self.mask


class CMPNetV2MF(nn.Module):

    def __init__(self, valid_dim=162, channels=192, code_channels=192, npart=16, quant_levels=8, opt=False,
                 init=False, device_id=0):
        super(CMPNetV2MF, self).__init__()
        self.slice = SphereSlice(npart, pad=0, opt=opt, device=device_id)
        self.uslice = SphereUslice(npart, pad=0, opt=opt, device=device_id)
        self.ctx = PseudoContextV2(npart, opt, device=device_id)
        self.ctx_ent = PseudoEntropyContext(npart, 1, opt, device=device_id)
        self.encoder = EncoderV2(channels, code_channels, npart, self.ctx, device_id)
        self.decoder = DecoderV2(channels, code_channels, npart, self.ctx, device_id)
        self.quant = PseudoQUANTV2(code_channels, quant_levels, npart, self.ctx, top_alpha=0.0001,
                                   device_id=device_id, ntop=2)
        self.vm = StubMask(valid_dim)
        self.ext = Extract(valid_dim)
        self.clip = ClipData()
        self.ent = EntropyNet(valid_dim // 4, npart, self.ctx_ent, 3, 3, device_id, drop_flag=init)
        self.mean_val = (quant_levels - 1) / 2.
        self.dtw = Dtow(2, True, device_id)

    def forward(self, x):
        code = self.encoder(self.slice(x))
        code_f, code_i = self.quant(code)
        code_f = code_f * self.vm(code_f)
        y = self.uslice(self.decoder(code_f))
        symbols = self.dtw(self.ext(code_i)) - self.mean_val
        ent_vec, mask = self.ent(symbols)
        return self.clip(y), ent_vec, mask


class CMPNetV2M(nn.Module):

    def __init__(self, valid_dim=162, channels=192, code_channels=192, npart=16, quant_levels=8, opt=False,
                 init=False, device_id=0):
        super(CMPNetV2M, self).__init__()
        self.slice = SphereSlice(npart, pad=0, opt=opt, device=device_id)
        self.uslice = SphereUslice(npart, pad=0, opt=opt, device=device_id)
        self.ctx = PseudoContextV2(npart, opt, device=device_id)
        self.encoder = EncoderV2(channels, code_channels, npart, self.ctx, device_id)
        self.decoder = DecoderV2(channels, code_channels, npart, self.ctx, device_id)
        self.quant = PseudoQUANTV2(code_channels, quant_levels, npart, self.ctx, top_alpha=0.0001,
                                   device_id=device_id, ntop=2)
        self.vm = StubMask(valid_dim)
        self.clip = ClipData()

    def forward(self, x):
        code_f, _ = self.quant(self.encoder(self.slice(x)))
        code_f = code_f * self.vm(code_f)
        return self.clip(self.uslice(self.decoder(code_f)))


class CMPNetV2MFExtractor(nn.Module):

    def __init__(self, valid_dim=162, channels=192, code_channels=192, npart=16, quant_levels=8, opt=False,
                 init=False, device_id=0):
        super(CMPNetV2MFExtractor, self).__init__()
        self.slice = SphereSlice(npart, pad=0, opt=opt, device=device_id)
        self.ctx = PseudoContextV2(npart, opt, device=device_id)
        self.encoder = EncoderV2(channels, code_channels, npart, self.ctx, device_id)
        self.quant = PseudoQUANTV2(code_channels, quant_levels, npart, self.ctx, top_alpha=0.0001,
                                   device_id=device_id, ntop=2)
        self.ext = Extract(valid_dim)
        self.mean_val = (quant_levels - 1) / 2.
        self.dtw = Dtow(2, True, device_id)

    def forward(self, x):
        _, code_i = self.quant(self.encoder(self.slice(x)))
        return self.dtw(self.ext(code_i))


class CMPNetV2Decoder(nn.Module):

    def __init__(self, channels=192, code_channels=192, npart=16, opt=False, init=False, device_id=0):
        super(CMPNetV2Decoder, self).__init__()
        self.uslice = SphereUslice(npart, pad=0, opt=opt, device=device_id)
        self.ctx = PseudoContextV2(npart, opt, device=device_id)
        self.decoder = DecoderV2(channels, code_channels, npart, self.ctx, device_id)
        self.clip = ClipData()

    def forward(self, x):
        return self.clip(self.uslice(self.decoder(x)))


class CMPNetV2MFEntropy(nn.Module):

    def __init__(self, valid_dim=162, channels=192, code_channels=192, npart=16, quant_levels=8, opt=False,
                 init=False, device_id=0):
        super(CMPNetV2MFEntropy, self).__init__()
        self.ctx = PseudoEntropyContext(npart, 1, opt, device=device_id)
        self.ent = EntropyNet(valid_dim // 4, npart, self.ctx, 3, 3, device_id, drop_flag=init)
        self.mean_val = (quant_levels - 1) / 2.

    def forward(self, x):
        return self.ent(x - self.mean_val)


class AccGrad():

    def __init__(self, params):
        self.acc_grad = [torch.zeros_like(p, memory_format=torch.preserve_format) for p in list(params)]
        self.num_param = len(self.acc_grad)

    def zero(self):
        for g in self.acc_grad:
            g.zero_()

    def acc(self, params):
        torch._foreach_add_(self.acc_grad, [p.grad for p in list(params)])

    def copy_back(self, param):
        torch._foreach_add_([p.grad for p in list(param)], self.acc_grad)
        self.zero()
```

Baseline: 95.27 MPix/s.

## Fuse stride-2 1x1 shortcut conv into GDN kernel epilogue for downsampling blocks

Adds a GDN kernel variant that also computes the stride-2 1x1 shortcut convolution as a second GEMM in the same launch. The shortcut result is added in the epilogue instead of being written to memory and read back as a residual. This removes one kernel launch and the round trip of the shortcut tensor through global memory in ResidualBlockDown. In exchange the kernel needs more registers and LDS (a second accumulator set and a second park buffer) and runs at different occupancy. By default it is enabled only for the shapes listed as measured (ch 192 with particular widths).

```diff
diff --git a/include/pconv_hip.h b/include/pconv_hip.h
--- a/include/pconv_hip.h
+++ b/include/pconv_hip.h
@@ -315,6 +315,13 @@
               const float *residual ,
               const long long *views ,
               void *stream);
+
+#define PCONV_SHORTCUT_DOWN 1
+int pconv_gdn_shortcut_takes(int mode, int ch, int sc_cin, int tn, int h, int w);
+int pconv_gdn_shortcut(const float *in, const float *packed_gamma, const float *beta, float *out,
+                       int tn, int ch, int h, int w, int inverse, const int32_t *col_limit, int npart,
+                       int mode, const float *sc_in, const float *sc_packed_w, const float *sc_bias,
+                       int sc_cin, int sc_h, int sc_w, const long long *views, void *stream);
 
 
 int pconv_dinput2(const float *packed, float *ctx, const int32_t *order, int lo, int len,
diff --git a/pseudocylindrical_convolution_amd/PCONV.py b/pseudocylindrical_convolution_amd/PCONV.py
--- a/pseudocylindrical_convolution_amd/PCONV.py
+++ b/pseudocylindrical_convolution_amd/PCONV.py
@@ -1842,12 +1842,45 @@
     return out
 
 
-def tile_gdn(owner, x, gamma, beta, inverse, col_limit=None, npart=0, residual=None, ring=0):
+GDN_SHORTCUT_DOWN = 1
+
+
+def gdn_shortcut_takes(conv, x, gdn_shape):
+    tn, ch, h, w = gdn_shape
+    if conv.kernel_size != (1, 1) or conv.stride != (2, 2) or conv.out_channels != ch or x.dim() != 4 or \
+            x.shape[0] != tn or ((x.shape[2] - 1) // 2 + 1, (x.shape[3] - 1) // 2 + 1) != (h, w):
+        return 0
+    return int(_native.hip_lib().pconv_gdn_shortcut_takes(GDN_SHORTCUT_DOWN, ch, conv.in_channels, tn, h, w))
+
+
+def tile_gdn(owner, x, gamma, beta, inverse, col_limit=None, npart=0, residual=None, ring=0, shortcut=None):
     x = _require_rows(x, "tile_gdn")
     tn, ch, h, w = x.shape
     stream = _stream(x.device)
     packed = packed_conv_weight(owner, gamma.view(ch, ch, 1, 1), stream)
     out = _ring_output((tn, ch, h, w), ring, x)
+    if shortcut is not None:
+        if residual is not None:
+            raise PconvError("tile_gdn: a shortcut stands where the residual stands: give one of them")
+        conv, xs = shortcut
+        xs = _require_rows(xs, "tile_gdn: shortcut input")
+        cin, hs, ws = xs.shape[1:]
+        if tuple(conv.weight.shape) != (ch, cin, 1, 1) or xs.shape[0] != tn or xs.device != x.device:
+            raise PconvError("tile_gdn: shortcut weight %s / input %s do not fit %s"
+                             % (tuple(conv.weight.shape), tuple(xs.shape), tuple(x.shape)))
+        views = _views(x, out, xs)
+
+        def describe_fused():
+            return (conv_kernel_name(ch, 1, 1, True, cin=ch, pixels=tn * h * w)[:-1] + ", 3, 1>", "GDN+sc %d w%d" % (ch, w),
+                    2.0 * ch * (ch + cin) * tn * h * w * _VALID_FRACTION,
+                    4.0 * tn * _VALID_FRACTION * (2 * ch * h * w + cin * hs * ws))
+
+        with _ConvTimed(x.device, describe_fused):
+            call("pconv_gdn_shortcut", _ptr(x), _ptr(packed), _ptr(beta.detach().contiguous()), _ptr(out), tn, ch, h, w,
+                 1 if inverse else 0, _ptr(col_limit), int(npart), GDN_SHORTCUT_DOWN, _ptr(xs),
+                 _ptr(_packed_weight(conv, conv.weight, "direct", stream)),
+                 _ptr(conv.bias.detach()) if conv.bias is not None else None, cin, hs, ws, ctypes.addressof(views), stream)
+        return out
     residual = _like_output(residual, out, "tile_gdn: residual")
     views = _views(x, out, residual)
 
diff --git a/pseudocylindrical_convolution_amd/PCONV_operator/ops.py b/pseudocylindrical_convolution_amd/PCONV_operator/ops.py
--- a/pseudocylindrical_convolution_amd/PCONV_operator/ops.py
+++ b/pseudocylindrical_convolution_amd/PCONV_operator/ops.py
@@ -175,13 +175,19 @@
             self._effective = (key, gamma.contiguous(), beta.contiguous())
         return self._effective[1], self._effective[2]
 
-    def forward(self, inputs, residual=None, trim=None, ring=0):
+    def fuses(self, inputs):
+        return hasattr(backend.ops(), "tile_gdn") and inputs.is_cuda and not torch.is_grad_enabled()
+
+    def forward(self, inputs, residual=None, trim=None, ring=0, shortcut=None):
         ops = backend.ops()
-        if hasattr(ops, "tile_gdn") and inputs.is_cuda and not torch.is_grad_enabled():
+        if self.fuses(inputs):
             gamma, beta = self.effective()
             ctx_op = self.ctx.native(inputs)
             limit, npart = ops.conv_col_limit(ctx_op, inputs.shape[2], inputs.shape[3], 0, inputs)
-            return ops.tile_gdn(self, inputs, gamma, beta, self.inverse, limit, npart, residual, ring)
+            return ops.tile_gdn(self, inputs, gamma, beta, self.inverse, limit, npart, residual, ring,
+                                **({} if shortcut is None else {"shortcut": shortcut}))
+        if shortcut is not None:
+            raise ValueError("PseudoGDNV2: a shortcut needs the fused launch (fuses(inputs))")
         out = self._formula(inputs)
         if residual is not None:
             out = residual + out
diff --git a/pseudocylindrical_convolution_amd/_native.py b/pseudocylindrical_convolution_amd/_native.py
--- a/pseudocylindrical_convolution_amd/_native.py
+++ b/pseudocylindrical_convolution_amd/_native.py
@@ -117,6 +117,8 @@
     "pconv_conv5_wgrad_workspace_bytes": [I, I, I],
     "pconv_conv5_wgrad": [P, P, P, P, P, I, I, I, I, I, P],
     "pconv_gdn": [P, P, P, P, I, I, I, I, I, P, I, P, P, P],
+    "pconv_gdn_shortcut_takes": [I, I, I, I, I, I],
+    "pconv_gdn_shortcut": [P, P, P, P, I, I, I, I, I, P, I, I, P, P, P, I, I, I, P, P],
     "pconv_wino_packed_size": [I, I],
     "pconv_wino_pack_weight": [P, P, I, I, P],
     "pconv_wino_supported": [I, I, I, I, I],
diff --git a/pseudocylindrical_convolution_amd/csrc/conv.hip b/pseudocylindrical_convolution_amd/csrc/conv.hip
--- a/pseudocylindrical_convolution_amd/csrc/conv.hip
+++ b/pseudocylindrical_convolution_amd/csrc/conv.hip
@@ -42,7 +42,7 @@
   static constexpr int STAGE = XSZ + WSZ;
   static constexpr int XLD = (XSZ + THREADS - 1) / THREADS;
   static constexpr int WLD = (WSZ / 4 + THREADS - 1) / THREADS;
-  static constexpr int MTv = MT, NTv = NT, KSv = KS;
+  static constexpr int MTv = MT, NTv = NT, KSv = KS, KCv = KC, Sv = S;
   static constexpr int patch_off(int k) {
     return (k / (KS * KS)) * P::PR * P::PC + ((k / KS) % KS) * P::PC + (k % KS);
   }
@@ -65,6 +65,12 @@
   int npart, act, trim;
   ConvView vres, vgate;
   int d2w;
+};
+
+struct ConvShortcut {
+  const float *in, *wp, *bias;
+  int cin, h, w, cout_pad;
+  ConvView vin;
 };
 
 
@@ -88,7 +94,8 @@
 __device__ __forceinline__ void conv_epilogue(f32x16 (&acc)[MT][NT], const ConvEpilogue &ep, const float *inp,
                                               float *outp, const ConvView &vin, const ConvView &vout, int t, int r0,
                                               int c0, int cout0, int cout, int ho, int wo, int wm, int wn, int l31,
-                                              int half, const float *bias_s, const float *slope_s) {
+                                              int half, const float *bias_s, const float *slope_s,
+                                              const f32x16 (*sc_acc)[NT] = nullptr, const float *sbias_s = nullptr) {
   const int32_t *__restrict__ col_limit = ep.col_limit;
   const int npart = ep.npart, act = ep.act;
   const int trim_at = ((ep.trim || act == 2 || act == 3) && col_limit) ? col_limit[t % npart] : wo;
@@ -169,6 +176,7 @@
             }
             if (gatep) v = q1[rr][n] * v;
             if (resp) v = rv[rr][n] + v;
+            if (sc_acc) v = (sc_acc[m][n][r] + sbias_s[co - cout0]) + v;
             if (ocol >= trim_at) v = 0.f;
             outp[oi] = v;
           }
@@ -276,12 +284,14 @@
   *reinterpret_cast<__attribute__((address_space(1))) v4f *>((glb_char_t *)base + off) = q;
 }
 
-template <int MT, int WM, int WN, bool SQ, bool RES>
+template <int MT, int WM, int WN, bool SQ, bool RES, bool SCUT = false>
 __device__ __forceinline__ void conv_epilogue_quads(f32x16 (&acc)[MT][1], const ConvEpilogue &ep, const float *in_t,
                                                     float *out_t, const ConvView &vin, const ConvView &vout, int t,
                                                     int r0, int c0, int cout0, int ho, int wo, int wm, int wn, int l31,
                                                     int half, float *park, const float *bias_s, const float *slope_s,
-                                                    int tid) {
+                                                    int tid, const f32x16 (*sc_acc)[1] = nullptr, float *park2 = nullptr,
+                                                    const float *sbias_s = nullptr) {
+  static_assert(!(RES && SCUT), "the shortcut stands where the residual stands");
   constexpr int PX = 32 * WN, QROW = PX / 4, RROWS = 32 * WM, NQR = RROWS * QROW / 512, RSTEP = 512 / QROW;
   static_assert(WM * WN == 8 && RROWS * QROW % 512 == 0 && 32 % RSTEP == 0, "eight waves, whole quads per lane and round");
   const int act = ep.act;
@@ -302,21 +312,21 @@
     float4 r, x;
   };
   constexpr int NF = MT * NQR;
-  constexpr int D = (SQ && RES) ? PCONV_QUAD_AHEAD_GDN : PCONV_QUAD_AHEAD;
+  constexpr int D = SCUT ? 1 : (SQ && RES) ? PCONV_QUAD_AHEAD_GDN : PCONV_QUAD_AHEAD;
   QuadIn ring[D + 1];
   auto request = [&](auto fc) {
     constexpr int f = decltype(fc)::value, m = f / NQR, j = f % NQR;
     if (RES) ring[f % (D + 1)].r = ld4_base_off(res_t + (size_t)krow(m, j) * ep.vres.cs, lb_res);
     if (SQ) ring[f % (D + 1)].x = ld4_base_off(x_t + (size_t)krow(m, j) * vin.cs, lb_in);
   };
-  auto finish = [&](float v, float xv, float rv, float sl, bool trimmed, auto preluc, auto trimc) {
+  auto finish = [&](float v, float xv, float rv, float sl, bool trimmed, auto preluc, auto trimc, auto addc) {
     if (SQ) {
       const float nrm = sqrtf(v);
       v = act == 2 ? xv / nrm : xv * nrm;
     } else if (decltype(preluc)::value) {
       if (v < 0) v = v * sl;
     }
-    if (RES) v = rv + v;
+    if (RES && decltype(addc)::value) v = rv + v;
     if (decltype(trimc)::value && trimmed) v = 0.f;
     return v;
   };
@@ -331,16 +341,38 @@
     const float xs[4] = {src.x.x, src.x.y, src.x.z, src.x.w};
     const float rs[4] = {src.r.x, src.r.y, src.r.z, src.r.w};
     float v[4];
-#pragma unroll
-    for (int k = 0; k < 4; k++) v[k] = finish(o[k] + bco, xs[k], rs[k], sl, ocol + k >= trim_at, preluc, trimc);
+    if constexpr (SCUT) {
+#pragma unroll
+      for (int k = 0; k < 4; k++) v[k] = finish(o[k] + bco, xs[k], 0.f, sl, false, preluc, std::false_type{}, std::false_type{});
+      asm volatile("" : "+v"(v[0]), "+v"(v[1]), "+v"(v[2]), "+v"(v[3]));
+      const float4 s4 = *reinterpret_cast<const float4 *>(park2 + (j * RSTEP + row0) * PX + px);
+      const float sb = sbias_s[cb];
+      const float ss[4] = {s4.x + sb, s4.y + sb, s4.z + sb, s4.w + sb};
+#pragma unroll
+      for (int k = 0; k < 4; k++) {
+        v[k] = ss[k] + v[k];
+        if (decltype(trimc)::value && ocol + k >= trim_at) v[k] = 0.f;
+      }
+    } else {
+#pragma unroll
+      for (int k = 0; k < 4; k++) v[k] = finish(o[k] + bco, xs[k], rs[k], sl, ocol + k >= trim_at, preluc, trimc, std::true_type{});
+    }
     if (row_ok) st4_base_off(o_t + (size_t)krow(m, j) * vout.cs, lb_out, make_float4(v[0], v[1], v[2], v[3]));
   };
   auto whole_tile = [&](auto preluc, auto trimc) {
-    if constexpr (RES || SQ) static_for_<0, (D < NF ? D : NF)>([&](auto fc) { request(fc); });
+    auto first_requests = [&]() {
+      if constexpr (RES || SQ) static_for_<0, (D < NF ? D : NF)>([&](auto fc) { request(fc); });
+    };
+    if constexpr (!SCUT) first_requests();
     static_for_<0, MT>([&](auto mc) {
       constexpr int m = decltype(mc)::value;
 #pragma unroll
       for (int r = 0; r < 16; r++) park[(wm * 32 + (r & 3) + 8 * (r >> 2) + 4 * half) * PX + wn * 32 + l31] = acc[m][0][r];
+      if constexpr (SCUT) {
+#pragma unroll
+        for (int r = 0; r < 16; r++) park2[(wm * 32 + (r & 3) + 8 * (r >> 2) + 4 * half) * PX + wn * 32 + l31] = sc_acc[m][0][r];
+        if constexpr (m == 0) first_requests();
+      }
       asm volatile("s_waitcnt lgkmcnt(0)\n\ts_barrier" ::: "memory");
       static_for_<0, NQR>([&](auto jc) {
         constexpr int f = m * NQR + decltype(jc)::value;
@@ -520,11 +552,88 @@
   }
 }
 
+template <class C, bool SQ>
+__device__ __forceinline__ void conv_gemm(f32x16 (&acc)[C::MTv][C::NTv], const float *inp, const float *wp, int cin, int h,
+                                          int w, int cout_pad, int cout0, const ConvView &vin, int r0, int c0, float *lds,
+                                          int tid, int wave, int wm, int wn, int l31, int half,
+                                          unsigned long long *first_chunk) {
+  using P = typename C::P;
+  constexpr int MT = C::MTv, NT = C::NTv, KC = C::KCv, S = C::Sv;
+  unsigned xoffs[C::XLD], woffs[C::WLD];
+#pragma unroll
+  for (int j = 0; j < C::XLD; j++) {
+    int e = tid + j * C::THREADS;
+    e = e < C::XSZ ? e : 0;
+    const int pc = e % P::PC;
+    const int pr = (e / P::PC) % P::PR;
+    const int ci = e / (P::PC * P::PR);
+    int ir = r0 * S + pr * P::PS;
+    int ic = c0 * S + pc * P::PS;
+    ir = ir < h ? ir : h - 1;
+    ic = ic < w ? ic : w - 1;
+    xoffs[j] = (unsigned)((ci * vin.cs + (long long)ir * vin.rs + ic) * 4);
+  }
+#pragma unroll
+  for (int j = 0; j < C::WLD; j++) {
+    int e4 = tid + j * C::THREADS;
+    e4 = e4 < C::WSZ / 4 ? e4 : 0;
+    const int kk = e4 / (C::BM / 4);
+    const int co = (e4 % (C::BM / 4)) * 4;
+    woffs[j] = (unsigned)(kk * cout_pad + co) * 4u;
+  }
+  const int nchunk = (cin + KC - 1) / KC;
+  const int tail = cin % KC;
+  const size_t xstep = (size_t)KC * vin.cs, wstep = (size_t)C::KK * cout_pad;
+
+  auto stager = [&](int chunk, int buf) {
+    float *xs = lds + buf * C::STAGE;
+    return ConvStager<C>{inp + chunk * xstep, wp + chunk * wstep + cout0, xs, xs + C::XSZ, xoffs, woffs, tid, wave, tail,
+                         vin.cs, chunk < nchunk, tail != 0 && chunk == nchunk - 1};
+  };
+
+  const unsigned lds0 = (unsigned)reinterpret_cast<uintptr_t>(lds);
+  unsigned abase = lds0 + (unsigned)(C::XSZ + half * C::BM + wm * MT * 32 + l31) * 4u;
+  unsigned bbase[NT][C::ND];
+#pragma unroll
+  for (int n = 0; n < NT; n++) {
+    const int seg = wn * NT + n;
+    const int prow = seg >> 1, pcol = (seg & 1) * 32 + l31;
+#pragma unroll
+    for (int d = 0; d < C::ND; d++)
+      bbase[n][d] = lds0 + (unsigned)(prow * P::Q * P::PC + pcol * P::Q + half * C::delta(d)) * 4u;
+  }
+  static_assert(C::STAGE * 4 <= 65536, "operand offsets of one buffer fit the 16-bit immediate");
+  static_assert(kAhead * (MT + NT) <= 15, "lgkmcnt counts to 15");
+
+  stager(0, 0).issue_all();
+  __syncthreads();
+#ifdef PCONV_CONV_STAMP
+  if (first_chunk) *first_chunk = __builtin_readcyclecounter();
+#endif
+
+  for (int chunk = 0; chunk < nchunk; chunk++) {
+    stager(chunk + 1, (chunk & 1) ^ 1).issue_all();
+    float a[kAhead + 1][MT], b[kAhead + 1][NT];
+    conv_chunk_prologue<C, 0>(a, b, abase, bbase);
+    conv_chunk_step<C, SQ, 0>(acc, a, b, abase, bbase);
+    const unsigned flip = (chunk & 1) ? (unsigned)(-C::STAGE * 4) : (unsigned)(C::STAGE * 4);
+    abase += flip;
+#pragma unroll
+    for (int n = 0; n < NT; n++)
+#pragma unroll
+      for (int d = 0; d < C::ND; d++) bbase[n][d] += flip;
+    __syncthreads();
+  }
+}
+
 #ifndef PCONV_1X1_WAVES_EU
 #define PCONV_1X1_WAVES_EU 2
 #endif
 #ifndef PCONV_1X1_EPI_ROWS
 #define PCONV_1X1_EPI_ROWS 16
+#endif
+#ifndef PCONV_SHORTCUT_WAVES_EU
+#define PCONV_SHORTCUT_WAVES_EU 4
 #endif
 
 #ifndef PCONV_QUAD_FALLBACK_ROWS
@@ -537,15 +646,19 @@
 #define CONV_STAMP(v)
 #endif
 
-template <int MT, int NT, int WM, int WN, int KS, int S, int KC, bool SQ, int WAY = 0>
-__global__ __launch_bounds__(64 * WM * WN, (KS == 1 && S == 1 && MT == 3) ? PCONV_1X1_WAVES_EU : 2) void conv_mfma_kernel(
+template <class C, int WM, int WN, int SC>
+constexpr int conv_lds_floats() {
+  return SC ? 2 * 32 * WM * 32 * WN + 3 * C::BM : 2 * C::STAGE;
+}
+
+template <int MT, int NT, int WM, int WN, int KS, int S, int KC, bool SQ, int WAY = 0, int SC = 0>
+__global__ __launch_bounds__(64 * WM * WN, SC ? PCONV_SHORTCUT_WAVES_EU : (KS == 1 && S == 1 && MT == 3) ? PCONV_1X1_WAVES_EU : 2) void conv_mfma_kernel(
     const float *__restrict__ in, const float *__restrict__ wp, float *__restrict__ out, int cin, int h,
     int w, int cout, int cout_pad, int ho, int wo, int tiles_r, int tiles_c, int cblocks, int xcd_group, ConvView vin,
-    ConvView vout, ConvEpilogue ep) {
+    ConvView vout, ConvEpilogue ep, ConvShortcut sc) {
   const int32_t *__restrict__ col_limit = ep.col_limit;
   const int npart = ep.npart;
   using C = ConvCfg<MT, NT, WM, WN, KS, S, KC>;
-  using P = typename C::P;
   constexpr int kThreads = C::THREADS;
   constexpr int kTileRows = C::ROWS;
   extern __shared__ float lds[];
@@ -582,60 +695,6 @@
   }
 
   const float *inp = in + (size_t)t * vin.ts;
-  const int nchunk = (cin + KC - 1) / KC;
-
-  f32x16 acc[MT][NT];
-#pragma unroll
-  for (int m = 0; m < MT; m++)
-#pragma unroll
-    for (int n = 0; n < NT; n++)
-#pragma unroll
-      for (int r = 0; r < 16; r++) acc[m][n][r] = 0.f;
-
-  unsigned xoffs[C::XLD], woffs[C::WLD];
-#pragma unroll
-  for (int j = 0; j < C::XLD; j++) {
-    int e = tid + j * kThreads;
-    e = e < C::XSZ ? e : 0;
-    const int pc = e % P::PC;
-    const int pr = (e / P::PC) % P::PR;
-    const int ci = e / (P::PC * P::PR);
-    int ir = r0 * S + pr * P::PS;
-    int ic = c0 * S + pc * P::PS;
-    ir = ir < h ? ir : h - 1;
-    ic = ic < w ? ic : w - 1;
-    xoffs[j] = (unsigned)((ci * vin.cs + (long long)ir * vin.rs + ic) * 4);
-  }
-#pragma unroll
-  for (int j = 0; j < C::WLD; j++) {
-    int e4 = tid + j * kThreads;
-    e4 = e4 < C::WSZ / 4 ? e4 : 0;
-    const int kk = e4 / (C::BM / 4);
-    const int co = (e4 % (C::BM / 4)) * 4;
-    woffs[j] = (unsigned)(kk * cout_pad + co) * 4u;
-  }
-  const int tail = cin % KC;
-  const size_t xstep = (size_t)KC * vin.cs, wstep = (size_t)C::KK * cout_pad;
-
-  auto stager = [&](int chunk, int buf) {
-    float *xs = lds + buf * C::STAGE;
-    return ConvStager<C>{inp + chunk * xstep, wp + chunk * wstep + cout0, xs, xs + C::XSZ, xoffs, woffs, tid, wave, tail,
-                         vin.cs, chunk < nchunk, tail != 0 && chunk == nchunk - 1};
-  };
-
-  const unsigned lds0 = (unsigned)reinterpret_cast<uintptr_t>(lds);
-  unsigned abase = lds0 + (unsigned)(C::XSZ + half * C::BM + wm * MT * 32 + l31) * 4u;
-  unsigned bbase[NT][C::ND];
-#pragma unroll
-  for (int n = 0; n < NT; n++) {
-    const int seg = wn * NT + n;
-    const int prow = seg >> 1, pcol = (seg & 1) * 32 + l31;
-#pragma unroll
-    for (int d = 0; d < C::ND; d++)
-      bbase[n][d] = lds0 + (unsigned)(prow * P::Q * P::PC + pcol * P::Q + half * C::delta(d)) * 4u;
-  }
-  static_assert(C::STAGE * 4 <= 65536, "operand offsets of one buffer fit the 16-bit immediate");
-  static_assert(kAhead * (MT + NT) <= 15, "lgkmcnt counts to 15");
 
   float my_bias = 0.f, my_slope = 0.f;
   if (tid < C::BM) {
@@ -643,34 +702,62 @@
     if (ep.bias) my_bias = ep.bias[co];
     if (ep.act == 1) my_slope = ep.slope[co];
   }
-
-  stager(0, 0).issue_all();
-  __syncthreads();
-  CONV_STAMP(st1);
-
-  for (int chunk = 0; chunk < nchunk; chunk++) {
-    stager(chunk + 1, (chunk & 1) ^ 1).issue_all();
-    float a[kAhead + 1][MT], b[kAhead + 1][NT];
-    conv_chunk_prologue<C, 0>(a, b, abase, bbase);
-    conv_chunk_step<C, SQ, 0>(acc, a, b, abase, bbase);
-    const unsigned flip = (chunk & 1) ? (unsigned)(-C::STAGE * 4) : (unsigned)(C::STAGE * 4);
-    abase += flip;
+  constexpr int kRound = 32 * WM * 32 * WN;
+  static_assert(!SC || 2 * kRound >= 2 * C::STAGE, "the shortcut's tables lie past the stages");
+  float *const tables = lds + (SC ? 2 * kRound : 0), *const park = SC ? lds : lds + 2 * C::BM;
+  f32x16 acc2[MT][NT];
+  if constexpr (SC) {
+    using C2 = ConvCfg<MT, NT, WM, WN, 1, 2, KC>;
+    static_assert(!SC || (KS == 1 && S == 1 && C2::XSZ == C::XSZ && C2::STAGE == C::STAGE), "the shortcut shares the layer's stages");
+#pragma unroll
+    for (int m = 0; m < MT; m++)
+#pragma unroll
+      for (int n = 0; n < NT; n++)
+#pragma unroll
+        for (int r = 0; r < 16; r++) acc2[m][n][r] = 0.f;
+    float my_sbias = 0.f;
+    if (tid < C::BM && sc.bias) my_sbias = sc.bias[cout0 + tid < cout ? cout0 + tid : cout - 1];
+    conv_gemm<C2, false>(acc2, sc.in + (size_t)t * sc.vin.ts, sc.wp, sc.cin, sc.h, sc.w, sc.cout_pad, cout0, sc.vin, r0, c0, lds,
+                         tid, wave, wm, wn, l31, half, nullptr);
+    if (tid < C::BM) {
+      tables[tid] = my_bias;
+      tables[C::BM + tid] = my_slope;
+      tables[2 * C::BM + tid] = my_sbias;
+    }
+  }
+
+  f32x16 acc[MT][NT];
+#pragma unroll
+  for (int m = 0; m < MT; m++)
 #pragma unroll
     for (int n = 0; n < NT; n++)
 #pragma unroll
-      for (int d = 0; d < C::ND; d++) bbase[n][d] += flip;
-    __syncthreads();
-  }
+      for (int r = 0; r < 16; r++) acc[m][n][r] = 0.f;
+
+  unsigned long long *first_chunk = nullptr;
+#ifdef PCONV_CONV_STAMP
+  unsigned long long st1 = 0;
+  first_chunk = &st1;
+#endif
+  conv_gemm<C, SQ>(acc, inp, wp, cin, h, w, cout_pad, cout0, vin, r0, c0, lds, tid, wave, wm, wn, l31, half, first_chunk);
 
   CONV_STAMP(st2);
   static_assert(2 * C::BM <= C::STAGE && C::BM <= kThreads, "bias / slope table fits the stage memory");
-  if (tid < C::BM) {
-    lds[tid] = my_bias;
-    lds[C::BM + tid] = my_slope;
+  if (!SC && tid < C::BM) {
+    tables[tid] = my_bias;
+    tables[C::BM + tid] = my_slope;
   }
   __syncthreads();
   {
-    if constexpr (WAY == 0) {
+    if constexpr (SC) {
+      static_assert(!SC || (WAY == 3 && MT == 3 && NT == 1 && kThreads == 512), "shortcut: the quad way out, 96 couts x 32 pixels per wave");
+      if (c0 + kTileCols <= wo && cout0 + C::BM <= cout)
+        conv_epilogue_quads<MT, WM, WN, SQ, false, true>(acc, ep, inp, outp, vin, vout, t, r0, c0, cout0, ho, wo, wm, wn, l31, half,
+                                                         park, tables, tables + C::BM, tid, acc2, park + kRound, tables + 2 * C::BM);
+      else
+        conv_epilogue<MT, NT, WN, PCONV_QUAD_FALLBACK_ROWS>(acc, ep, inp, outp, vin, vout, t, r0, c0, cout0, cout, ho, wo, wm, wn, l31, half,
+                                                           tables, tables + C::BM, acc2, tables + 2 * C::BM);
+    } else if constexpr (WAY == 0) {
       conv_epilogue<MT, NT, WN, (KS == 1 && S == 1 && MT == 3) ? PCONV_1X1_EPI_ROWS : 16>(acc, ep, inp, outp, vin, vout, t, r0, c0, cout0,
                                                                                           cout, ho, wo, wm, wn, l31, half, lds, lds + C::BM);
     } else if constexpr (WAY == 5) {
@@ -1125,10 +1212,10 @@
   packed[i] = (co < cout && kk < red) ? w[(size_t)co * red + kk] : 0.f;
 }
 
-template <int MT, int NT, int WM, int WN, int KS, int S, int KC, bool SQ = false, int WAY = 0>
+template <int MT, int NT, int WM, int WN, int KS, int S, int KC, bool SQ = false, int WAY = 0, int SC = 0>
 int launch_conv(const float *in, const float *wp, float *out, int tn, int cin, int h, int w, int cout,
                 int cout_pad, int ho, int wo, const ConvView &vin, const ConvView &vout, const ConvEpilogue &ep,
-                const ConvOptions &opt, hipStream_t stream) {
+                const ConvOptions &opt, hipStream_t stream, const ConvShortcut &sc = ConvShortcut()) {
   using C = ConvCfg<MT, NT, WM, WN, KS, S, KC>;
   constexpr int kThreads = C::THREADS;
   constexpr int kTileRows = C::ROWS;
@@ -1140,15 +1227,15 @@
     pconv_set_error("conv2d: grid %lld out of range", grid);
     return PCONV_EINVAL;
   }
-  const size_t smem = (size_t)2 * C::STAGE * sizeof(float);
-  auto kern = conv_mfma_kernel<MT, NT, WM, WN, KS, S, KC, SQ, WAY>;
+  const size_t smem = (size_t)conv_lds_floats<C, WM, WN, SC>() * sizeof(float);
+  auto kern = conv_mfma_kernel<MT, NT, WM, WN, KS, S, KC, SQ, WAY, SC>;
   if (smem > 64 * 1024) {
     static std::atomic<unsigned long long> raised{0};
     if (int rc = pconv_raise_lds(kern, smem, raised, "conv2d")) return rc;
   }
   const int xcd_group = (opt.xcd == 1 && KS == 3) ? cblocks * tiles_r : 0;
   hipLaunchKernelGGL(kern, dim3((unsigned)grid), dim3(kThreads), smem, stream, in, wp, out, cin, h, w, cout,
-                     cout_pad, ho, wo, tiles_r, tiles_c, cblocks, xcd_group, vin, vout, ep);
+                     cout_pad, ho, wo, tiles_r, tiles_c, cblocks, xcd_group, vin, vout, ep, sc);
   return PCONV_OK;
 }
 
@@ -1357,3 +1444,48 @@
   PCONV_LAUNCH_CHECK("gdn");
   return PCONV_OK;
 }
+
+namespace {
+inline bool shortcut_kernel_takes(const ConvOptions &opt, int mode, int ch, int tn, int h, int w) {
+  return mode == PCONV_SHORTCUT_DOWN && ch > 96 && quad_way_out(opt) && !use_resident_1x1(opt, ch, ch, tn, h, w);
+}
+}
+
+extern "C" int pconv_gdn_shortcut_takes(int mode, int ch, int sc_cin, int tn, int h, int w) {
+  const ConvOptions opt = ConvOptions::from_env();
+  if (!shortcut_kernel_takes(opt, mode, ch, tn, h, w) || sc_cin <= 0) return 0;
+  const bool measured = ch == 192 && ((sc_cin == 3 && w == 2048) || (sc_cin == 192 && (w == 1024 || w == 512)));
+  return measured ? 2 : 1;
+}
+
+extern "C" int pconv_gdn_shortcut(const float *in, const float *packed_gamma, const float *beta, float *out, int tn, int ch,
+                                  int h, int w, int inverse, const int32_t *col_limit, int npart, int mode,
+                                  const float *sc_in, const float *sc_packed_w, const float *sc_bias, int sc_cin, int sc_h,
+                                  int sc_w, const long long *views, void *stream) {
+  PCONV_REQUIRE(in && packed_gamma && beta && out && in != out && sc_in && sc_packed_w && sc_in != out, "gdn_shortcut: bad pointer");
+  PCONV_REQUIRE(tn > 0 && ch > 0 && h > 0 && w > 0, "gdn_shortcut: bad shape");
+  PCONV_REQUIRE(!col_limit || npart > 0, "gdn_shortcut: col_limit needs npart");
+  PCONV_REQUIRE(mode == PCONV_SHORTCUT_DOWN, "gdn_shortcut: mode %d is not built", mode);
+  PCONV_REQUIRE(sc_cin > 0 && sc_h > 0 && sc_w > 0 && (sc_h - 1) / 2 + 1 == h && (sc_w - 1) / 2 + 1 == w,
+                "gdn_shortcut: a %d x %d shortcut input does not give %d x %d at stride 2", sc_h, sc_w, h, w);
+  int cp, rp, scp, srp;
+  pconv_conv_packed_size(ch, ch, 1, &cp, &rp);
+  pconv_conv_packed_size(ch, sc_cin, 1, &scp, &srp);
+  hipStream_t s = as_stream(stream);
+  const ConvOptions opt = ConvOptions::from_env();
+  PCONV_REQUIRE(shortcut_kernel_takes(opt, mode, ch, tn, h, w), "gdn_shortcut: %d channels with these options: no kernel", ch);
+  const ConvView vin = view_at(views, 0, ch, h, w), vout = view_at(views, 1, ch, h, w);
+  const ConvShortcut sc = {sc_in, sc_packed_w, sc_bias, sc_cin, sc_h, sc_w, scp, view_at(views, 2, sc_cin, sc_h, sc_w)};
+  const ConvEpilogue ep = {beta, nullptr, nullptr, nullptr, col_limit, npart, inverse ? 3 : 2, 1,
+                           dense_view(ch, h, w), dense_view(ch, h, w), 0};
+  PCONV_REQUIRE(view_ok(vin, ch, h, w) && view_ok(vout, ch, h, w) && view_ok(sc.vin, sc_cin, sc_h, sc_w), "gdn_shortcut: strides overlap");
+  PCONV_REQUIRE(((long long)(32 - 1) * vin.cs + (long long)(h - 1) * vin.rs + w) * 4 < (1LL << 32) &&
+                    ((long long)(PCONV_KC1 - 1) * sc.vin.cs + (long long)(sc_h - 1) * sc.vin.rs + sc_w) * 4 < (1LL << 32) &&
+                    ((long long)(32 - 1) * vout.cs + (long long)(h - 1) * vout.rs + w) * 4 < (1LL << 32),
+                "gdn_shortcut: channel stride too large for 32-bit byte offsets");
+  if (int rc = launch_conv<3, 1, 2, 4, 1, 1, PCONV_KC1, true, 3, 1>(in, packed_gamma, out, tn, ch, h, w, ch, cp, h, w, vin, vout, ep,
+                                                                     opt, s, sc))
+    return rc;
+  PCONV_LAUNCH_CHECK("gdn_shortcut");
+  return PCONV_OK;
+}
diff --git a/pseudocylindrical_convolution_amd/model_zoo_v2.py b/pseudocylindrical_convolution_amd/model_zoo_v2.py
--- a/pseudocylindrical_convolution_amd/model_zoo_v2.py
+++ b/pseudocylindrical_convolution_amd/model_zoo_v2.py
@@ -92,6 +92,7 @@
 
 
 RING = 2 if os.environ.get("PCONV_PAD_RING", "1") == "1" else 0
+GDN_SHORTCUT = os.environ.get("PCONV_GDN_SHORTCUT", "auto")
 
 
 def _conv(cin, cout, k, stride=1):
@@ -169,11 +170,22 @@
         self.trim = PseudoFillV2(0, npart, ctx, device=device_id)
         self.__dict__["ctx"] = ctx
 
+    def _fused_shortcut(self, x):
+        ops = backend.ops()
+        if GDN_SHORTCUT == "off" or not hasattr(ops, "gdn_shortcut_takes") or x.dim() != 4 or not self.relu2.fuses(x):
+            return False
+        out = (x.shape[0], self.short_cut.out_channels, (x.shape[2] - 1) // 2 + 1, (x.shape[3] - 1) // 2 + 1)
+        return ops.gdn_shortcut_takes(self.short_cut, x, out) >= (1 if GDN_SHORTCUT == "on" else 2)
+
     def forward(self, x):
         live = (self.ctx, x.shape[3] // 2)
-        t = self.short_cut(x, live)
+        fused = self._fused_shortcut(x)
+        t = None if fused else self.short_cut(x, live)
         y = self.conv1.fuse(self.pad1(x), self.relu1, live, ring=RING)
-        return self.relu2(self.conv2(self.pad2(y), live), residual=t, trim=self.trim, ring=RING)
+        y = self.conv2(self.pad2(y), live)
+        if fused:
+            return self.relu2(y, shortcut=(self.short_cut, x), trim=self.trim, ring=RING)
+        return self.relu2(y, residual=t, trim=self.trim, ring=RING)
 
 
 class SphereConv2(nn.Module):
```

Result: no change. 95.81 MPix/s (median of 6 runs) (+0.6%).
